# DerekRowell/AudioSDR

Hardware: AMD Instinct MI355X
Metric: Msamples/s through full SSB demod chain, batched 128-sample blocks (higher is better)
Workload: dtype f32

## Files before the change

### audiosdr_amd/binding.py

```python
import ctypes as C
import os

import numpy as np

BLOCK = 128
ALL = -1
STREAM_BATCH = (1 << 64) - 1
LSBmode, USBmode, CW_LSBmode, CW_USBmode, AMmode, SAMmode, WSPRmode = range(7)
(audioAM, audioCW, audioWSPR, audio2100, audio2300, audio2500, audio2700, audio2900, audio3100, audio3300,
 audioBypass) = range(11)
AGCoff, AGCfast, AGCmedium, AGCslow = range(4)
TAPS = ["SCALED_I", "SCALED_Q", "NB_I", "NB_Q", "IF_I", "IF_Q", "MIX_I", "MIX_Q", "DEMOD", "AUDIO_FILT", "AGC", "ALS"]

_HERE = os.path.dirname(os.path.abspath(__file__))


class AsdrError(RuntimeError):
    pass


def library_path():
    return os.path.join(_HERE, "libasdr_hip.so")


def library_sha256(path=None):
    import hashlib
    with open(path or library_path(), "rb") as f:
        return hashlib.sha256(f.read()).hexdigest()


_f, _i, _u = C.c_float, C.c_int, C.c_uint
_SETTERS_VOID = ["init", "enableAudioFilter", "disableAudioFilter", "enableALSfilter", "disableALSfilter",
                 "setALSfilterNotch", "setALSfilterPeak", "setALSfilterAdaptive", "setALSfilterStatic", "enableAGC",
                 "disableAGC", "enableNoiseBlanker", "disableNoiseBlanker"]
_SETTERS_F = ["setInputGain", "setIQgainBalance", "setOutputGain", "setAGCthreshold", "setAGCslope", "setAGCkneeWidth",
              "setAGCattackTime", "setAGCreleaseTime", "setAGChangTime", "setAGCstaticGain", "setNoiseBlankerThreshold",
              "setNoiseBlankerThresholdDb"]
_SETTERS_I = ["setMute", "setAudioFilter", "setAGCmode"]
_GETTERS_F = ["getTuningOffset", "getBPFlower", "getBPFupper", "getAGCthreshold", "getAGCslope", "getAGCkneeWidth",
              "getAGCattack", "getAGCrelease", "getAAGalphaAttack", "getAGCbetaAttack", "getAGCalphaRelease",
              "getAGCbetaRelease", "getAGCstaticGain", "getAMcarrierLevel", "getSAMfrequency"]
_GETTERS_I = ["getMute", "getAudioFilter", "ALSfilterIsEnabled", "ALSfilterIsNotch", "ALSfilterIsPeak",
              "ALSfilterIsAdaptive", "AGCisEnabled", "AGCisActive", "NoiseBlankerisEnabled", "NoiseBlankerDetection",
              "getSAMphaseLockStatus"]

EXPORTS = (["asdr_create", "asdr_destroy", "asdr_last_error", "asdr_n_channels", "asdr_update", "asdr_update_device",
            "asdr_synchronize", "asdr_setDemodMode", "asdr_getDemodMode", "asdr_setALSfilterParams", "asdr_getAGClookup",
            "asdr_read_status", "asdr_control_plane_flush", "asdr_get_chain_constants", "asdr_stream_pipeline_launches", "asdr_schedule_layout", "asdr_set_exact_unknown_mode", "asdr_get_exact_unknown_mode", "asdr_stream_pipeline_recoveries", "asdr_stream_pipeline_max_groups", "asdr_set_stream_fir_helpers", "asdr_stream_pipeline_h3_calls", "asdr_set_stream_pipeline", "asdr_set_sam_launch_form", "asdr_set_als_launch_form", "asdr_debug_set_stream_spin_limit", "asdr_debug_set_stream_max_groups", "asdr_enable_taps", "asdr_read_taps", "asdr_last_kernel_ms", "asdr_version",
            "asdr_kernel_timing_begin", "asdr_kernel_timing_end", "asdr_set_launch_timing", "asdr_region_timing_begin", "asdr_region_timing_end", "asdr_update_device_strided", "asdr_capture_open",
            "asdr_capture_close", "asdr_capture_capacity", "asdr_capture_position", "asdr_capture_rewind",
            "asdr_capture_device_ptr", "asdr_capture_update_device", "asdr_capture_read",
            "asdr_create_sharded", "asdr_n_shards", "asdr_shard", "asdr_shard_first_channel", "asdr_shard_device",
            "asdr_host_alloc", "asdr_host_free", "asdr_host_register", "asdr_host_unregister", "asdr_set_host_chunks",
            "asdr_host_path_info", "asdr_stream_pipeline_alloc_failures", "asdr_set_launch_split", "asdr_order_after", "asdr_order_before", "asdr_lane_calls", "asdr_sam_role_calls", "asdr_sam_chunk_calls", "asdr_als_role_calls", "asdr_set_lanes"] +
           ["asdr_" + n for n in _SETTERS_VOID + _SETTERS_F + _SETTERS_I + _GETTERS_F + _GETTERS_I])

_lib = None


def host_autopin(on=-1):
    return int(load_library().asdr_host_autopin(int(on)))


def host_autopin_clear():
    load_library().asdr_host_autopin_clear()


def host_autopin_info():
    out = (C.c_long * 4)()
    load_library().asdr_host_autopin_info(out)
    return {"registered_now": int(out[0]), "registrations": int(out[1]), "released": int(out[2]), "refused": int(out[3])}


def kernels_launched(reset=False):
    L = load_library()
    out = {}
    for i in range(L.asdr_kernels_count()):
        n = int(L.asdr_kernels_launches(i))
        if n:
            out[L.asdr_kernels_name(i).decode()] = n
    if reset:
        L.asdr_kernels_launches_reset()
    return out


def load_library(path=None):
    global _lib
    if _lib is not None and path is None:
        return _lib
    p = path or library_path()
    if not os.path.exists(p):
        raise AsdrError("%s not found: build it with `python -m audiosdr_amd.build` (hipcc, gfx950). "
                        "There is no CPU fallback." % p)
    L = C.CDLL(p)
    vp, i16p = C.c_void_p, C.POINTER(C.c_int16)
    L.asdr_create.argtypes = [_i, _i]; L.asdr_create.restype = vp
    L.asdr_destroy.argtypes = [vp]; L.asdr_destroy.restype = None
    L.asdr_last_error.restype = C.c_char_p
    L.asdr_version.restype = C.c_char_p
    L.asdr_set_pool_priority.argtypes = [_i]; L.asdr_set_pool_priority.restype = _i
    L.asdr_host_autopin.argtypes = [_i]; L.asdr_host_autopin.restype = _i
    L.asdr_host_autopin_clear.restype = None
    L.asdr_host_autopin_info.argtypes = [C.POINTER(C.c_long)]; L.asdr_host_autopin_info.restype = _i
    L.asdr_kernels_count.restype = _i
    L.asdr_kernels_name.argtypes = [_i]; L.asdr_kernels_name.restype = C.c_char_p
    L.asdr_kernels_launches.argtypes = [_i]; L.asdr_kernels_launches.restype = C.c_ulonglong
    L.asdr_kernels_launches_reset.restype = None
    L.asdr_n_channels.argtypes = [vp]; L.asdr_n_channels.restype = _i
    L.asdr_update.argtypes = [vp, i16p, i16p, i16p, _i]; L.asdr_update.restype = _i
    L.asdr_update_device.argtypes = [vp, vp, vp, vp, _i, vp]; L.asdr_update_device.restype = _i
    L.asdr_synchronize.argtypes = [vp]; L.asdr_synchronize.restype = _i
    L.asdr_update_device_strided.argtypes = [vp, vp, vp, vp, _i, C.c_long, C.c_long, vp]; L.asdr_update_device_strided.restype = _i
    L.asdr_capture_open.argtypes = [vp, C.c_long]; L.asdr_capture_open.restype = _i
    for n in ("asdr_capture_close", "asdr_capture_rewind"):
        getattr(L, n).argtypes = [vp]; getattr(L, n).restype = _i
    for n in ("asdr_capture_capacity", "asdr_capture_position"):
        getattr(L, n).argtypes = [vp]; getattr(L, n).restype = C.c_long
    L.asdr_capture_device_ptr.argtypes = [vp]; L.asdr_capture_device_ptr.restype = vp
    L.asdr_capture_update_device.argtypes = [vp, vp, vp, _i, C.c_long, vp]; L.asdr_capture_update_device.restype = _i
    L.asdr_capture_read.argtypes = [vp, _i, C.c_long, C.c_long, i16p]; L.asdr_capture_read.restype = _i
    L.asdr_last_kernel_ms.argtypes = [vp]; L.asdr_last_kernel_ms.restype = _f
    for n in _SETTERS_VOID:
        fn = getattr(L, "asdr_" + n); fn.argtypes = [vp, _i]; fn.restype = None
    for n in _SETTERS_F:
        fn = getattr(L, "asdr_" + n); fn.argtypes = [vp, _i, _f]; fn.restype = None
    for n in _SETTERS_I:
        fn = getattr(L, "asdr_" + n); fn.argtypes = [vp, _i, _i]; fn.restype = None
    for n in _GETTERS_F:
        fn = getattr(L, "asdr_" + n); fn.argtypes = [vp, _i]; fn.restype = _f
    for n in _GETTERS_I:
        fn = getattr(L, "asdr_" + n); fn.argtypes = [vp, _i]; fn.restype = _i
    L.asdr_setDemodMode.argtypes = [vp, _i, _i]; L.asdr_setDemodMode.restype = _f
    L.asdr_getDemodMode.argtypes = [vp, _i]; L.asdr_getDemodMode.restype = C.c_int16
    L.asdr_setALSfilterParams.argtypes = [vp, _i, _u, _f, _f]; L.asdr_setALSfilterParams.restype = None
    L.asdr_getAGClookup.argtypes = [vp, _i, _i]; L.asdr_getAGClookup.restype = _f
    i32p, fp = C.POINTER(C.c_int32), C.POINTER(C.c_float)
    L.asdr_read_status.argtypes = [vp, i32p, i32p, i32p, fp, fp]; L.asdr_read_status.restype = _i
    if path is None or hasattr(L, "asdr_get_chain_constants"):
        L.asdr_get_chain_constants.argtypes = [vp, _i, C.POINTER(C.c_float)]; L.asdr_get_chain_constants.restype = C.c_uint
    if path is None or hasattr(L, "asdr_control_plane_flush"):
        L.asdr_control_plane_flush.argtypes = [vp, C.POINTER(C.c_longlong)]; L.asdr_control_plane_flush.restype = _i
    L.asdr_enable_taps.argtypes = [vp, _i]; L.asdr_enable_taps.restype = _i
    L.asdr_read_taps.argtypes = [vp, fp]; L.asdr_read_taps.restype = _i
    L.asdr_kernel_timing_begin.argtypes = [vp, _i]; L.asdr_kernel_timing_begin.restype = _i
    if path is None or hasattr(L, "asdr_stream_pipeline_launches"):
        L.asdr_stream_pipeline_launches.argtypes = [vp]; L.asdr_stream_pipeline_launches.restype = C.c_long
    if path is None or hasattr(L, "asdr_set_stream_pipeline"):
        L.asdr_stream_pipeline_recoveries.argtypes = [vp]; L.asdr_stream_pipeline_recoveries.restype = C.c_long
        L.asdr_stream_pipeline_max_groups.argtypes = [vp]; L.asdr_stream_pipeline_max_groups.restype = _i
        if hasattr(L, "asdr_set_stream_fir_helpers"):
            L.asdr_set_stream_fir_helpers.argtypes = [vp, _i]; L.asdr_set_stream_fir_helpers.restype = _i
            L.asdr_stream_pipeline_h3_calls.argtypes = [vp]; L.asdr_stream_pipeline_h3_calls.restype = C.c_long
        L.asdr_set_stream_pipeline.argtypes = [vp, _i]; L.asdr_set_stream_pipeline.restype = _i
        L.asdr_set_sam_launch_form.argtypes = [vp, _i, _i]; L.asdr_set_sam_launch_form.restype = _i
        if hasattr(L, "asdr_set_als_launch_form"):
            L.asdr_set_als_launch_form.argtypes = [vp, _i]; L.asdr_set_als_launch_form.restype = _i
        L.asdr_debug_set_stream_spin_limit.argtypes = [vp, _u]; L.asdr_debug_set_stream_spin_limit.restype = _i
        L.asdr_debug_set_stream_max_groups.argtypes = [vp, _i]; L.asdr_debug_set_stream_max_groups.restype = _i
    if path is None or hasattr(L, "asdr_set_exact_unknown_mode"):
        L.asdr_set_exact_unknown_mode.argtypes = [vp, _i]; L.asdr_set_exact_unknown_mode.restype = _i
        L.asdr_get_exact_unknown_mode.argtypes = [vp]; L.asdr_get_exact_unknown_mode.restype = _i
    if path is None or hasattr(L, "asdr_schedule_layout"):
        L.asdr_schedule_layout.argtypes = [vp, C.POINTER(C.c_int)]; L.asdr_schedule_layout.restype = _i
    if path is None or hasattr(L, "asdr_region_timing_begin"):
        L.asdr_set_launch_timing.argtypes = [vp, _i]; L.asdr_set_launch_timing.restype = _i
        L.asdr_region_timing_begin.argtypes = [vp, vp]; L.asdr_region_timing_begin.restype = _i
        L.asdr_region_timing_end.argtypes = [vp, C.POINTER(C.c_float), C.POINTER(C.c_long)]; L.asdr_region_timing_end.restype = _i
    L.asdr_kernel_timing_end.argtypes = [vp, fp, _i]; L.asdr_kernel_timing_end.restype = _i
    if path is None or hasattr(L, "asdr_create_sharded"):
        L.asdr_create_sharded.argtypes = [_i, _i, C.POINTER(C.c_int)]; L.asdr_create_sharded.restype = vp
        L.asdr_n_shards.argtypes = [vp]; L.asdr_n_shards.restype = _i
        L.asdr_shard.argtypes = [vp, _i]; L.asdr_shard.restype = vp
        L.asdr_shard_first_channel.argtypes = [vp, _i]; L.asdr_shard_first_channel.restype = _i
        L.asdr_shard_device.argtypes = [vp, _i]; L.asdr_shard_device.restype = _i
        L.asdr_host_alloc.argtypes = [C.c_size_t]; L.asdr_host_alloc.restype = vp
        L.asdr_host_free.argtypes = [vp]; L.asdr_host_free.restype = None
        L.asdr_host_register.argtypes = [vp, C.c_size_t]; L.asdr_host_register.restype = _i
        L.asdr_host_unregister.argtypes = [vp]; L.asdr_host_unregister.restype = _i
        L.asdr_set_host_chunks.argtypes = [vp, _i]; L.asdr_set_host_chunks.restype = _i
        L.asdr_host_path_info.argtypes = [vp, C.POINTER(C.c_int)]; L.asdr_host_path_info.restype = _i
        L.asdr_stream_pipeline_alloc_failures.argtypes = [vp]; L.asdr_stream_pipeline_alloc_failures.restype = C.c_long
        L.asdr_set_launch_split.argtypes = [vp, _i, _i]; L.asdr_set_launch_split.restype = _i
        L.asdr_order_after.argtypes = [vp, vp]; L.asdr_order_after.restype = _i
        L.asdr_order_before.argtypes = [vp, vp]; L.asdr_order_before.restype = _i
        L.asdr_lane_calls.argtypes = [vp]; L.asdr_lane_calls.restype = C.c_long
        L.asdr_sam_role_calls.argtypes = [vp]; L.asdr_sam_role_calls.restype = C.c_long
        L.asdr_als_role_calls.argtypes = [vp]; L.asdr_als_role_calls.restype = C.c_long
        L.asdr_sam_chunk_calls.argtypes = [vp]; L.asdr_sam_chunk_calls.restype = C.c_long
        L.asdr_set_lanes.argtypes = [vp, _i, _i]; L.asdr_set_lanes.restype = _i
    if path is None or hasattr(L, "asdr_lanes_overlap_probe"):
        L.asdr_lanes_overlap_probe.argtypes = [vp]; L.asdr_lanes_overlap_probe.restype = _i
        L.asdr_lanes_enabled.argtypes = [vp]; L.asdr_lanes_enabled.restype = _i
        L.asdr_stream_pipeline_headroom_refusals.argtypes = [vp]; L.asdr_stream_pipeline_headroom_refusals.restype = C.c_long
    if path is None:
# ... 112 lines not shown
    def update_device(self, dI, dQ, dOut, n_blocks, stream=0):
        self._chk(self._L.asdr_update_device(self._h, C.c_void_p(dI), C.c_void_p(dQ), C.c_void_p(dOut), int(n_blocks),
                                             C.c_void_p(stream)))

    def update_device_strided(self, dI, dQ, dOut, n_blocks, in_stride_blocks, out_stride_blocks, stream=0):
        self._chk(self._L.asdr_update_device_strided(self._h, C.c_void_p(dI), C.c_void_p(dQ), C.c_void_p(dOut), int(n_blocks),
                                                     int(in_stride_blocks), int(out_stride_blocks), C.c_void_p(stream)))

    def synchronize(self):
        self._chk(self._L.asdr_synchronize(self._h))

    def capture_open(self, capacity_blocks):
        self._chk(self._L.asdr_capture_open(self._h, int(capacity_blocks)))

    def capture_close(self):
        self._chk(self._L.asdr_capture_close(self._h))

    def capture_rewind(self):
        self._chk(self._L.asdr_capture_rewind(self._h))

    @property
    def capture_position(self):
        return int(self._L.asdr_capture_position(self._h))

    @property
    def capture_capacity(self):
        return int(self._L.asdr_capture_capacity(self._h))

    def capture_device_ptr(self):
        return int(self._L.asdr_capture_device_ptr(self._h) or 0)

    def capture_update_device(self, dI, dQ, n_blocks, in_stride_blocks=None, stream=0):
        self._chk(self._L.asdr_capture_update_device(self._h, C.c_void_p(dI), C.c_void_p(dQ), int(n_blocks),
                                                     int(n_blocks if in_stride_blocks is None else in_stride_blocks), C.c_void_p(stream)))

    def capture_read(self, ch, first_block=0, n_blocks=None):
        if n_blocks is None:
            n_blocks = self.capture_position - first_block
        out = np.empty(int(n_blocks) * BLOCK, dtype=np.int16)
        self._chk(self._L.asdr_capture_read(self._h, int(ch), int(first_block), int(n_blocks), out.ctypes.data_as(C.POINTER(C.c_int16))))
        return out

    def chain_constants(self, ch=0):
        out = (C.c_float * 12)()
        hang = int(self._L.asdr_get_chain_constants(self._h, int(ch), out))
        return hang, np.array(list(out), dtype=np.float32)

    def control_plane_flush(self):
        st = (C.c_longlong * 4)()
        self._chk(self._L.asdr_control_plane_flush(self._h, st))
        return {"rows_refilled": int(st[0]), "schedule_rebuilt": bool(st[1]), "waves_plain": int(st[2]) & 0x1FFFFF,
                "waves_sam": (int(st[2]) >> 21) & 0x1FFFFF, "waves_als": (int(st[2]) >> 42) & 0x1FFFFF, "agc_tables_alive": int(st[3])}

    def last_kernel_ms(self):
        return float(self._L.asdr_last_kernel_ms(self._h))

    def set_exact_unknown_mode(self, on=True):
        self._chk(self._L.asdr_set_exact_unknown_mode(self._h, 1 if on else 0))

    def stream_pipeline_launches(self):
        return int(self._L.asdr_stream_pipeline_launches(self._h))

    def stream_pipeline_recoveries(self):
        return int(self._L.asdr_stream_pipeline_recoveries(self._h))

    def stream_pipeline_max_groups(self):
        return int(self._L.asdr_stream_pipeline_max_groups(self._h))

    def set_stream_fir_helpers(self, mode):
        self._chk(self._L.asdr_set_stream_fir_helpers(self._h, int(mode)))

    def stream_pipeline_h3_calls(self):
        return int(self._L.asdr_stream_pipeline_h3_calls(self._h))

    def set_stream_pipeline(self, on=True):
        self._chk(self._L.asdr_set_stream_pipeline(self._h, 1 if on else 0))

    def set_sam_launch_form(self, fused=False, split_min_channels=0):
        self._chk(self._L.asdr_set_sam_launch_form(self._h, 1 if fused else 0, int(split_min_channels)))

    def set_als_launch_form(self, split_min_channels=0):
        self._chk(self._L.asdr_set_als_launch_form(self._h, int(split_min_channels)))

    def debug_set_stream_max_groups(self, groups):
        self._chk(self._L.asdr_debug_set_stream_max_groups(self._h, int(groups)))

    def debug_set_stream_spin_limit(self, polls):
        self._chk(self._L.asdr_debug_set_stream_spin_limit(self._h, int(polls)))

    def schedule_layout(self):
        out = (C.c_int * 8)()
        self._chk(self._L.asdr_schedule_layout(self._h, out))
        v = list(out)
        return {"plain": v[0], "sam": v[1], "als_long": v[2], "als_compact": v[3], "sam_als": v[4], "remainders": v[5],
                "remainder_kind": v[6], "sam_three_launches": bool(v[7] & 1), "als_two_launches": bool(v[7] & 2)}

    def set_launch_timing(self, on):
        self._chk(self._L.asdr_set_launch_timing(self._h, 1 if on else 0))

    def region_timing_begin(self, stream=None):
        self._chk(self._L.asdr_region_timing_begin(self._h, stream))

    def region_timing_end(self):
        ms, n = C.c_float(0.0), C.c_long(0)
        self._chk(self._L.asdr_region_timing_end(self._h, C.byref(ms), C.byref(n)))
        return float(ms.value), int(n.value)
# ... 92 lines not shown
```

### audiosdr_amd/csrc/asdr_device.h

```cpp
#ifndef ASDR_DEVICE_H_
#define ASDR_DEVICE_H_

#include <stdint.h>

#define ASDR_N 128
#define ASDR_PLL_WRAP_MAX 64

#define ASDR_F_NB_EN        (1u << 0)
#define ASDR_F_AF_EN        (1u << 1)
#define ASDR_F_AGC_EN       (1u << 2)
#define ASDR_F_ALS_EN       (1u << 3)
#define ASDR_F_ALS_NOTCH    (1u << 4)
#define ASDR_F_ALS_ADAPTIVE (1u << 5)
#define ASDR_F_MUTED        (1u << 6)

#define ASDR_R_IF   (1u << 0)
#define ASDR_R_AF   (1u << 1)
#define ASDR_R_NB   (1u << 2)
#define ASDR_R_ALS  (1u << 3)
#define ASDR_R_IMG  (1u << 4)
#define ASDR_R_ALL  (1u << 5)

typedef struct {
  uint32_t mode;
// ... 59 lines not shown
#define ASDR_LO_ENTRIES 8
#define ASDR_LO_WRITER 0x100u
#define ASDR_LO_WRITER_LANE(l) (0x100u << (l))

typedef struct {
  uint32_t key_phase, key_inc;
  float phase_end;
  uint32_t pad_;
  float c[ASDR_N], s[ASDR_N];
} LoEntry;

typedef struct {
  const ChanParams *params;
  ChanSmall *small;
  int16_t *nb_hist;
  uint8_t *nb_mask;
  float *hil_q, *hil_i, *als_x, *als_w;
  float *audio_prev;
  const float *agc_tab;
  const SlotInfo *sched;
  int32_t n_sched;
  int32_t n_channels;
  const int16_t *in_i, *in_q;
  int16_t *out;
  int32_t n_blocks;
  uint32_t nb_phase;
  uint32_t als_phase;
  LoEntry *lo_cache;
  uint32_t lo_parity;
  uint32_t lo_write;
  uint32_t lo_writer_bit;
  uint32_t direct_lo;
  int32_t direct_ch0;
  uint32_t direct_mode, direct_flags;
  int32_t in_stride;
  int32_t out_stride;
  float *taps;
  float *xch_a;
  float *xch_b;
  float *xch_c;
  uint32_t *stream_prog;
  uint32_t *stream_err;
  uint32_t stream_spin_limit;
  const uint32_t *run_if;
  int32_t stream_waves;
  float *xch_sam;
  uint32_t *sam_lock;
  uint32_t sam_set, sam_sets;
  uint32_t sam_set_stride, sam_lock_stride;
  float *als_stage;
  uint32_t als_stage_cur, als_stage_prev;
  LoEntry *lo_ring;
  ChainConsts k;
} UpdateArgs;
#define ASDR_ALS_STAGE_SLOTS 32
#define ASDR_ALS_CHUNK 8
#define ASDR_STREAM_DEPTH 4
#define ASDR_LO_RING 8
#define ASDR_STREAM_SPIN_LIMIT (1u << 18)
#define ASDR_STREAM_FAIL 0xFFFFFFFFu
#define ASDR_SNAP_BYTES (448 + 1536 + ASDR_NB_MASK_ROW + 1024 + 1024 + 512)

#define ASDR_KERNEL_PLAIN 0
#define ASDR_KERNEL_SAM 1
#define ASDR_KERNEL_ALS 2
#define ASDR_KERNEL_ALS_SMALL 3
#define ASDR_KERNEL_SAM_ALS 4
#define ASDR_KERNEL_KINDS 5
#ifndef ASDR_SAM_WAVES
#define ASDR_SAM_WAVES 4
#endif

#endif
```

### audiosdr_amd/csrc/asdr_host.cpp

```cpp
#include <hip/hip_runtime.h>

#include <algorithm>
#include <atomic>
#include <chrono>
#include <condition_variable>
#include <functional>
#include <memory>
#include <mutex>
#include <thread>
#include <cmath>
#include <cstdio>
#include <cstring>
#include <string>
#include <unordered_map>
#include <vector>

#include "../../include/asdr.h"
#include "asdr_device.h"
#include "asdr_tables.h"

#ifndef ASDR_SAM_CHUNK
#define ASDR_SAM_CHUNK 8
#define ASDR_SAM_CHUNK_SETS 32
#define ASDR_SAM_CHUNK_MAX_WAVES 512
// ... 118 lines not shown
  explicit CopyPool(int n) { for (int i = 0; i < n; i++) th_.emplace_back([this] { loop(); }); }
  ~CopyPool() { { std::lock_guard<std::mutex> g(m_); quit_ = true; } cv_.notify_all(); for (auto &t : th_) t.join(); }
  int threads() const { return (int)th_.size(); }
  void start(Job *j) { j->workers_left.store((int)th_.size()); { std::lock_guard<std::mutex> g(m_); job_ = j; gen_++; } cv_.notify_all(); }
  static void work(Job *j) {
    const int n_tasks = j->n_chunks * j->slices;
    for (int t; (t = j->next_in.fetch_add(1)) < n_tasks;) { const int k = t / j->slices; j->copy_in(k, t % j->slices, j->slices); j->in_done[k].fetch_add(1, std::memory_order_release); }
    for (int t; (t = j->next_out.fetch_add(1)) < n_tasks;) {
      const int k = t / j->slices;
      while (!j->out_ready[k].load(std::memory_order_acquire)) nap();
      j->copy_out(k, t % j->slices, j->slices); j->out_finished.fetch_add(1, std::memory_order_release);
    }
  }
 private:
  void loop() {
    unsigned long seen = 0;
    for (;;) {
      Job *j;
      { std::unique_lock<std::mutex> g(m_); cv_.wait(g, [&] { return quit_ || gen_ != seen; }); if (quit_) return; seen = gen_; j = job_; }
      work(j);
      j->workers_left.fetch_sub(1, std::memory_order_release);
    }
  }
  std::vector<std::thread> th_;
  std::mutex m_; std::condition_variable cv_;
  Job *job_ = nullptr; unsigned long gen_ = 0; bool quit_ = false;
};

struct HostPlan { int K = 1; std::vector<int> bound, need_in, last_part; long sched_gen = -1; int n_blocks = 0; };

}

#define ASDR_LANES 8
#define ASDR_AUX_STREAMS (ASDR_KERNEL_KINDS + 1 + 8)
struct asdr_batch {
  int n = 0, device = 0;
  hipStream_t stream = nullptr;
  std::vector<Chan> ch;
  std::vector<AgcTable> agc_pool;
  std::unordered_map<uint64_t, std::vector<int>> agc_index;
  std::vector<uint32_t> agc_refs;
  std::vector<ChanParams> hp;
  std::vector<uint32_t> reset;
  std::vector<SlotInfo> sched;
  std::vector<int32_t> dirty;
  std::vector<uint8_t> dirty_flag;
  bool all_dirty = true;
  bool sched_dirty = true, reset_pending = true, agc_pool_dirty = true;
  bool agc_refs_changed = true;
  int reset_lo = 0x7fffffff, reset_hi = -1;
  int kind_first[ASDR_KERNEL_KINDS] = {}, kind_slots[ASDR_KERNEL_KINDS] = {}, kind_uniform_slots[ASDR_KERNEL_KINDS] = {};
  int left_first = 0, left_slots = 0, left_kind = ASDR_KERNEL_PLAIN;
  bool kind_direct[ASDR_KERNEL_KINDS] = {};
  long stat_rows_refilled = 0, stat_sched_rebuilds = 0, stat_bulk_uploads = 0;
  int stat_lo_groups_without_entry = 0;
  ChanParams *d_params = nullptr;
  ChanSmall *d_small = nullptr;
  int16_t *d_nb_hist = nullptr;
  uint8_t *d_nb_mask = nullptr;
  float *d_hil_q = nullptr, *d_hil_i = nullptr, *d_als_x = nullptr,
        *d_als_w = nullptr, *d_agc_tab = nullptr, *d_taps = nullptr;
  float *d_audio_prev = nullptr;
  bool exact_unknown_mode = true;
  size_t agc_tab_cap = 0;
  SlotInfo *d_sched = nullptr;
  uint32_t *d_reset = nullptr;
  int16_t *d_io[3] = {nullptr, nullptr, nullptr};
  int16_t *h_io[3] = {nullptr, nullptr, nullptr};
  size_t h_io_cap = 0;
  hipStream_t h2d_stream = nullptr, d2h_stream = nullptr;
  std::vector<hipEvent_t> ev_host;
  HostPlan host_plan;
  std::unique_ptr<CopyPool> copy_pool;
  int host_chunks_forced = 0;
  hipStream_t lane[ASDR_LANES + 1] = {};
  hipEvent_t ev_lane[ASDR_LANES + 1] = {};
  int n_lanes = 2, n_lanes_sam = 3;
  int sched_lanes = 2;
  bool lanes_pending = false;
  bool sched_sam_heavy = false;
  bool last_was_lanes = false;
  int lanes_min_waves = 1024;
  bool lanes_enabled = true;
  bool lanes_forced = false;
  long stat_lane_calls = 0;
  int launch_split = 1, launch_split_min_waves = 2048;
  int stat_host_chunks = 0, stat_host_pinned = 0;
  std::vector<asdr_batch *> shards;
  std::vector<int> shard_first;
  void *workers = nullptr;
  int16_t *d_capture = nullptr;
  long capture_cap = 0, capture_pos = 0;
  size_t io_cap = 0;
  bool taps_on = false;
  hipEvent_t ev0 = nullptr, ev1 = nullptr;
  bool ev_valid = false;
  bool time_calls = false;
  hipEvent_t rev0 = nullptr, rev1 = nullptr;
  hipStream_t region_stream = nullptr;
  bool region_on_lanes = false;
  long region_calls = -1;
  std::vector<hipEvent_t> tev;
  size_t tev_used = 0;
  hipStream_t last_stream = nullptr;
  hipEvent_t ev_last = nullptr;
  hipStream_t aux[ASDR_AUX_STREAMS] = {};
// ... 132 lines not shown
  c.agc_en = true;
  rebuild_agc(b, c);
}

void chan_init(asdr_batch *b, int idx) {
  Chan &c = b->ch[idx];
  c.audio_table = ASDR_TBL_AUDIO_BASE + ASDR_audio2700;
  c.if_table = ASDR_TBL_IF_SSB;
  mark_reset(b, idx, ASDR_R_AF | ASDR_R_IF | ASDR_R_IMG | ASDR_R_NB);
  agc_init(b, c);
  set_mode(b, idx, ASDR_LSBmode);
  c.muted = false;
}

void fill_params(const Chan &c, ChanParams &p) {
  memset(&p, 0, sizeof p);
  p.mode = c.mode;
  p.flags = (c.nb_en ? ASDR_F_NB_EN : 0u) | (c.af_en ? ASDR_F_AF_EN : 0u) | (c.agc_en ? ASDR_F_AGC_EN : 0u) |
            (c.als_en ? ASDR_F_ALS_EN : 0u) | (c.als_notch ? ASDR_F_ALS_NOTCH : 0u) |
            (c.als_adaptive ? ASDR_F_ALS_ADAPTIVE : 0u) | (c.muted ? ASDR_F_MUTED : 0u);
  p.if_table = c.if_table; p.audio_table = c.audio_table; p.agc_table = c.agc_table;
  p.in_gain_i = c.in_gain_i; p.in_gain_q = c.in_gain_q; p.output_gain = c.output_gain;
  p.freq_shift = c.freq_shift; p.nb_threshold = c.nb_threshold;
  p.agc_alpha_att = c.agc_alpha_att; p.agc_beta_att = c.agc_beta_att;
  p.agc_alpha_rel = c.agc_alpha_rel; p.agc_beta_rel = c.agc_beta_rel;
  p.agc_static_gain = c.agc_static_gain; p.agc_hang_count = c.agc_hang_count;
  p.als_m = c.als_m; p.als_delay = c.als_delay; p.als_lambda = c.als_lambda;
}

int g_force_split = -1;
int kernel_kind(const ChanParams &p) {
  if (g_force_split < 0) g_force_split = getenv("ASDR_FORCE_SPLIT") ? 1 : 0;
  if (g_force_split && !(p.flags & ASDR_F_ALS_EN)) return ASDR_KERNEL_SAM;
  if (p.flags & ASDR_F_ALS_EN) {
    const bool small = p.als_m >= 0 && p.als_m <= 64 && p.als_delay >= 0 && p.als_delay + p.als_m <= 65;
    return !small ? ASDR_KERNEL_ALS : (p.mode == ASDR_SAMmode ? ASDR_KERNEL_SAM_ALS : ASDR_KERNEL_ALS_SMALL);
  }
  return (p.mode == ASDR_SAMmode) ? ASDR_KERNEL_SAM : ASDR_KERNEL_PLAIN;
}
#ifndef ASDR_SAM_SPLIT_MIN_CHANNELS
#define ASDR_SAM_SPLIT_MIN_CHANNELS 512
#endif
uint64_t sched_key(const ChanParams &p) {
  return ((uint64_t)kernel_kind(p) << 60) | ((uint64_t)(p.mode & 0xFFFF) << 40) | ((uint64_t)(p.flags & 0xFF) << 32) |
         ((uint64_t)(p.if_table & 0xFF) << 24) | ((uint64_t)(p.audio_table & 0xFF) << 16) | (uint64_t)(p.agc_table & 0xFFFF);
}

void mark_dirty(asdr_batch *b, int i) {
  if (b->all_dirty) return;
  if (!b->dirty_flag[i]) { b->dirty_flag[i] = 1; b->dirty.push_back(i); }
  if (b->dirty.size() > (size_t)b->n / 8 + 64) { b->all_dirty = true; }
}

void flush_host(asdr_batch *b, std::vector<int32_t> &rows_out, bool &bulk, bool &sched_rebuilt) {
  const int rows = b->n + 1;
  compact_agc_pool(b);
  bulk = b->all_dirty;
  rows_out.clear();
  b->stat_rows_refilled = 0;
  if (bulk) {
    for (int i = 0; i < rows; i++) {
      const uint64_t old_key = sched_key(b->hp[i]);
      fill_params(b->ch[i], b->hp[i]);
      if (i < b->n && sched_key(b->hp[i]) != old_key) b->sched_dirty = true;
    }
    b->stat_rows_refilled = rows;
    b->stat_bulk_uploads++;
  } else if (!b->dirty.empty()) {
    std::sort(b->dirty.begin(), b->dirty.end());
    for (int32_t i : b->dirty) {
      const uint64_t old_key = sched_key(b->hp[i]);
      fill_params(b->ch[i], b->hp[i]);
      if (sched_key(b->hp[i]) != old_key) b->sched_dirty = true;
      b->dirty_flag[i] = 0;
    }
    rows_out = b->dirty;
    b->stat_rows_refilled = (long)rows_out.size();
  }
  b->dirty.clear();
  if (bulk) std::fill(b->dirty_flag.begin(), b->dirty_flag.end(), 0);
  b->all_dirty = false;
  sched_rebuilt = false;
  if (b->sched_dirty) {
    std::vector<std::pair<uint64_t, int32_t>> order(b->n);
    for (int i = 0; i < b->n; i++) order[i] = {sched_key(b->hp[i]), i};
    std::sort(order.begin(), order.end());
    int uni[ASDR_KERNEL_KINDS] = {}, rem[ASDR_KERNEL_KINDS] = {};
    int n_sam = 0;
    for (int i = 0; i < b->n; i++) { const int k = (int)(order[i].first >> 60); n_sam += (k == ASDR_KERNEL_SAM || k == ASDR_KERNEL_SAM_ALS); }
    b->sam_split = !b->sam_fused && n_sam >= b->sam_split_min;
    {
      int n_als_small = 0;
      for (int i = 0; i < b->n; i++) n_als_small += ((int)(order[i].first >> 60) == ASDR_KERNEL_ALS_SMALL);
      b->als_split = n_als_small >= b->als_split_min;
    }
    const bool sam_general_only = !b->sam_split;
    int left = 0; bool left_general = false;
    for (int i = 0; i < b->n;) {
      int j = i + 1;
      while (j < b->n && order[j].first == order[i].first) j++;
      const int k = (int)(order[i].first >> 60), g = j - i;
      if (k == ASDR_KERNEL_SAM && sam_general_only) rem[k] += g;
      else { uni[k] += g / 8 * 8; left += g % 8; if (g % 8) left_general = left_general || (k != ASDR_KERNEL_PLAIN); }
      i = j;
    }
    int pos = 0;
    for (int k = 0; k < ASDR_KERNEL_KINDS; k++) {
      b->kind_first[k] = pos; b->kind_uniform_slots[k] = uni[k]; b->kind_slots[k] = uni[k] + ((rem[k] + 7) / 8) * 8;
      pos += b->kind_slots[k];
    }
    b->left_first = pos; b->left_slots = (left + 7) / 8 * 8; b->left_kind = left_general ? ASDR_KERNEL_ALS : ASDR_KERNEL_PLAIN;
    pos += b->left_slots;
    b->sched.assign(pos, SlotInfo{b->n, b->hp[b->n].mode, b->hp[b->n].flags, 0u});
    int at_u[ASDR_KERNEL_KINDS], at_m[ASDR_KERNEL_KINDS], at_left = b->left_first;
    for (int k = 0; k < ASDR_KERNEL_KINDS; k++) { at_u[k] = b->kind_first[k]; at_m[k] = b->kind_first[k] + uni[k]; }
    std::unordered_map<uint64_t, uint32_t> lo_of_key;
    {
      std::vector<std::pair<int, uint64_t>> cand;
      for (int i = 0; i < b->n;) {
        int j = i + 1;
        while (j < b->n && order[j].first == order[i].first) j++;
        const int k = (int)(order[i].first >> 60), g = j - i;
        const int whole = (k == ASDR_KERNEL_SAM && sam_general_only) ? 0 : g / 8 * 8;
        const uint32_t gm = b->hp[order[i].second].mode;
        const bool mixes_early = (gm == ASDR_USBmode || gm == ASDR_LSBmode || gm == ASDR_CW_USBmode || gm == ASDR_CW_LSBmode || gm == ASDR_WSPRmode || gm == ASDR_AMmode);
        if (whole > 0 && mixes_early) cand.push_back({-whole, order[i].first});
        i = j;
      }
// ... 5 lines not shown
      int j = i + 1;
      while (j < b->n && order[j].first == order[i].first) j++;
      const int k = (int)(order[i].first >> 60), g = j - i;
      const bool fused = (k == ASDR_KERNEL_SAM && sam_general_only);
      const int whole = fused ? 0 : g / 8 * 8;
      const auto lo_it = lo_of_key.find(order[i].first);
      const uint32_t lo_id = (whole > 0 && lo_it != lo_of_key.end()) ? lo_it->second : 0u;
      for (int t = 0; t < g; t++) {
        const int c = order[i + t].second;
        int &at = (t < whole) ? at_u[k] : (fused ? at_m[k] : at_left);
        const uint32_t lo = (t < whole) ? (lo_id | ((t < 8 && lo_id) ? ASDR_LO_WRITER : 0u)) : 0u;
        b->sched[at++] = SlotInfo{c, b->hp[c].mode, b->hp[c].flags, lo};
      }
      i = j;
    }
    {
      const int sam_slots_ = b->kind_slots[ASDR_KERNEL_SAM] + b->kind_slots[ASDR_KERNEL_SAM_ALS];
      b->sched_sam_heavy = b->sam_split && 2 * sam_slots_ >= pos;
      b->sched_lanes = b->sched_sam_heavy ? b->n_lanes_sam : b->n_lanes;
    }
    for (int k = 0; k < ASDR_KERNEL_KINDS; k++) {
      const long w = b->kind_uniform_slots[k] / 8;
      for (int l = 1; l < b->sched_lanes; l++) {
        const int lo = b->kind_first[k] + (int)(w * l / b->sched_lanes) * 8, hi = b->kind_first[k] + (int)(w * (l + 1) / b->sched_lanes) * 8;
        uint32_t seen = 0;
        for (int sl = lo; sl < hi; sl += 8) {
          const uint32_t id = b->sched[sl].lo & 0xFFu;
          if (id == 0u || (seen >> id) & 1u) continue;
          seen |= 1u << id;
          for (int t = 0; t < 8; t++) b->sched[sl + t].lo |= ASDR_LO_WRITER_LANE(l);
        }
      }
    }
    for (int k = 0; k < ASDR_KERNEL_KINDS; k++) {
      const SlotInfo *sl = b->sched.data() + b->kind_first[k];
      bool direct = b->kind_uniform_slots[k] > 0;
      for (int j = 1; j < b->kind_uniform_slots[k] && direct; j++)
        direct = (sl[j].ch == sl[0].ch + j) && sl[j].mode == sl[0].mode && sl[j].flags == sl[0].flags;
      b->kind_direct[k] = direct;
    }
    {
      const SlotInfo *sl = b->sched.data() + b->kind_first[ASDR_KERNEL_PLAIN];
      bool ssb = b->kind_uniform_slots[ASDR_KERNEL_PLAIN] > 0;
      for (int j = 0; j < b->kind_uniform_slots[ASDR_KERNEL_PLAIN] && ssb; j += 8) {
        const uint32_t m = sl[j].mode;
        ssb = (m == ASDR_USBmode || m == ASDR_LSBmode || m == ASDR_CW_USBmode || m == ASDR_CW_LSBmode || m == ASDR_WSPRmode ||
               m == ASDR_AMmode);
      }
      b->plain_uniform_ssb = ssb;
    }
    b->sched_dirty = false;
    sched_rebuilt = true;
    b->stat_sched_rebuilds++;
  }
}

int flush(asdr_batch *b, hipStream_t stream) {
  const int rows = b->n + 1;
  std::vector<int32_t> changed;
  bool bulk = false, sched_rebuilt = false;
  flush_host(b, changed, bulk, sched_rebuilt);
  bool uploaded = false;
  if (b->agc_pool_dirty) {
    const size_t need = b->agc_pool.size() * ASDR_AGC_TAB_ROW;
    if (need > b->agc_tab_cap) {
      HIPCHK(hipStreamSynchronize(stream));
      if (b->d_agc_tab) HIPCHK(hipFree(b->d_agc_tab));
      b->agc_tab_cap = need * 2;
      HIPCHK(hipMalloc(&b->d_agc_tab, b->agc_tab_cap * sizeof(float)));
    }
    std::vector<float> flat(need);
    for (size_t i = 0; i < b->agc_pool.size(); i++) memcpy(&flat[i * ASDR_AGC_TAB_ROW], b->agc_pool[i].v, sizeof(float) * ASDR_AGC_TAB_ROW);
    HIPCHK(hipMemcpyAsync(b->d_agc_tab, flat.data(), need * sizeof(float), hipMemcpyHostToDevice, stream));
    HIPCHK(hipStreamSynchronize(stream));
    b->agc_pool_dirty = false;
  }
  if (bulk) {
    HIPCHK(hipMemcpyAsync(b->d_params, b->hp.data(), rows * sizeof(ChanParams), hipMemcpyHostToDevice, stream));
    uploaded = true;
  } else {
    for (size_t i = 0; i < changed.size();) {
      size_t j = i + 1;
      while (j < changed.size() && changed[j] == changed[j - 1] + 1) j++;
      HIPCHK(hipMemcpyAsync(b->d_params + changed[i], &b->hp[changed[i]], (j - i) * sizeof(ChanParams), hipMemcpyHostToDevice, stream));
      uploaded = true;
      i = j;
    }
  }
  if (sched_rebuilt) {
    HIPCHK(hipMemcpyAsync(b->d_sched, b->sched.data(), b->sched.size() * sizeof(SlotInfo), hipMemcpyHostToDevice, stream));
    uploaded = true;
  }
  if (uploaded) HIPCHK(hipStreamSynchronize(stream));
  return 0;
}

void fill_args(asdr_batch *b, UpdateArgs &a) {
  memset(&a, 0, sizeof a);
  a.params = b->d_params; a.small = b->d_small;
  a.nb_hist = b->d_nb_hist; a.nb_mask = b->d_nb_mask; a.hil_q = b->d_hil_q; a.hil_i = b->d_hil_i;
  a.als_x = b->d_als_x; a.als_w = b->d_als_w; a.agc_tab = b->d_agc_tab;
  a.audio_prev = b->exact_unknown_mode ? b->d_audio_prev : nullptr;
  a.sched = b->d_sched; a.n_sched = 0; a.n_channels = b->n;
  a.taps = b->taps_on ? b->d_taps : nullptr;
  a.nb_phase = b->nb_phase; a.als_phase = b->als_phase;
  a.lo_cache = b->d_lo; a.lo_parity = b->lo_parity; a.lo_write = 0; a.lo_writer_bit = ASDR_LO_WRITER;
  a.k = b->k;
}

int apply_resets(asdr_batch *b, hipStream_t stream) {
  if (!b->reset_pending) return 0;
  const int lo = b->reset_lo < 0 ? 0 : b->reset_lo, hi = b->reset_hi > b->n ? b->n : b->reset_hi;
  if (hi >= lo) {
    const int cnt = hi - lo + 1;
    HIPCHK(hipMemcpyAsync(b->d_reset + lo, b->reset.data() + lo, cnt * sizeof(uint32_t), hipMemcpyHostToDevice, stream));
    UpdateArgs a;
    fill_args(b, a);
    if (asdr_launch_reset(&a, b->d_reset, lo, cnt, stream) != 0) return fail("reset kernel launch failed");
    HIPCHK(hipStreamSynchronize(stream));
    std::fill(b->reset.begin() + lo, b->reset.begin() + hi + 1, 0u);
  }
  b->reset_pending = false; b->reset_lo = 0x7fffffff; b->reset_hi = -1;
  return 0;
}

inline bool is_sharded(const asdr_batch *b) { return b && !b->shards.empty(); }
asdr_batch *shard_of(asdr_batch *b, int &ch) {
  if (ch < 0 || ch >= b->n) return nullptr;
  const std::vector<int> &f = b->shard_first;
  int g = (int)(std::upper_bound(f.begin(), f.end(), ch) - f.begin()) - 1;
  ch -= f[g];
  return b->shards[g];
}
template <typename F>
void each(asdr_batch *&b, int ch, F f) {
  if (!b) return;
  if (is_sharded(b)) {
    asdr_batch *const parent = b;
    if (ch == ASDR_ALL) { for (asdr_batch *sh : parent->shards) { b = sh; each(b, ASDR_ALL, f); } }
    else { int local = ch; asdr_batch *sh = shard_of(parent, local); if (sh) { b = sh; each(b, local, f); } }
    b = parent;
    return;
  }
  if (ch == ASDR_ALL) { for (int i = 0; i < b->n; i++) f(i, b->ch[i]); b->all_dirty = true; }
  else if (ch >= 0 && ch < b->n) { f(ch, b->ch[ch]); mark_dirty(b, ch); }
  else return;
}
const Chan *get(asdr_batch *&b, int ch) {
  if (is_sharded(b)) { asdr_batch *sh = shard_of(b, ch); if (!sh) return nullptr; b = sh; }
  return (b && ch >= 0 && ch < b->n) ? &b->ch[ch] : nullptr;
}

constexpr int kPoolMax = 16;
int g_pool_priority = -1;
bool g_pool_created = false;
struct StreamPool { hipStream_t s[kPoolMax] = {}; int size = 0; std::mutex m; };
StreamPool g_pool[16];
constexpr int kPoolDevices = 16;
hipStream_t pool_stream(int device, int i) {
  if (device < 0 || device >= kPoolDevices) return nullptr;
// ... 73 lines not shown
  }
  return 0;
}
int sync_all(asdr_batch *b) {
  HIPCHK(hipStreamSynchronize(b->last_stream));
  HIPCHK(hipStreamSynchronize(b->stream));
  if (b->lanes_pending) { for (int l = 0; l < ASDR_LANES + 1; l++) if (b->lane[l]) HIPCHK(hipStreamSynchronize(b->lane[l])); b->lanes_pending = false; }

  return 0;
}

int check_stream_error(asdr_batch *b) {
  if (!b->stream_launched || !b->d_stream_prog) return 0;
  if (sync_all(b) != 0) return -1;
  uint32_t *word = b->d_stream_prog + 3 * ((b->n + 7) / 8) + 1, v[2] = {0, 0};
  HIPCHK(hipMemcpy(v, word, sizeof v, hipMemcpyDeviceToHost));
  b->stream_launched = false;
  b->stat_stream_recoveries = (long)v[1];
  if (v[0]) return fail("streaming pipeline: error word still set after the recovery launches (internal error)");
  return 0;
}

int read_small(asdr_batch *b, int ch, ChanSmall &s) {
  if (!b || ch < 0 || ch >= b->n) return fail("bad channel");
  if (is_sharded(b)) b = shard_of(b, ch);
  if (b->device == ASDR_NO_DEVICE) return fail("control-plane-only batch has no device state");
  HIPCHK(hipSetDevice(b->device));
  if (sync_all(b) != 0) return -1;
  if (check_stream_error(b) != 0) return -1;
  if (apply_resets(b, b->stream) != 0) return -1;
  HIPCHK(hipMemcpy(&s, b->d_small + ch, sizeof s, hipMemcpyDeviceToHost));
  return 0;
}

}

#define FOR_SHARDS(b, call) do { if (is_sharded(b)) { for (asdr_batch *sh_ : (b)->shards) { const int rc_ = (call); if (rc_ != 0) return rc_; } return 0; } } while (0)

extern "C" {

const char *asdr_last_error(void) { return g_err.c_str(); }
}
int asdr_internal_fail(const std::string &m) { return fail(m); }
extern "C" {
const char *asdr_version(void) { return "asdr-hip 0.1 (gfx950, wave64, -ffp-contract=off)"; }

asdr_batch_t *asdr_create(int n_channels, int device) {
  if (n_channels <= 0 || n_channels > (1 << 20)) { fail("n_channels must be in 1..1048576"); return nullptr; }
  asdr_batch *b = new asdr_batch();
  b->n = n_channels; b->device = device;
  b->sam_fused = getenv("ASDR_SAM_FUSED") != nullptr;
  b->sam_split_min = getenv("ASDR_SAM_SPLIT_MIN") ? atoi(getenv("ASDR_SAM_SPLIT_MIN")) : ASDR_SAM_SPLIT_MIN_CHANNELS;
  b->stream_pipeline = getenv("ASDR_NO_STREAM_PIPELINE") == nullptr;
  b->als_split_min = getenv("ASDR_ALS_SPLIT_MIN") ? atoi(getenv("ASDR_ALS_SPLIT_MIN")) : 0x7fffffff;
  if (getenv("ASDR_LAUNCH_SPLIT")) b->launch_split = std::max(1, std::min(atoi(getenv("ASDR_LAUNCH_SPLIT")), 8));
  if (getenv("ASDR_LAUNCH_SPLIT_MIN_WAVES")) b->launch_split_min_waves = std::max(8, atoi(getenv("ASDR_LAUNCH_SPLIT_MIN_WAVES")));
  const size_t rows = (size_t)n_channels + 1;
  if (device != ASDR_NO_DEVICE) {
    int ndev = 0;
    if (hipGetDeviceCount(&ndev) != hipSuccess || ndev <= 0) { delete b; fail("no HIP device: libasdr_hip has no CPU path"); return nullptr; }
    if (device < 0 || device >= ndev) { delete b; fail("bad device ordinal"); return nullptr; }
    if (device >= 16) { delete b; fail("device ordinal >= 16: the per-device stream pool of this library has 16 entries"); return nullptr; }
    if (hipSetDevice(device) != hipSuccess) { delete b; fail("hipSetDevice failed"); return nullptr; }
    autopin_batch_created();
    bool ok = true;
    auto alloc = [&](void **p, size_t bytes) { if (ok && hipMalloc(p, bytes) != hipSuccess) ok = false; };
    alloc((void **)&b->d_params, rows * sizeof(ChanParams));
    alloc((void **)&b->d_small, rows * sizeof(ChanSmall));
    alloc((void **)&b->d_nb_hist, rows * 768 * sizeof(int16_t));
    alloc((void **)&b->d_nb_mask, rows * ASDR_NB_MASK_ROW * sizeof(uint8_t));
    alloc((void **)&b->d_hil_q, rows * 256 * sizeof(float));
    alloc((void **)&b->d_hil_i, rows * 256 * sizeof(float));
    alloc((void **)&b->d_als_x, rows * 256 * sizeof(float));
    alloc((void **)&b->d_als_w, rows * 128 * sizeof(float));
    alloc((void **)&b->d_audio_prev, rows * 128 * sizeof(float));
    if (ok && hipMemset(b->d_audio_prev, 0, rows * 128 * sizeof(float)) != hipSuccess) ok = false;
    alloc((void **)&b->d_sched, (rows + 32) * sizeof(SlotInfo));
    alloc((void **)&b->d_reset, rows * sizeof(uint32_t));
    alloc((void **)&b->d_lo, (1 + ASDR_LANES) * 2 * ASDR_LO_ENTRIES * sizeof(LoEntry));
    if (ok && hipMemset(b->d_lo, 0xFF, (1 + ASDR_LANES) * 2 * ASDR_LO_ENTRIES * sizeof(LoEntry)) != hipSuccess) ok = false;
    if (ok && hipStreamSynchronize(nullptr) != hipSuccess) ok = false;
    for (int i = 0; i < ASDR_LANES + 1 && ok; i++)
      if (hipEventCreateWithFlags(&b->ev_lane[i], hipEventDisableTiming) != hipSuccess) ok = false;
    b->lanes_enabled = getenv("ASDR_NO_LANES") == nullptr;
    b->sam_role_streams = getenv("ASDR_NO_SAM_ROLE_STREAMS") == nullptr;
    b->als_role_streams = getenv("ASDR_NO_ALS_ROLE_STREAMS") == nullptr;
    if (getenv("ASDR_ALS_ROLE_STAGES")) b->als_role_stages = atoi(getenv("ASDR_ALS_ROLE_STAGES")) == 2 ? 2 : 3;
    if (ok && (b->stream = pool_stream(device, 0)) == nullptr) ok = false;
    if (ok && hipEventCreate(&b->ev0) != hipSuccess) ok = false;
    if (ok && hipEventCreate(&b->ev1) != hipSuccess) ok = false;
    if (ok && hipEventCreate(&b->rev0) != hipSuccess) ok = false;
    if (ok && hipEventCreate(&b->rev1) != hipSuccess) ok = false;
    if (ok && hipEventCreateWithFlags(&b->ev_last, hipEventDisableTiming) != hipSuccess) ok = false;
    if (ok && hipEventCreateWithFlags(&b->ev_fork, hipEventDisableTiming) != hipSuccess) ok = false;
    for (int i = 0; i < ASDR_AUX_STREAMS && ok; i++)
      if (hipEventCreateWithFlags(&b->ev_join[i], hipEventDisableTiming) != hipSuccess) ok = false;
    if (ok && asdr_kernels_upload_tables() != 0) ok = false;
    if (ok) {
      int cus = 0;
      const int cap = asdr_stream_capacity(device, &cus, 1);
      const int cap3 = asdr_stream_capacity(device, nullptr, 3);
      b->stream_cap_h3 = cap3 > 0 ? cap3 : 0; b->stream_cus = cus;
      { const char *e = getenv("ASDR_STREAM_H3"); if (e) b->stream_h3 = atoi(e) != 0 ? 1 : 0; }
      b->stream_cap_workgroups = cap > 0 ? cap : 0;
      b->stream_max_waves = cap >= 3 ? cap / 3 : 0;
      if (b->stream_max_waves > ASDR_STREAM_MAX_WAVES) b->stream_max_waves = ASDR_STREAM_MAX_WAVES;
      b->stream_query_waves = b->stream_max_waves;
    }
    if (!ok) { fail("device allocation / table upload failed"); asdr_destroy(b); return nullptr; }
  }

  ChainConsts &k = b->k;
  k.if_center = kIFcenter;
  k.two_pi_f = (float)(2.0 * kPI);
  k.half_pi_f = (float)(0.5 * kPI);
  k.inv_two_pi_d = 1.0 / (double)k.two_pi_f;
  k.sin_index_scale_d = (65535.0 / (double)k.two_pi_f) * (1.0 + 0x1p-49);
  k.half_pi_d = kPI / 2.0;
  k.phase_inc_unit = k.two_pi_f / kFs;
  k.nb_alpha = 0.995f;
  k.nb_beta = (float)(1.0 - (double)k.nb_alpha);
  {
    const float wn = 0.07f, zeta = 0.707f, Ka = 1000.f;
    const float tau1 = Ka / (wn * wn);
    const float tau2 = 2 * zeta / wn;
    k.pll_b0 = (float)((double)(2 * Ka / tau1) * (1.0 + 2.0 * (double)tau2));
    k.pll_b1 = (float)((double)(2 * Ka / tau1) * (1.0 - 2.0 * (double)tau2));
    k.pll_a1 = -1.0f;
  }
  k.pll_alpha_freq = 0.995f;
  k.pll_beta_freq = (float)(1.0 - (double)k.pll_alpha_freq);
  k.pll_f_conv = kFs / k.two_pi_f;
  k.pll_lock_lo = (float)((double)kIFcenter - 1000.0);
  k.pll_lock_hi = (float)((double)kIFcenter + 1000.0);

  b->ch.assign(rows, Chan());
  b->hp.resize(rows);
  memset(b->hp.data(), 0, rows * sizeof(ChanParams));
  b->dirty_flag.assign(rows, 0);
  b->reset.assign(rows, ASDR_R_ALL);
  b->reset_lo = 0; b->reset_hi = (int)rows - 1;
  for (size_t i = 0; i < rows; i++) chan_init(b, (int)i);
  b->all_dirty = true; b->sched_dirty = true; b->reset_pending = true;
  return b;
}

asdr_batch_t *asdr_create_sharded(int n_channels, int n_shards, const int *devices) {
  if (n_channels <= 0 || n_channels > (1 << 23)) { fail("n_channels must be in 1..8388608"); return nullptr; }
  if (n_shards <= 0 || n_shards > 64 || n_shards > n_channels || !devices) { fail("n_shards must be in 1..min(64, n_channels), with one device ordinal per shard"); return nullptr; }
  asdr_batch *b = new asdr_batch();
  b->n = n_channels; b->device = ASDR_NO_DEVICE;
  b->shard_first.resize((size_t)n_shards + 1);
  for (int g = 0; g <= n_shards; g++) b->shard_first[g] = (int)(((long)n_channels * g) / n_shards);
  for (int g = 0; g < n_shards; g++) {
    asdr_batch *sh = asdr_create(b->shard_first[g + 1] - b->shard_first[g], devices[g]);
    if (!sh) { const std::string e = g_err; asdr_destroy(b); fail("shard " + std::to_string(g) + ": " + e); return nullptr; }
    b->shards.push_back(sh);
  }
  b->k = b->shards[0]->k;
  return b;
}
int asdr_n_shards(const asdr_batch_t *b) { return b ? (is_sharded(b) ? (int)b->shards.size() : 1) : 0; }
asdr_batch_t *asdr_shard(asdr_batch_t *b, int shard) {
  if (!b) return nullptr;
  if (!is_sharded(b)) return shard == 0 ? b : nullptr;
  return (shard >= 0 && shard < (int)b->shards.size()) ? b->shards[shard] : nullptr;
}
int asdr_shard_first_channel(const asdr_batch_t *b, int shard) {
  if (!b) return -1;
  if (!is_sharded(b)) return shard == 0 ? 0 : (shard == 1 ? b->n : -1);
  return (shard >= 0 && shard <= (int)b->shards.size()) ? b->shard_first[shard] : -1;
}
int asdr_shard_device(const asdr_batch_t *b, int shard) {
  if (!b) return ASDR_NO_DEVICE;
  if (!is_sharded(b)) return b->device;
  return (shard >= 0 && shard < (int)b->shards.size()) ? b->shards[shard]->device : ASDR_NO_DEVICE;
}

void asdr_destroy(asdr_batch_t *b) {
  if (!b) return;
  if (is_sharded(b) || !b->shard_first.empty()) { shard_workers_stop(b); for (asdr_batch *sh : b->shards) asdr_destroy(sh); delete b; return; }
  if (b->device == ASDR_NO_DEVICE) { delete b; return; }
  hipSetDevice(b->device);
  hipDeviceSynchronize();
  autopin_batch_gone();
  void *ptrs[] = {b->d_params, b->d_small, b->d_nb_hist, b->d_nb_mask, b->d_hil_q, b->d_hil_i, b->d_als_x, b->d_als_w,
                  b->d_agc_tab, b->d_taps, b->d_sched, b->d_reset, b->d_lo, b->d_io[0], b->d_io[1], b->d_io[2], b->d_capture,
                  b->d_xch_a, b->d_xch_b, b->d_stream_prog, b->d_lo_ring, b->d_xch_sam, b->d_audio_prev, b->d_stream_snap, b->d_als_stage, b->d_xch_sam_chunk};
  for (void *p : ptrs) if (p) hipFree(p);
  b->copy_pool.reset();
  for (int i = 0; i < 3; i++) if (b->h_io[i]) hipHostFree(b->h_io[i]);
  for (hipEvent_t e : b->ev_host) hipEventDestroy(e);
// ... 96 lines not shown
  if (als_roles) {
    const uintptr_t in_bytes = ((uintptr_t)(b->n - 1) * (uintptr_t)in_stride_blocks + (uintptr_t)n_blocks) * ASDR_N * sizeof(int16_t);
    const uintptr_t out_bytes = ((uintptr_t)(b->n - 1) * (uintptr_t)out_stride_blocks + (uintptr_t)n_blocks) * ASDR_N * sizeof(int16_t);
    const uintptr_t o0 = (uintptr_t)dOut, o1 = o0 + out_bytes;
    for (uintptr_t i0 : {(uintptr_t)dI, (uintptr_t)dQ}) if (o0 < i0 + in_bytes && i0 < o1) als_roles = false;
  }
  if (als_roles && !b->d_als_stage) {
    float *st = nullptr;
    if (hipMalloc(&st, (size_t)(b->n + 1) * ASDR_ALS_STAGE_SLOTS * ASDR_N * sizeof(float)) == hipSuccess) b->d_als_stage = st; else { (void)hipGetLastError(); als_roles = false; }
  }
  const bool per_block = n_blocks > 1 && (sam_split || als_split || total_slots >= 8 * ASDR_PER_BLOCK_LAUNCH_WAVES);
  bool io_alias = false;
  {
    const uintptr_t in_bytes = ((uintptr_t)(b->n - 1) * (uintptr_t)in_stride_blocks + (uintptr_t)n_blocks) * ASDR_N * sizeof(int16_t);
    const uintptr_t out_bytes = ((uintptr_t)(b->n - 1) * (uintptr_t)out_stride_blocks + (uintptr_t)n_blocks) * ASDR_N * sizeof(int16_t);
    const uintptr_t o0 = (uintptr_t)dOut, o1 = o0 + out_bytes;
    for (uintptr_t i0 : {(uintptr_t)dI, (uintptr_t)dQ}) io_alias = io_alias || (o0 < i0 + in_bytes && i0 < o1);
  }
  int pipe_sub = -1, other_waves = 0;
  for (int i = 0; i < n_sub; i++) { if (subs[i].kind == ASDR_KERNEL_PLAIN && subs[i].uniform) pipe_sub = i; else other_waves += subs[i].slots / 8; }
  bool take_pipeline = parts == 1 && b->stream_pipeline && !io_alias && n_blocks >= ASDR_STREAM_MIN_BLOCKS && pipe_sub >= 0 && b->plain_uniform_ssb &&
                       other_waves <= ASDR_STREAM_SIDE_WAVES && !sam_split && !als_split &&
#ifndef ASDR_TIMELINE
                       !b->taps_on &&
#endif
                       subs[pipe_sub].slots / 8 <= b->stream_max_waves;
  if (take_pipeline && other_waves > 0 && b->stream_cap_workgroups > 0 &&
      3 * (subs[pipe_sub].slots / 8) + other_waves + ASDR_STREAM_SIDE_MARGIN > b->stream_cap_workgroups) { take_pipeline = false; b->stat_stream_headroom_refusals++; }
  if (take_pipeline) {
    if (!b->d_xch_a) {
      float *xa = nullptr, *xb = nullptr; uint32_t *prog = nullptr; LoEntry *ring = nullptr; void *snap = nullptr;
      const size_t n_prog = (size_t)(3 * ((b->n + 7) / 8) + 3);
      bool ok = hipMalloc(&xa, (size_t)(b->n + 1) * ASDR_STREAM_DEPTH * 2 * ASDR_N * sizeof(float)) == hipSuccess &&
                hipMalloc(&xb, (size_t)(b->n + 1) * ASDR_STREAM_DEPTH * (ASDR_N + 1) * sizeof(float)) == hipSuccess &&
                hipMalloc(&prog, n_prog * sizeof(uint32_t)) == hipSuccess &&
                hipMalloc(&ring, ASDR_LO_RING * sizeof(LoEntry)) == hipSuccess &&
                hipMalloc(&snap, (size_t)(((b->n + 7) / 8) * 8) * ASDR_SNAP_BYTES) == hipSuccess &&
                hipMemsetAsync(prog, 0, n_prog * sizeof(uint32_t), stream) == hipSuccess;
      if (!ok) {
        for (void *p : {(void *)xa, (void *)xb, (void *)prog, (void *)ring, snap}) if (p) hipFree(p);
        (void)hipGetLastError();
        b->stream_pipeline = false; b->stat_stream_alloc_failures++; take_pipeline = false;
      } else {
        b->d_xch_a = xa; b->d_xch_b = xb; b->d_stream_prog = prog; b->d_lo_ring = ring; b->d_stream_snap = snap;
      }
    }
  }
  if (take_pipeline) {
    const UpdateArgs a_side = a;
    const int w = subs[pipe_sub].slots / 8;
    HIPCHK(hipMemsetAsync(b->d_stream_prog, 0, (size_t)(3 * w + 1) * sizeof(uint32_t), stream));
    if (n_sub > 1) HIPCHK(hipEventRecord(b->ev_fork, stream));
    a.sched = b->d_sched + subs[pipe_sub].first; a.n_sched = subs[pipe_sub].slots;
    a.direct_ch0 = -1;
    if (b->kind_direct[ASDR_KERNEL_PLAIN]) { const SlotInfo &s0 = b->sched[subs[pipe_sub].first]; a.direct_ch0 = s0.ch; a.direct_mode = s0.mode; a.direct_flags = s0.flags; a.direct_lo = s0.lo; }
    a.lo_write = 0u;
    a.xch_a = b->d_xch_a; a.xch_b = b->d_xch_b; a.xch_c = b->d_xch_b + (size_t)(b->n + 1) * ASDR_STREAM_DEPTH * ASDR_N; a.stream_prog = b->d_stream_prog; a.stream_err = b->d_stream_prog + 3 * ((b->n + 7) / 8) + 1;
    a.stream_waves = w; a.lo_ring = b->d_lo_ring; a.stream_spin_limit = b->stream_spin_limit;
    if (e0) HIPCHK(hipEventRecord(e0, stream));
    if (asdr_launch_stream_snapshot(&a, b->d_stream_snap, 0, stream) != 0) return fail("stream snapshot launch failed");
    const bool h3 = b->stream_h3 != 0 && b->stream_cap_h3 > 0 && 3 * w + other_waves + ASDR_STREAM_SIDE_MARGIN <= b->stream_cap_h3 &&
                    (b->stream_h3 == 1 || 3 * w <= b->stream_cus);
    if (h3) b->stat_stream_h3_calls++;
    if (asdr_launch_stream(&a, stream, h3 ? 3 : 1) != 0) return fail("stream kernel launch failed");
    if (asdr_launch_stream_snapshot(&a, b->d_stream_snap, 1, stream) != 0) return fail("stream restore launch failed");
    {
      UpdateArgs f = a;
      f.run_if = a.stream_err; f.stream_waves = 0; f.xch_a = nullptr; f.xch_b = nullptr; f.xch_c = nullptr; f.stream_prog = nullptr; f.lo_ring = nullptr;
      if (asdr_launch_update(&f, ASDR_KERNEL_PLAIN, 1, stream) != 0) return fail("stream fallback launch failed");
    }
    if (asdr_launch_stream_ack(a.stream_err, stream) != 0) return fail("stream acknowledge launch failed");
    {
      int n_aux = 0;
      for (int i = 0; i < n_sub; i++) {
        if (i == pipe_sub) continue;
        hipStream_t s = aux_stream(b, n_aux++);
        if (!s) return fail("stream creation failed");
        HIPCHK(hipStreamWaitEvent(s, b->ev_fork, 0));
        UpdateArgs o = a_side;
        o.sched = b->d_sched + subs[i].first; o.n_sched = subs[i].slots; o.direct_ch0 = -1; o.lo_write = 1u;
        if (subs[i].uniform && b->kind_direct[subs[i].kind]) { const SlotInfo &s0 = b->sched[subs[i].first]; o.direct_ch0 = s0.ch; o.direct_mode = s0.mode; o.direct_flags = s0.flags; o.direct_lo = s0.lo; }
        if (asdr_launch_update(&o, subs[i].kind, subs[i].uniform, s) != 0) return fail("update kernel launch failed");
        HIPCHK(hipEventRecord(b->ev_join[n_aux - 1], s));
      }
      for (int j = 0; j < n_aux; j++) HIPCHK(hipStreamWaitEvent(stream, b->ev_join[j], 0));
    }
    if (e1) HIPCHK(hipEventRecord(e1, stream));
    b->stream_launched = true; b->stat_stream_launches++;
    b->ev_last_valid = true;
    b->ev_valid = (e0 != nullptr && e0 == b->ev0);
    if (b->region_calls >= 0) b->region_calls++;
    b->last_stream = stream; b->last_was_lanes = false;
    b->nb_phase = (b->nb_phase + (uint32_t)(n_blocks % 3)) % 3u;
    b->als_phase = (b->als_phase + (uint32_t)n_blocks) & 1u;
    b->lo_parity ^= 1u;
    return 0;
  }
  const int n_launch = per_block ? n_blocks : 1;
  float *const taps = a.taps;
  if (e0 && part == 0) HIPCHK(hipEventRecord(e0, stream));
  if (use_lanes) {
    if (batch_stream) {
      if (b->ev_last_valid && !b->last_was_lanes) {
        HIPCHK(hipEventRecord(b->ev_last, b->last_stream));
        for (int i = 0; i <= b->sched_lanes; i++) { hipStream_t ls = lane_stream(b, i == b->sched_lanes ? ASDR_LANES : i); if (!ls) return fail("stream creation failed"); HIPCHK(hipStreamWaitEvent(ls, b->ev_last, 0)); }
      }
    } else {
      HIPCHK(hipEventRecord(b->ev_fork, stream));
      for (int i = 0; i <= b->sched_lanes; i++) { hipStream_t ls = lane_stream(b, i == b->sched_lanes ? ASDR_LANES : i); if (!ls) return fail("stream creation failed"); HIPCHK(hipStreamWaitEvent(ls, b->ev_fork, 0)); }
    }
    const int NL = b->sched_lanes;
    for (int l = 0; l <= NL; l++) {
      hipStream_t ls = lane_stream(b, (l == NL) ? ASDR_LANES : l);
      if (!ls) return fail("stream creation failed");
      for (int lb = 0; lb < n_launch; lb++) {
        for (int i = 0; i < n_sub; i++) {
          const Sub &su = subs[i];
          const long w = su.slots / 8;
          int lo = (int)(w * l / NL) * 8, cnt = (int)(w * (l + 1) / NL) * 8 - lo;
          if (l == NL) { lo = 0; cnt = su.uniform ? 0 : su.slots; } else if (!su.uniform) cnt = 0;
          const int first = su.first + lo;
          if (cnt == 0) continue;
          UpdateArgs al = a;
          al.sched = b->d_sched + first; al.n_sched = cnt;
          al.direct_ch0 = -1;
          if (su.uniform && b->kind_direct[su.kind]) { const SlotInfo &s0 = b->sched[su.first]; al.direct_ch0 = s0.ch + lo; al.direct_mode = s0.mode; al.direct_flags = s0.flags; al.direct_lo = s0.lo; }
          al.lo_cache = b->d_lo + (size_t)(1 + (l % ASDR_LANES)) * 2 * ASDR_LO_ENTRIES;
          al.lo_write = 1u;
          al.lo_writer_bit = ASDR_LO_WRITER_LANE(l % ASDR_LANES);
          if (sam_split && (su.kind == ASDR_KERNEL_SAM || su.kind == ASDR_KERNEL_SAM_ALS)) set_sam_rows(al, su.kind, first, 0);
          const int form = (als_split && su.kind == ASDR_KERNEL_ALS_SMALL && su.uniform) ? 2 : su.uniform;
          if (per_block) {
            al.in_i = dI + (size_t)lb * ASDR_N; al.in_q = dQ + (size_t)lb * ASDR_N; al.out = dOut + (size_t)lb * ASDR_N; al.n_blocks = 1;
            al.nb_phase = (b->nb_phase + (uint32_t)(lb % 3)) % 3u;
            al.als_phase = (b->als_phase + (uint32_t)lb) & 1u;
            al.lo_parity = b->lo_parity ^ (uint32_t)(lb & 1);
          }
          if (asdr_launch_update(&al, su.kind, form, ls) != 0) return fail("update kernel launch failed");
        }
      }
    }
    if (!batch_stream) { if (lanes_join_into(b, stream) != 0) return -1; b->lanes_pending = false; b->last_was_lanes = false; b->last_stream = stream; }
    else { b->lanes_pending = true; b->last_was_lanes = true; }
    b->ev_last_valid = true; b->ev_valid = false; b->stat_lane_calls++;
    if (b->region_calls >= 0) b->region_calls++;
    b->nb_phase = (b->nb_phase + (uint32_t)(n_blocks % 3)) % 3u;
    b->als_phase = (b->als_phase + (uint32_t)n_blocks) & 1u;
    b->lo_parity ^= (uint32_t)(n_launch & 1);
    return 0;
  }
  struct Item { int sub, first, slots; };
  Item items[ASDR_AUX_STREAMS + 1]; int n_items = 0;
  for (int i = 0; i < n_sub; i++) {
    const long w = subs[i].slots / 8;
    const int lo = (int)(w * part / parts) * 8, cnt = (int)(w * (part + 1) / parts) * 8 - lo;
    if (cnt == 0) continue;
    int pieces = 1;
    if (b->launch_split > 1 && cnt / 8 >= b->launch_split_min_waves) pieces = std::min(b->launch_split, ASDR_AUX_STREAMS + 1 - n_items - (n_sub - 1 - i));
    if (pieces < 1) pieces = 1;
    for (int q = 0; q < pieces; q++) {
      const int qlo = (int)((long)(cnt / 8) * q / pieces) * 8, qhi = (int)((long)(cnt / 8) * (q + 1) / pieces) * 8;
      if (qhi > qlo && n_items < ASDR_AUX_STREAMS + 1) items[n_items++] = Item{i, subs[i].first + lo + qlo, qhi - qlo};
    }
  }
  int main_item = 0;
  for (int i = 1; i < n_items; i++) if (items[i].slots > items[main_item].slots) main_item = i;
  const bool sam_roles = b->sam_role_streams && per_block && n_launch >= 2 && parts == 1 && n_items == 1 && taps == nullptr && sam_split &&
                         (subs[items[0].sub].kind == ASDR_KERNEL_SAM || subs[items[0].sub].kind == ASDR_KERNEL_SAM_ALS);
  hipStream_t s_pre = nullptr, s_pll = nullptr;
  if (sam_roles) {
    s_pre = aux_stream(b, 0); s_pll = aux_stream(b, 1);
    if (!s_pre || !s_pll) return fail("stream creation failed");
    for (int i = 0; i < 6; i++) if (!b->ev_role[i]) HIPCHK(hipEventCreateWithFlags(&b->ev_role[i], hipEventDisableTiming));
    HIPCHK(hipEventRecord(b->ev_fork, stream));
    HIPCHK(hipStreamWaitEvent(s_pre, b->ev_fork, 0)); HIPCHK(hipStreamWaitEvent(s_pll, b->ev_fork, 0));
    b->stat_sam_role_calls++;
  }
  bool sam_chunks = sam_roles && subs[items[0].sub].kind == ASDR_KERNEL_SAM && subs[items[0].sub].uniform && n_blocks >= 2 * ASDR_SAM_CHUNK &&
                    items[0].slots <= 8 * ASDR_SAM_CHUNK_MAX_WAVES && getenv("ASDR_NO_SAM_CHUNKS") == nullptr;
  auto chunk_tiles = [&](int slots) -> bool {
    if ((size_t)slots <= b->xch_sam_chunk_slots) return true;
    if (hipStreamSynchronize(stream) != hipSuccess) return false;
    float *grown = nullptr;
    const size_t per_set = (size_t)slots * 2 * ASDR_N * sizeof(float) + (size_t)slots * sizeof(uint32_t);
    if (hipMalloc(&grown, ASDR_SAM_CHUNK_SETS * per_set) != hipSuccess) { (void)hipGetLastError(); return false; }
    if (b->d_xch_sam_chunk) hipFree(b->d_xch_sam_chunk);
    b->d_xch_sam_chunk = grown; b->xch_sam_chunk_slots = (size_t)slots;
    return true;
  };
  if (sam_chunks && !chunk_tiles(items[0].slots)) sam_chunks = false;
  int parity_launches_sam = -1;
  if (sam_chunks) {
    constexpr int S = ASDR_SAM_CHUNK_SETS, G = ASDR_SAM_CHUNK, R = S / G;
    static_assert(S % G == 0 && R >= 4, "tile sets for four chunks");
    for (int i = 0; i < 3 * R; i++) if (!b->ev_samc[i]) HIPCHK(hipEventCreateWithFlags(&b->ev_samc[i], hipEventDisableTiming));
    const int i0 = items[0].sub, first0 = items[0].first;
    const size_t slots = b->xch_sam_chunk_slots;
    a.sched = b->d_sched + first0; a.n_sched = items[0].slots; a.direct_ch0 = -1; a.lo_write = 1u;
    if (b->kind_direct[subs[i0].kind]) { const SlotInfo &s0 = b->sched[subs[i0].first]; a.direct_ch0 = s0.ch; a.direct_mode = s0.mode; a.direct_flags = s0.flags; a.direct_lo = s0.lo; }
    a.xch_sam = b->d_xch_sam_chunk; a.sam_lock = reinterpret_cast<uint32_t *>(b->d_xch_sam_chunk + (size_t)S * slots * 2 * ASDR_N);
    a.sam_sets = (uint32_t)S; a.sam_set_stride = (uint32_t)(slots * 2 * ASDR_N); a.sam_lock_stride = (uint32_t)slots;
    a.taps = nullptr;
    const int n_chunks = (n_blocks + G - 1) / G;
    auto chunk_args = [&](int k) {
      const int b0 = k * G, g = (n_blocks - b0 < G) ? n_blocks - b0 : G;
      a.in_i = dI + (size_t)b0 * ASDR_N; a.in_q = dQ + (size_t)b0 * ASDR_N; a.out = dOut + (size_t)b0 * ASDR_N; a.n_blocks = g;
      a.nb_phase = (b->nb_phase + (uint32_t)(b0 % 3)) % 3u;
      a.als_phase = (b->als_phase + (uint32_t)b0) & 1u;
      a.lo_parity = b->lo_parity ^ (uint32_t)(k & 1);
      a.sam_set = (uint32_t)(b0 % S);
    };
    for (int k = 0; k <= n_chunks; k++) {
      if (k < n_chunks) {
        const int kr = k % R;
        chunk_args(k);
        if (asdr_launch_sam_role(&a, ASDR_KERNEL_SAM, 1, 0, stream) != 0) return fail("update kernel launch failed");
        HIPCHK(hipEventRecord(b->ev_samc[kr], stream)); HIPCHK(hipStreamWaitEvent(s_pll, b->ev_samc[kr], 0));
        if (asdr_launch_sam_role(&a, ASDR_KERNEL_SAM, 1, 1, s_pll) != 0) return fail("update kernel launch failed");
        HIPCHK(hipEventRecord(b->ev_samc[R + kr], s_pll));
      }
      if (k >= 1) {
        chunk_args(k - 1);
        HIPCHK(hipStreamWaitEvent(stream, b->ev_samc[R + (k - 1) % R], 0));
        if (asdr_launch_sam_role(&a, ASDR_KERNEL_SAM, 1, 2, stream) != 0) return fail("update kernel launch failed");
      }
    }
    parity_launches_sam = n_chunks;
    b->stat_sam_chunk_calls++;
  }
  const bool als_role_call = als_roles && n_items == 1 && taps == nullptr;
  int parity_launches = n_launch;
  if (als_role_call) {
    constexpr int S = ASDR_ALS_STAGE_SLOTS, G = ASDR_ALS_CHUNK, R = S / G;
    static_assert(S % G == 0 && R >= 3, "the stage holds at least three chunks");
    hipStream_t s_chain = aux_stream(b, 0);
    if (!s_chain) return fail("stream creation failed");
    for (int i = 0; i < 2 * R; i++) if (!b->ev_als[i]) HIPCHK(hipEventCreateWithFlags(&b->ev_als[i], hipEventDisableTiming));
    HIPCHK(hipEventRecord(b->ev_fork, stream));
    HIPCHK(hipStreamWaitEvent(s_chain, b->ev_fork, 0));
    const int i0 = items[0].sub, first0 = items[0].first;
    a.sched = b->d_sched + first0; a.n_sched = items[0].slots; a.direct_ch0 = -1; a.lo_write = 1u;
    if (b->kind_direct[subs[i0].kind]) { const SlotInfo &s0 = b->sched[subs[i0].first]; a.direct_ch0 = s0.ch; a.direct_mode = s0.mode; a.direct_flags = s0.flags; a.direct_lo = s0.lo; }
    a.als_stage = b->d_als_stage; a.als_stage_cur = 0u; a.als_stage_prev = (uint32_t)(S - 1); a.als_phase = b->als_phase;
    if (asdr_launch_als_stage_seed(&a, 0, b->n, s_chain) != 0) return fail("update kernel launch failed");
    const int n_chunks = (n_blocks + G - 1) / G;
    static_assert(ASDR_SAM_CHUNK == ASDR_ALS_CHUNK, "the two chunked forms share the tile sets");
    constexpr int RT = ASDR_SAM_CHUNK_SETS / G;
    static_assert(RT == R, "the front stage's wait indexes ev_als[(k - RT) % R]: the event of back chunk k - RT only while tile sets and stage slots hold the same number of chunks");
    hipStream_t s_front = nullptr;
    bool three = b->als_role_stages == 3 && chunk_tiles(items[0].slots);
    if (three) { s_front = aux_stream(b, 1); if (!s_front) three = false; }
    if (three) {
      for (int i = 2 * R; i < 3 * R; i++) if (!b->ev_als[i]) HIPCHK(hipEventCreateWithFlags(&b->ev_als[i], hipEventDisableTiming));
      HIPCHK(hipStreamWaitEvent(s_front, b->ev_fork, 0));
      const size_t slots = b->xch_sam_chunk_slots;
      a.xch_sam = b->d_xch_sam_chunk; a.sam_lock = reinterpret_cast<uint32_t *>(b->d_xch_sam_chunk + (size_t)ASDR_SAM_CHUNK_SETS * slots * 2 * ASDR_N);
      a.sam_sets = (uint32_t)ASDR_SAM_CHUNK_SETS; a.sam_set_stride = (uint32_t)(slots * 2 * ASDR_N); a.sam_lock_stride = (uint32_t)slots;
    }
    for (int k = 0; k < n_chunks; k++) {
      const int b0 = k * G, g = (n_blocks - b0 < G) ? n_blocks - b0 : G;
      a.in_i = dI + (size_t)b0 * ASDR_N; a.in_q = dQ + (size_t)b0 * ASDR_N; a.out = dOut + (size_t)b0 * ASDR_N; a.n_blocks = g;
      a.nb_phase = (b->nb_phase + (uint32_t)(b0 % 3)) % 3u;
      a.als_phase = (b->als_phase + (uint32_t)b0) & 1u;
      a.lo_parity = b->lo_parity ^ (uint32_t)(k & 1);
      a.als_stage_cur = (uint32_t)(b0 % S); a.als_stage_prev = (uint32_t)((b0 + S - 1) % S);
      a.sam_set = (uint32_t)(b0 % ASDR_SAM_CHUNK_SETS);
      if (three) {
        if (k >= RT) HIPCHK(hipStreamWaitEvent(s_front, b->ev_als[(k - RT) % R], 0));
        if (asdr_launch_als_role(&a, 2, s_front) != 0) return fail("update kernel launch failed");
        HIPCHK(hipEventRecord(b->ev_als[2 * R + k % R], s_front)); HIPCHK(hipStreamWaitEvent(s_chain, b->ev_als[2 * R + k % R], 0));
      }
      if (k >= R - 1) HIPCHK(hipStreamWaitEvent(s_chain, b->ev_als[R + (k + 1) % R], 0));
      if (asdr_launch_als_role(&a, three ? 3 : 0, s_chain) != 0) return fail("update kernel launch failed");
      HIPCHK(hipEventRecord(b->ev_als[k % R], s_chain)); HIPCHK(hipStreamWaitEvent(stream, b->ev_als[k % R], 0));
      if (asdr_launch_als_role(&a, 1, stream) != 0) return fail("update kernel launch failed");
      HIPCHK(hipEventRecord(b->ev_als[R + k % R], stream));
    }
    parity_launches = n_chunks;
    b->stat_als_role_calls++;
  }
  if (parity_launches_sam >= 0) parity_launches = parity_launches_sam;
  for (int lb = 0; lb < ((als_role_call || sam_chunks) ? 0 : n_launch); lb++) {
    if (per_block) {
      a.in_i = dI + (size_t)lb * ASDR_N; a.in_q = dQ + (size_t)lb * ASDR_N; a.out = dOut + (size_t)lb * ASDR_N; a.n_blocks = 1;
      a.nb_phase = (b->nb_phase + (uint32_t)(lb % 3)) % 3u;
      a.als_phase = (b->als_phase + (uint32_t)lb) & 1u;
      a.lo_parity = b->lo_parity ^ (uint32_t)(lb & 1);
      a.taps = (lb == n_launch - 1) ? taps : nullptr;
    }
    if (n_items > 1) HIPCHK(hipEventRecord(b->ev_fork, stream));
    int n_aux = 0;
    for (int it = 0; it < n_items; it++) {
      const int i = items[it].sub, first = items[it].first;
      hipStream_t s = (it == main_item) ? stream : aux_stream(b, n_aux++);
      if (!s && it != main_item) return fail("stream creation failed");
      if (it != main_item) HIPCHK(hipStreamWaitEvent(s, b->ev_fork, 0));
      a.sched = b->d_sched + first; a.n_sched = items[it].slots;
      a.direct_ch0 = -1;
      a.lo_write = 1u;
      if (subs[i].uniform && b->kind_direct[subs[i].kind]) {
        const SlotInfo &s0 = b->sched[subs[i].first];
        a.direct_ch0 = s0.ch + (first - subs[i].first); a.direct_mode = s0.mode; a.direct_flags = s0.flags; a.direct_lo = s0.lo;
        if (first != subs[i].first) a.lo_write = 0u;
      }
      const bool sam3 = sam_split && (subs[i].kind == ASDR_KERNEL_SAM || subs[i].kind == ASDR_KERNEL_SAM_ALS);
      if (sam3) set_sam_rows(a, subs[i].kind, first, sam_roles ? (lb & 1) : 0);
      const int form = (als_split && subs[i].kind == ASDR_KERNEL_ALS_SMALL && subs[i].uniform) ? 2 : subs[i].uniform;
      if (sam_roles) {
        const int pa = lb & 1;
        if (lb >= 2) HIPCHK(hipStreamWaitEvent(s_pre, b->ev_role[4 + pa], 0));
        if (asdr_launch_sam_role(&a, subs[i].kind, form, 0, s_pre) != 0) return fail("update kernel launch failed");
        HIPCHK(hipEventRecord(b->ev_role[pa], s_pre)); HIPCHK(hipStreamWaitEvent(s_pll, b->ev_role[pa], 0));
        if (asdr_launch_sam_role(&a, subs[i].kind, form, 1, s_pll) != 0) return fail("update kernel launch failed");
        HIPCHK(hipEventRecord(b->ev_role[2 + pa], s_pll)); HIPCHK(hipStreamWaitEvent(stream, b->ev_role[2 + pa], 0));
        if (asdr_launch_sam_role(&a, subs[i].kind, form, 2, stream) != 0) return fail("update kernel launch failed");
        HIPCHK(hipEventRecord(b->ev_role[4 + pa], stream));
        continue;
      }
      if (asdr_launch_update(&a, subs[i].kind, form, s) != 0) return fail("update kernel launch failed");
      if (it != main_item) HIPCHK(hipEventRecord(b->ev_join[n_aux - 1], s));
    }
    for (int j = 0; j < n_aux; j++) HIPCHK(hipStreamWaitEvent(stream, b->ev_join[j], 0));
  }
  if (part + 1 < parts) return 0;
  if (e1) HIPCHK(hipEventRecord(e1, stream));
  b->ev_last_valid = true;
  b->ev_valid = (e0 != nullptr && e0 == b->ev0);
  if (b->region_calls >= 0) b->region_calls++;
  b->last_stream = stream; b->last_was_lanes = false;
  b->nb_phase = (b->nb_phase + (uint32_t)(n_blocks % 3)) % 3u;
  b->als_phase = (b->als_phase + (uint32_t)n_blocks) & 1u;
  b->lo_parity ^= (uint32_t)(parity_launches & 1);
  return 0;
}

extern "C" {
int asdr_update_device_strided(asdr_batch_t *b, const int16_t *dI, const int16_t *dQ, int16_t *dOut, int n_blocks,
                               long in_stride_blocks, long out_stride_blocks, void *stream_) {
  if (is_sharded(b)) {
    if (!dI || !dQ) return 0;
    if (!dOut) return fail("null output");
    for (asdr_batch *sh : b->shards) if (sh->device != b->shards[0]->device || sh->device == ASDR_NO_DEVICE)
      return fail("sharded batch over several devices: device pointers go to the shards (asdr_shard), host rows to asdr_update");
    for (size_t g = 0; g < b->shards.size(); g++) {
      const size_t f = (size_t)b->shard_first[g];
      if (update_device_part(b->shards[g], dI + f * (size_t)in_stride_blocks * ASDR_N, dQ + f * (size_t)in_stride_blocks * ASDR_N,
                             dOut + f * (size_t)out_stride_blocks * ASDR_N, n_blocks, in_stride_blocks, out_stride_blocks, stream_, 0, 1) != 0) return -1;
    }
    return 0;
  }
  return update_device_part(b, dI, dQ, dOut, n_blocks, in_stride_blocks, out_stride_blocks, stream_, 0, 1);
}

int asdr_update_device(asdr_batch_t *b, const int16_t *dI, const int16_t *dQ, int16_t *dOut, int n_blocks, void *stream_) {
  return asdr_update_device_strided(b, dI, dQ, dOut, n_blocks, n_blocks, n_blocks, stream_);
// ... 834 lines not shown
  b->sam_fused = fused != 0;
  b->sam_split_min = split_min_channels > 0 ? split_min_channels : ASDR_SAM_SPLIT_MIN_CHANNELS;
  b->sched_dirty = true;
  return 0;
}
int asdr_debug_set_stream_max_groups(asdr_batch_t *b, int groups) {
  if (!b) return fail("null batch");
  FOR_SHARDS(b, asdr_debug_set_stream_max_groups(sh_, groups));
  if (groups < 0 || groups > ASDR_STREAM_MAX_WAVES) return fail("bad group count");
  if (b->stream_query_waves > 0 && groups > b->stream_query_waves) groups = b->stream_query_waves;
  b->stream_max_waves = groups;
  return 0;
}
int asdr_debug_set_stream_spin_limit(asdr_batch_t *b, unsigned int polls) {
  if (!b) return fail("null batch");
  FOR_SHARDS(b, asdr_debug_set_stream_spin_limit(sh_, polls));
  b->stream_spin_limit = polls ? polls : ASDR_STREAM_SPIN_LIMIT;
  return 0;
}

int asdr_set_exact_unknown_mode(asdr_batch_t *b, int on) {
  if (!b) return fail("null batch");
  FOR_SHARDS(b, asdr_set_exact_unknown_mode(sh_, on));
  const bool want = on != 0;
  if (want && !b->exact_unknown_mode && b->device != ASDR_NO_DEVICE) {
    HIPCHK(hipSetDevice(b->device));
    if (sync_all(b) != 0) return -1;
    HIPCHK(hipMemset(b->d_audio_prev, 0, ((size_t)b->n + 1) * 128 * sizeof(float)));
    HIPCHK(hipStreamSynchronize(nullptr));
  }
  b->exact_unknown_mode = want;
  return 0;
}
int asdr_get_exact_unknown_mode(asdr_batch_t *b) { if (is_sharded(b)) b = b->shards[0]; return b ? (b->exact_unknown_mode ? 1 : 0) : -1; }

int asdr_schedule_layout(asdr_batch_t *b, int out[8]) {
  if (!b || !out) return fail("null argument");
  if (is_sharded(b)) {
    int acc[8] = {0, 0, 0, 0, 0, 0, -1, 0};
    for (asdr_batch *sh : b->shards) {
      int o[8];
      if (asdr_schedule_layout(sh, o) != 0) return -1;
      for (int k = 0; k < 6; k++) acc[k] += o[k];
      acc[6] = std::max(acc[6], o[6]); acc[7] |= o[7];
    }
    memcpy(out, acc, sizeof acc);
    return 0;
  }
  for (int k = 0; k < ASDR_KERNEL_KINDS; k++) out[k] = b->kind_slots[k];
  out[5] = b->left_slots; out[6] = b->left_slots ? b->left_kind : -1; out[7] = (b->sam_split ? 1 : 0) | (b->als_split ? 2 : 0);
  return 0;
}

int asdr_control_plane_flush(asdr_batch_t *b, long long stats[4]) {
  if (!b) return fail("null batch");
  if (is_sharded(b)) {
    long long acc[4] = {0, 0, 0, 0};
    for (asdr_batch *sh : b->shards) {
      long long st[4];
      if (asdr_control_plane_flush(sh, st) != 0) return -1;
      acc[0] += st[0]; acc[1] |= st[1]; acc[2] += st[2]; acc[3] += st[3];
    }
    if (stats) memcpy(stats, acc, sizeof acc);
    return 0;
  }
  if (b->device != ASDR_NO_DEVICE) return fail("asdr_control_plane_flush is for control-plane-only batches: a device batch flushes in update()");
  std::vector<int32_t> changed;
  bool bulk = false, rebuilt = false;
  flush_host(b, changed, bulk, rebuilt);
  b->agc_pool_dirty = false;
  if (stats) {
    stats[0] = b->stat_rows_refilled; stats[1] = rebuilt ? 1 : 0;
    const int lw = b->left_slots / 8;
    stats[2] = (long long)(b->kind_slots[ASDR_KERNEL_PLAIN] / 8 + (b->left_kind == ASDR_KERNEL_PLAIN ? lw : 0)) | ((long long)(b->kind_slots[ASDR_KERNEL_SAM] / 8) << 21) |
               ((long long)((b->kind_slots[ASDR_KERNEL_ALS] + b->kind_slots[ASDR_KERNEL_ALS_SMALL] + b->kind_slots[ASDR_KERNEL_SAM_ALS]) / 8 + (b->left_kind == ASDR_KERNEL_ALS ? lw : 0)) << 42);
    long long live = 0;
    for (uint32_t r : b->agc_refs) live += (r != 0);
    stats[3] = live;
  }
  return 0;
}

int asdr_enable_taps(asdr_batch_t *b, int on) {
  if (!b) return fail("null batch");
  FOR_SHARDS(b, asdr_enable_taps(sh_, on));
  if (b->device == ASDR_NO_DEVICE) return fail("control-plane-only batch has no device state");
  HIPCHK(hipSetDevice(b->device));
  if (on && !b->d_taps) {
    const size_t bytes = (size_t)ASDR_N_TAPS * b->n * ASDR_N * sizeof(float);
    HIPCHK(hipMalloc(&b->d_taps, bytes));
    HIPCHK(hipMemset(b->d_taps, 0, bytes));
    HIPCHK(hipStreamSynchronize(nullptr));
  }
  b->taps_on = on != 0;
  return 0;
}

int asdr_read_taps(asdr_batch_t *b, float *dst) {
  if (is_sharded(b)) {
    if (!dst) return fail("taps not enabled");
    std::vector<float> tmp;
    for (size_t g = 0; g < b->shards.size(); g++) {
      asdr_batch *sh = b->shards[g];
      tmp.resize((size_t)ASDR_N_TAPS * sh->n * ASDR_N);
      if (asdr_read_taps(sh, tmp.data()) != 0) return -1;
      for (int t = 0; t < ASDR_N_TAPS; t++)
// ... 12 lines not shown
```

### audiosdr_amd/csrc/asdr_kernels.hip

```cpp
#include <hip/hip_runtime.h>
#include <stdint.h>
#include <stddef.h>
#include <string.h>
#include <stdlib.h>
#include <type_traits>

#include "asdr_device.h"
#include "asdr_tables.h"
#include "../../include/asdr.h"

#define W0 0
#define W1 128
#define PH 256
#define XP 0
#ifndef ASDR_STRIDE
#define ASDR_STRIDE 388
#endif
#ifndef ASDR_AGC_QUIET_PATH
#define ASDR_AGC_QUIET_PATH 1
#endif
#ifndef ASDR_MW_OWN_STORES
#define ASDR_MW_OWN_STORES 1
#endif
#ifndef ASDR_AGC_LEAN
// ... 819 lines not shown
          const int i = 128 + n, h = s8 >> 2;
          float y = 0.0f;
          if (als_m_default) y = als_dot_split_const<ALS_M_DEFAULT>(L + AW + WH * h, L + XB + (i - D - h), h);
          else if (als_m_uniform) y = als_dot_split_uniform(L + AW + WH * h, L + XB + (i - D - h), M_u, h);
          else if (als_en && adaptive) y = als_dot_split(L + AW + WH * h, L + XB + (i - D - h), M, h);
          if (mine) {
            const float e = L[XB + i] - y;
            L[OUT + n] = notch ? e : y;
            if ((n & 3) == 0) L[SCR] = e;
          }
        } else if (mine) {
          if constexpr (!COMPACT) {
            const int i = 128 + n;
            const float y = als_dot<true, WH>(L + AW, L + XB, i - D, M);
            const float e = L[XB + i] - y;
            L[OUT + n] = notch ? e : y;
            if ((n & 3) == 0) L[SCR] = e;
          }
        }
        WAVE_SYNC();
        const int nu = (ep < 0) ? 0 : 4 * ep + 4;
        if (als_en && adaptive && nu < ASDR_N) {
          const float e = L[SCR];
          const int iu = 128 + nu;
          if (als_m_default) {
            als_tap_update_const<ALS_M_DEFAULT>(L + XB + iu - D - s8, L + AW + ALS_TAP(s8, WH), e, lam, s8);
          } else if (als_m_uniform && als_safe) {
            const float *xq = L + XB + iu - D - s8;
            float *wq = L + AW + ALS_TAP(s8, WH);
            const int nk = (M_u - s8 + 7) >> 3, nk_max = (M_u + 7) >> 3;
#pragma unroll 1
            for (int k0 = 0; k0 < nk_max; k0 += 8) {
              float xv[8], wv[8];
#pragma unroll
              for (int j = 0; j < 8; ++j) { xv[j] = xq[-8 * (k0 + j)]; wv[j] = wq[4 * (k0 + j)]; }
#pragma unroll
              for (int j = 0; j < 8; ++j) { const float gq = e * xv[j]; const float dq = lam * gq; const float wn = wv[j] + dq; wv[j] = (k0 + j < nk) ? wn : wv[j]; }
#pragma unroll
              for (int j = 0; j < 8; ++j) wq[4 * (k0 + j)] = wv[j];
            }
          } else if (als_safe) {
#pragma unroll 2
            for (int q = s8; q < M; q += 8) { const float gq = e * L[XB + iu - D - q]; const float dq = lam * gq; L[AW + ALS_TAP(q, WH)] += dq; }
          } else {
            if constexpr (!COMPACT) {
              for (int q = s8; q < M; q += 8) { const float gq = e * (((iu - D - q) >= 0 && (iu - D - q) < 256) ? L[XB + (iu - D - q)] : 0.0f); const float dq = lam * gq; L[AW + ALS_TAP(q, WH)] += dq; }
            }
          }
        }
        WAVE_SYNC();
      }
    }
}
template <int STRIDE, bool HAS_ALS, bool HAS_SAM, bool UNIFORM, int WAVES, int ROLE = 0, bool ONEBLK_ = false, int FIR_HELPERS = 1>
__device__ __forceinline__ void asdr_update_body(const UpdateArgs &a, float *lds_wg) {
  constexpr bool C16 = (STRIDE == 320);
  constexpr bool PRE_ROLE = (ROLE == 4 || ROLE == 8), POST_ROLE = (ROLE == 5 || ROLE == 9 || ROLE == 10), LOOPED_ROLE = (ROLE == 7 || ROLE == 8 || ROLE == 9 || ROLE == 10);
  constexpr bool DO1 = (ROLE == 0 || ROLE == 1 || PRE_ROLE || ROLE == 6 || ROLE == 7), DO2 = (ROLE == 0 || ROLE == 2 || POST_ROLE || ROLE == 6 || ROLE == 7),
                 DO3 = (ROLE == 0 || ROLE == 3 || POST_ROLE || ROLE == 6 || ROLE == 7);
  constexpr bool TO_ALS = (ROLE == 6 || ROLE == 7 || ROLE == 10);
#ifndef ASDR_ALS_FULL_OPT
#define ASDR_ALS_FULL_OPT 2
#endif
  constexpr bool ALS_LOOPFREE = (ASDR_ONEBLK_ALS != 0) && (ONEBLK_ || (ROLE >= 4 && !LOOPED_ROLE && ASDR_ONEBLK_ROLES));
  constexpr bool ALS_FULL_OPT = (ASDR_ALS_FULL_OPT >= 1) && ASDR_COMPACT_ROWS(STRIDE) && ALS_LOOPFREE,
                 ALS_FULL_OPT2 = (ASDR_ALS_FULL_OPT >= 2) && ASDR_COMPACT_ROWS(STRIDE) && ALS_LOOPFREE;
  constexpr bool STREAM = (ROLE >= 1 && ROLE <= 3);
  constexpr bool PIPE_PK = ((ASDR_PIPE_PK_MASK & 1) && HAS_ALS) || ((ASDR_PIPE_PK_MASK & 2) && !HAS_ALS && !HAS_SAM && ROLE == 0) ||
                           ((ASDR_PIPE_PK_MASK & 4) && (HAS_SAM || ROLE > 3)) || ((ASDR_PIPE_PK_MASK & 8) && STREAM);
  if (ROLE == 0 && a.run_if != nullptr && *a.run_if == 0u) return;
  constexpr bool MW = (WAVES > 1) && !HAS_SAM && (ROLE == 0);
  constexpr int MW_SHARE = MW ? ASDR_MW_SHARE : 0;
  const int wave = (WAVES > 1) ? (int)(threadIdx.x >> 6) : 0;
#ifndef ASDR_MW_ROT
#define ASDR_MW_ROT 0
#endif
  const uint32_t mw_b = blockIdx.x;
  const uint32_t mw_rot = (ASDR_MW_ROT == 0) ? mw_b : (ASDR_MW_ROT == 1) ? (mw_b >> 3) : (ASDR_MW_ROT == 2) ? ((mw_b >> 3) + (mw_b >> 8)) :
                          (ASDR_MW_ROT == 3) ? ((mw_b * 0x9E3779B1u) >> 30) : (ASDR_MW_ROT == 4) ? ((mw_b >> 3) % 3u) : (mw_b >> 5);
  const int mw_rel = MW ? (int)(((uint32_t)wave - mw_rot) & (uint32_t)(WAVES - 1)) : 0;
  float *const mwx = lds_wg + WAVES * 8 * STRIDE;
#ifndef ASDR_MW_STRAGGLER_PRIO
#define ASDR_MW_STRAGGLER_PRIO 0
#endif
  int *const mw_prog = reinterpret_cast<int *>(lds_wg + WAVES * 8 * STRIDE + 8 * WAVES * 16 + 260);
  int *const mw_flags = mw_prog + 4;
  constexpr bool PIPE_AGC = MW && WAVES == 4 && (MW_SHARE & 7) == 7 && (ASDR_MW_AGC_PIPELINED != 0) && (ASDR_AGC_LEAN != 0) && (ASDR_MW_OWN_STORES != 0) && ABL_ON(ABL_AGC) && ABL_ON(ABL_AF) && ABL_ON(ABL_NB);
  if constexpr (PIPE_AGC) { if (threadIdx.x < 3) mw_flags[1 + threadIdx.x] = 0; }
  if constexpr (MW && ASDR_MW_STRAGGLER_PRIO != 0) { if ((threadIdx.x & 63) == 0) mw_prog[wave] = 0; }
  auto mw_straggler = [&](int point) {
    if constexpr (MW && ASDR_MW_STRAGGLER_PRIO != 0) {
      if ((threadIdx.x & 63) == 0) mw_prog[wave] = point;
      const int4 pr = *reinterpret_cast<const int4 *>(mw_prog);
      const int behind = (pr.x < point) + (pr.y < point) + (pr.z < point) + (pr.w < point);
      const bool last = __builtin_amdgcn_readfirstlane(behind) == 0;
      if (last) __builtin_amdgcn_s_setprio(ASDR_MW_STRAGGLER_PRIO); else __builtin_amdgcn_s_setprio(0);
    }
  };
  constexpr int MWX = 16;
  auto mw_channel = [&](int q) -> int { const int sidx = (int)blockIdx.x * (8 * WAVES) + q; return (sidx < a.n_sched) ? a.direct_ch0 + sidx : a.n_channels; };
  const int wave_g = STREAM ? (int)blockIdx.x % a.stream_waves : (int)blockIdx.x * WAVES + wave;
  float *const lds = lds_wg + wave * 8 * STRIDE;
  const int lane = threadIdx.x & 63, c8 = lane >> 3, s8_ = lane & 7;
#ifndef ASDR_MW_SINE_LDS
#define ASDR_MW_SINE_LDS 0
#endif
  constexpr bool MW_SINE = MW && (ASDR_MW_SINE_LDS != 0);
  constexpr bool MW_SINE_LAZY = MW_SINE && (ASDR_MW_SINE_LDS == 2) && (MW_SHARE & 2) != 0 && WAVES == 4;
  constexpr bool SINE_LDS = HAS_SAM || (MW_SINE && !MW_SINE_LAZY);
  constexpr bool SINE_LDS_PC = HAS_SAM || MW_SINE;
  float *const sine_tab = HAS_SAM ? lds_wg + WAVES * 8 * STRIDE : (MW_SINE ? lds_wg + WAVES * 8 * STRIDE + 8 * WAVES * 16 : nullptr);
  float *const sine = SINE_LDS ? sine_tab : nullptr;
  int *const mw_sflag = reinterpret_cast<int *>(lds_wg + WAVES * 8 * STRIDE + 8 * WAVES * 16 + 260) + 8;
  if (HAS_SAM) for (int i = lane; i < ASDR_SINE_TABLE_LEN; i += 64) sine_tab[i] = c_sine[i];
  if (MW_SINE && !MW_SINE_LAZY) { for (int i = (int)threadIdx.x; i < ASDR_SINE_TABLE_LEN; i += 64 * WAVES) sine_tab[i] = c_sine[i]; __syncthreads(); }

  int4 slot = make_int4(a.n_channels, 0, 0, 0);
  const bool mw_pad = MW && (wave_g * 8 >= a.n_sched);
  if (UNIFORM && a.direct_ch0 >= 0) slot = make_int4(mw_pad ? a.n_channels : a.direct_ch0 + wave_g * 8 + c8, (int)a.direct_mode, (int)a.direct_flags, (int)((a.direct_lo & 0xFFu) | (wave_g == 0 ? a.lo_writer_bit : 0u)));
  else if (WAVES == 1 || wave_g * 8 < a.n_sched) slot = *reinterpret_cast<const int4 *>(a.sched + wave_g * 8 + c8);
  else { const ChanParams *pd = a.params + a.n_channels; slot.y = (int)pd->mode; slot.z = (int)pd->flags; }
  const int ch_ = slot.x;
  const bool valid = (UNIFORM && !mw_pad) || (ch_ < a.n_channels);
  const int loff_ = c8 * STRIDE;
#define P (*Pp)
  const ChainConsts K = a.k;

  const uint32_t mode = UNIFORM ? (uint32_t)__builtin_amdgcn_readfirstlane(slot.y) : (uint32_t)slot.y;
  const uint32_t pflags = UNIFORM ? (uint32_t)__builtin_amdgcn_readfirstlane(slot.z) : (uint32_t)slot.z;
  const uint32_t lo_slot = UNIFORM ? (uint32_t)__builtin_amdgcn_readfirstlane(slot.w) : 0u;
  const bool is_ssb = DO2 && ((mode == ASDR_USBmode) || (mode == ASDR_LSBmode) || (mode == ASDR_CW_USBmode) ||
                              (mode == ASDR_CW_LSBmode) || (mode == ASDR_WSPRmode));
#ifndef ASDR_MW_NO_AM
#define ASDR_MW_NO_AM 0
#endif
  const bool is_am = !C16 && !(MW && ASDR_MW_NO_AM) && (mode == ASDR_AMmode), is_sam = (HAS_SAM || ROLE >= 4) && (mode == ASDR_SAMmode);
  const bool sub_q = (mode == ASDR_USBmode) || (mode == ASDR_CW_USBmode) || (mode == ASDR_WSPRmode);
  const bool nb_en = DO1 && (pflags & ASDR_F_NB_EN), af_en = DO3 && (pflags & ASDR_F_AF_EN), agc_en = DO3 && (pflags & ASDR_F_AGC_EN);
  if constexpr (MW_SINE_LAZY) {
    if (!(ABL_ON(ABL_NB) && __any(nb_en))) {
      for (int i = (int)threadIdx.x; i < ASDR_SINE_TABLE_LEN; i += 64 * WAVES) sine_tab[i] = c_sine[i];
      __syncthreads();
    }
  }
  const bool als_en = HAS_ALS && (pflags & ASDR_F_ALS_EN);
  const bool muted = pflags & ASDR_F_MUTED;
  const float two_pi = K.two_pi_f;
  WAVE_SYNC();
  uint32_t seen_in = 0u, seen_free = 0u, seen_lo = 0u, sig_pending = 0u;
  float carry_phase = 0.0f, carry_fsh = 0.0f;
  uint32_t carry_hs = 0u;
#ifndef ASDR_STREAM_PREFETCH_IN
#define ASDR_STREAM_PREFETCH_IN 1
#endif
  int4 pf_in[4] = {make_int4(0, 0, 0, 0), make_int4(0, 0, 0, 0), make_int4(0, 0, 0, 0), make_int4(0, 0, 0, 0)};
#ifndef ASDR_STREAM_R2_ONE_TRIP
#define ASDR_STREAM_R2_ONE_TRIP 1
#endif
#ifndef ASDR_STREAM_R2_PREFETCH
#define ASDR_STREAM_R2_PREFETCH 1
#endif
  constexpr bool R2_ONE_TRIP = (ROLE == 2) && (FIR_HELPERS == 3) && (ASDR_STREAM_R2_ONE_TRIP != 0);
  constexpr bool R2_PREFETCH = R2_ONE_TRIP && (ASDR_STREAM_R2_PREFETCH != 0);
  v4f r2n_key = (v4f){0.f, 0.f, 0.f, 0.f}, r2n_c4[4], r2n_s4[4], r2n_vi[4], r2n_vq[4];
  bool r2_pref = false;
  uint32_t r2_look_in = 0u, r2_look_lo = 0u;
#ifndef ASDR_STREAM_R1_CARRY
#define ASDR_STREAM_R1_CARRY 0
#endif
  float4 r1_if_s4 = make_float4(0.f, 0.f, 0.f, 0.f);
  float r1_if_cf[5] = {0.f, 0.f, 0.f, 0.f, 0.f}, r1_gain_i = 0.f, r1_gain_q = 0.f;
  uint32_t *const my_prog = STREAM ? a.stream_prog + (ROLE - 1) * a.stream_waves + wave_g : nullptr;

  constexpr bool ONEBLK = (!HAS_ALS || ASDR_ONEBLK_ALS) && (ONEBLK_ || (ROLE >= 4 && !LOOPED_ROLE && ASDR_ONEBLK_ROLES));
  constexpr bool UNIT_OK = (ASDR_UNIT_SCALE != 0) && ((ONEBLK && ROLE == 0) || ROLE == 1);
  static_assert(!C16 || (ONEBLK && UNIFORM && !HAS_ALS && !HAS_SAM && WAVES == 1 && ROLE == 0), "the 16-waves-per-CU form is the plain uniform one-block kernel");
#pragma unroll 1
  for (int blk = 0; blk < (ONEBLK ? 1 : a.n_blocks); ++blk) {
    int s8 = s8_; asm volatile("" : "+v"(s8));
    int loff = loff_; asm volatile("" : "+v"(loff));
    int ch = ch_; asm volatile("" : "+v"(ch));
    int lane_i = lane; asm volatile("" : "+v"(lane_i));
#ifdef ASDR_TIMELINE
    if (STREAM && a.taps != nullptr && wave_g == 0 && lane == 0) (reinterpret_cast<unsigned long long *>(a.taps) + 64 * (3 + ROLE) + 32 * (blk & 1))[16] = clock64();
#endif
    if (STREAM) {
      uint32_t *prog = a.stream_prog, *err = a.stream_err;
      const uint32_t b1 = (uint32_t)blk + 1u, freed = (blk >= ASDR_STREAM_DEPTH) ? (uint32_t)(blk - ASDR_STREAM_DEPTH + 1) : 0u;
      const bool need_in = (ROLE != 1) && seen_in < b1, need_free = (ROLE != 3) && seen_free < freed;
      if ((need_in || need_free) && sig_pending) { stream_signal(my_prog, sig_pending, lane); sig_pending = 0u; }
      if (need_in) { seen_in = stream_wait(prog + (ROLE - 2) * a.stream_waves + wave_g, b1, err, a.stream_spin_limit); if (seen_in == ASDR_STREAM_FAIL) break; }
      if (need_free) { seen_free = stream_wait(prog + ROLE * a.stream_waves + wave_g, freed, err, a.stream_spin_limit); if (seen_free == ASDR_STREAM_FAIL) break; }
    }
    const ChanParams *Pp = row_ptr(a.params, (uint32_t)ch * (uint32_t)sizeof(ChanParams));
    ChanSmall *S = row_ptr(a.small, (uint32_t)ch * (uint32_t)sizeof(ChanSmall));
    float *L = lds + loff;
    int *Li = reinterpret_cast<int *>(L);
    constexpr bool PLB = (ASDR_PIPE_BANK_SELECT != 0);
#define pl_st (PLB ? ((lane_i & 15) >> 2) : (s8 & 3))
#define pl_iq (PLB ? (lane_i & 1) : (s8 >> 2))
#define pl_c (PLB ? (2 * (lane_i >> 4) + ((lane_i >> 1) & 1)) : (lane_i >> 3))
#define pa_c (PLB ? (2 * (lane_i >> 4) + (lane_i & 1)) : (lane_i >> 3))
#define pa_real (PLB ? ((lane_i & 3) < 2) : ((lane_i & 7) < 4))
#if ASDR_PIPE_BANK_SELECT
#define PL_CH(c) (__builtin_amdgcn_ds_bpermute((c) << 5, ch))
#define Sp row_ptr(a.small, (uint32_t)PL_CH(pl_c) * (uint32_t)sizeof(ChanSmall))
#define Spa row_ptr(a.small, (uint32_t)PL_CH(pa_c) * (uint32_t)sizeof(ChanSmall))
#define Ppl row_ptr(a.params, (uint32_t)PL_CH(pl_c) * (uint32_t)sizeof(ChanParams))
#define Ppa row_ptr(a.params, (uint32_t)PL_CH(pa_c) * (uint32_t)sizeof(ChanParams))
#define Lp (lds + pl_c * STRIDE)
#define Lpa (lds + pa_c * STRIDE)
#else
#define PL_CH(c) ch
#define Sp S
#define Spa S
#define Ppl Pp
#define Ppa Pp
#define Lp L
#define Lpa L
#endif
    const bool af_en_pa = (PLB && !UNIFORM) ? (__builtin_amdgcn_ds_bpermute(pa_c << 5, af_en ? 1 : 0) != 0) : af_en;
    const int k0 = 16 * s8, kA = 8 * s8, kF = 4 * s8;
    const bool lead = (s8 == 0);
#ifdef ASDR_TIMELINE
    const int tl_wg = ((int)blockIdx.x == 0) ? 0 : (((int)blockIdx.x == 683) ? 1 : (((int)blockIdx.x == 1365) ? 2 : (((int)blockIdx.x == 2047) ? 3 : -1)));
    const int tl_slot = STREAM ? ((wave_g == 0) ? 2 * (3 + ROLE) + (blk & 1) : -1)
                               : (MW ? ((tl_wg < 0) ? -1 : 4 * tl_wg + wave)
                                     : ((wave_g == 0) ? 0 : ((wave_g == 2731) ? 1 : ((wave_g == 5461) ? 2 : ((wave_g == 8191) ? 3 : -1)))));
    unsigned long long *tl = reinterpret_cast<unsigned long long *>(a.taps) + 32 * (tl_slot < 0 ? 0 : tl_slot);
#define TL(i) do { if (a.taps != nullptr && tl_slot >= 0 && lane == 0) tl[i] = clock64(); } while (0)
    const bool tap_on = false;
    TL(0);
    if (MW && a.taps != nullptr && tl_slot >= 0 && lane == 0) { uint32_t hw; asm volatile("s_getreg_b32 %0, hwreg(HW_REG_HW_ID)" : "=s"(hw)); tl[29] = hw; }
#else
#define TL(i) do { } while (0)
    const bool tap_on = (a.taps != nullptr) && valid && (blk == a.n_blocks - 1);
#endif
    float *tap_base = tap_on ? a.taps + (size_t)ch * ASDR_N + kA : nullptr;
    const size_t tap_stride = (size_t)a.n_channels * ASDR_N;
#define TAP8(id, h, v) do { if (tap_on) store8(tap_base + (size_t)(id) * tap_stride + 64 * (h), v); } while (0)
#define TAP4(id, m, v) do { if (tap_on) store4(tap_base - kA + kF + (size_t)(id) * tap_stride + 32 * (m), v); } while (0)
#define TAP_ROW(id, rowoff) do { if (tap_on) { for (int h_ = 0; h_ < 2; ++h_) { float tv_[8]; load8(L + (rowoff) + kA + 64 * h_, tv_); \
                                  store8(tap_base + (size_t)(id) * tap_stride + 64 * h_, tv_); } } } while (0)

    uint32_t status = S->status;
    const uint32_t status_in = status;
    const bool mix_early = is_ssb || (DO2 && is_am);
    float mphase = 0.0f, minc = 0.0f, mphase_end = 0.0f;
    float fsh_raw = 0.0f;
    if (mix_early) {
      if (ROLE == 2 && blk > 0) { mphase = carry_phase; fsh_raw = carry_fsh; }
      else { mphase = is_ssb ? S->phase_ssb : S->phase_am; fsh_raw = P.freq_shift; }
    }
    const float nb_thr = P.nb_threshold;
    const uint32_t lo_e = (lo_slot & 0xFFu) ? (lo_slot & 0xFFu) - 1u : 0u;
    const bool lo_has = (ROLE == 2) || ((lo_slot & 0xFFu) != 0u);
    const LoEntry *lo_rd = (ROLE == 2) ? a.lo_ring + (blk % ASDR_LO_RING) : a.lo_cache + (a.lo_parity & 1u) * ASDR_LO_ENTRIES + lo_e;
    uint32_t lo_kp, lo_ki;
    float lo_end;
    v4f r2_c4[4], r2_s4[4], r2_vi[4], r2_vq[4];
    if (ROLE == 2) {
      v4f key;
      if (R2_PREFETCH && r2_pref) {
        key = r2n_key;
#pragma unroll
        for (int m = 0; m < 4; ++m) { r2_c4[m] = r2n_c4[m]; r2_s4[m] = r2n_s4[m]; r2_vi[m] = r2n_vi[m]; r2_vq[m] = r2n_vq[m]; }
        r2_pref = false;
      } else {
      if (seen_lo < (uint32_t)blk + 1u) { seen_lo = stream_wait(a.stream_prog + 3 * a.stream_waves, (uint32_t)blk + 1u, a.stream_err, a.stream_spin_limit); if (seen_lo == ASDR_STREAM_FAIL) break; }
      if (R2_ONE_TRIP) {
        const float *lp = lo_rd->c + 4 * s8_, *xp = a.xch_a + ((size_t)ch * ASDR_STREAM_DEPTH + (size_t)(blk % ASDR_STREAM_DEPTH)) * (2 * ASDR_N) + 4 * s8_;
        asm volatile("global_load_dwordx4 %0, %17, off sc1\n\t"
                     "global_load_dwordx4 %1, %18, off sc1\n\tglobal_load_dwordx4 %2, %18, off offset:128 sc1\n\tglobal_load_dwordx4 %3, %18, off offset:256 sc1\n\tglobal_load_dwordx4 %4, %18, off offset:384 sc1\n\t"
                     "global_load_dwordx4 %5, %18, off offset:512 sc1\n\tglobal_load_dwordx4 %6, %18, off offset:640 sc1\n\tglobal_load_dwordx4 %7, %18, off offset:768 sc1\n\tglobal_load_dwordx4 %8, %18, off offset:896 sc1\n\t"
                     "global_load_dwordx4 %9, %19, off sc1\n\tglobal_load_dwordx4 %10, %19, off offset:128 sc1\n\tglobal_load_dwordx4 %11, %19, off offset:256 sc1\n\tglobal_load_dwordx4 %12, %19, off offset:384 sc1\n\t"
                     "global_load_dwordx4 %13, %19, off offset:512 sc1\n\tglobal_load_dwordx4 %14, %19, off offset:640 sc1\n\tglobal_load_dwordx4 %15, %19, off offset:768 sc1\n\tglobal_load_dwordx4 %16, %19, off offset:896 sc1\n\t"
                     "s_waitcnt vmcnt(0)"
                     : "=&v"(key), "=&v"(r2_c4[0]), "=&v"(r2_c4[1]), "=&v"(r2_c4[2]), "=&v"(r2_c4[3]), "=&v"(r2_s4[0]), "=&v"(r2_s4[1]), "=&v"(r2_s4[2]), "=&v"(r2_s4[3]),
                       "=&v"(r2_vi[0]), "=&v"(r2_vi[1]), "=&v"(r2_vi[2]), "=&v"(r2_vi[3]), "=&v"(r2_vq[0]), "=&v"(r2_vq[1]), "=&v"(r2_vq[2]), "=&v"(r2_vq[3])
                     : "v"(lo_rd), "v"(lp), "v"(xp) : "memory");
      } else
      asm volatile("global_load_dwordx4 %0, %1, off sc1\n\ts_waitcnt vmcnt(0)" : "=&v"(key) : "v"(lo_rd) : "memory");
      }
      lo_kp = __float_as_uint(key[0]); lo_ki = __float_as_uint(key[1]); lo_end = key[2];
    } else {
      lo_kp = lo_rd->key_phase; lo_ki = lo_rd->key_inc; lo_end = lo_rd->phase_end;
    }
    const uint32_t ns = (a.nb_phase + (uint32_t)blk) % 3u;
    const uint32_t hs = (ROLE == 2 && blk > 0) ? carry_hs : (S->hil_slot & 1u);
    const uint32_t ns_mid = (ns + 1u) % 3u, ns_new = (ns + 2u) % 3u;
    float carrier_now = 0.0f;
    bool carrier_fresh = false;
    const size_t io = ((size_t)ch * a.in_stride + blk) * ASDR_N + kA;
    const size_t io_out = ((size_t)ch * a.out_stride + blk) * ASDR_N + kA;
    const bool nb_wave = ABL_ON(ABL_NB) && __any(nb_en);
    int16_t *hist = row_ptr(a.nb_hist, (uint32_t)ch * 1536u);
    uint32_t *mrow = reinterpret_cast<uint32_t *>(row_ptr(a.nb_mask, (uint32_t)ch * ASDR_NB_MASK_ROW + 4u * (uint32_t)s8));

    union Raw8 { int4 v; int16_t s[8]; };
    Raw8 ri[2], rq[2], roi[2], roq[2], rmi[2], rmq[2];
    ri[0].v = ri[1].v = rq[0].v = rq[1].v = make_int4(0, 0, 0, 0);
    roi[0].v = roi[1].v = roq[0].v = roq[1].v = rmi[0].v = rmi[1].v = rmq[0].v = rmq[1].v = make_int4(0, 0, 0, 0);
    uint32_t mkc[5] = {0x01010101u, 0x01010101u, 0x01010101u, 0x01010101u, 0x01010101u};
    float gain_i, gain_q;
    if (ROLE == 1 && ASDR_STREAM_R1_CARRY && blk > 0) { gain_i = r1_gain_i; gain_q = r1_gain_q; }
    else { gain_i = P.in_gain_i; gain_q = P.in_gain_q; if (ROLE == 1) { r1_gain_i = gain_i; r1_gain_q = gain_q; } }
    float g_oi = gain_i, g_oq = gain_q, g_mi = 0.0f, g_mq = 0.0f, nb_avg0 = 0.0f;
    uint32_t agc_hc_early = 0u, agc_hang_early = 0u;
    bool agc_piped = false;
    if (nb_wave && nb_en) {
      g_oi = S->nb_gain[ns][0]; g_oq = S->nb_gain[ns][1]; g_mi = S->nb_gain[ns_mid][0]; g_mq = S->nb_gain[ns_mid][1];
      nb_avg0 = S->nb_avg;
      if constexpr (PIPE_AGC) { agc_hc_early = S->agc_hang_counter; agc_hang_early = P.agc_hang_count; }
      const int4 *old4 = reinterpret_cast<const int4 *>(hist + ns * 256 + kA), *mid4 = reinterpret_cast<const int4 *>(hist + ns_mid * 256 + kA);
#if ASDR_NT_LOADS >= 2
      rmi[0].v = mid4[0]; rmi[1].v = mid4[8]; rmq[0].v = mid4[16]; rmq[1].v = mid4[24];
      roi[0].v = load_int4_nt(old4); roi[1].v = load_int4_nt(old4 + 8); roq[0].v = load_int4_nt(old4 + 16); roq[1].v = load_int4_nt(old4 + 24);
#else
      rmi[0].v = mid4[0]; rmi[1].v = mid4[8]; rmq[0].v = mid4[16]; rmq[1].v = mid4[24];
      roi[0].v = old4[0]; roi[1].v = old4[8]; roq[0].v = old4[16]; roq[1].v = old4[24];
#endif
#pragma unroll
      for (int r = 0; r < 5; ++r) mkc[r] = mrow[8 * r];
      if constexpr (C16) {
        const uint32_t all1 = (mkc[0] & mkc[1] & mkc[2] & mkc[3] & mkc[4]) == 0x01010101u && (mkc[0] | mkc[1] | mkc[2] | mkc[3] | mkc[4]) == 0x01010101u ? 0x01010101u : 0u;
#pragma unroll
        for (int r = 0; r < 5; ++r) mkc[r] = all1;
      }
    }
    if (DO1 && valid) {
      const int4 *pi = reinterpret_cast<const int4 *>(a.in_i + io);
      const int4 *pq = reinterpret_cast<const int4 *>(a.in_q + io);
      if constexpr (ROLE == 1 && ASDR_STREAM_PREFETCH_IN != 0) {
        if (blk == 0) { ri[0].v = load_int4_nt(pi); ri[1].v = load_int4_nt(pi + 8); rq[0].v = load_int4_nt(pq); rq[1].v = load_int4_nt(pq + 8); }
        else { ri[0].v = pf_in[0]; ri[1].v = pf_in[1]; rq[0].v = pf_in[2]; rq[1].v = pf_in[3]; }
      } else {
#if ASDR_NT_LOADS >= 1
      ri[0].v = load_int4_nt(pi); ri[1].v = load_int4_nt(pi + 8); rq[0].v = load_int4_nt(pq); rq[1].v = load_int4_nt(pq + 8);
#else
      ri[0].v = pi[0]; ri[1].v = pi[8]; rq[0].v = pq[0]; rq[1].v = pq[8];
#endif
      }
    }
    if (mix_early) minc = (is_ssb ? -fsh_raw : -K.if_center) * K.phase_inc_unit;
    bool ph_ready = false;
    bool lo_hit = false;
    if ((blk == 0 || ROLE == 2) && lo_has) lo_hit = __all(mix_early && __float_as_uint(mphase) == lo_kp && __float_as_uint(minc) == lo_ki);
    if (lo_hit && lead) { if (is_ssb) S->phase_ssb = lo_end; else S->phase_am = lo_end; }

    if (nb_wave) {
    } else if (DO1) {
      const bool unit_in = UNIT_OK && __all(gain_i == 1.0f && gain_q == 1.0f);
#pragma unroll
      for (int h = 0; h < 2; ++h) {
        float xi[8], xq[8];
        scale8(ri[h].s, (double)gain_i, xi, unit_in); scale8(rq[h].s, (double)gain_q, xq, unit_in);
        TAP8(ASDR_TAP_SCALED_I, h, xi); TAP8(ASDR_TAP_SCALED_Q, h, xq);
        store8(L + W0 + kA + 64 * h, xi); store8(L + W1 + kA + 64 * h, xq);
        SCHED_FENCE();
      }
    }

    float4 if_s4 = make_float4(0.f, 0.f, 0.f, 0.f);
    float if_cf[5] = {0.f, 0.f, 0.f, 0.f, 0.f};
    bool if_pre = false;
    auto load_if_rows_early = [&]() {
      if_s4 = *reinterpret_cast<const float4 *>(&Sp->if_state[pl_iq][4 * pl_st]);
      const float *cf = &c_bq_pool[Ppl->if_table][5 * pl_st];
#pragma unroll
      for (int z = 0; z < 5; ++z) if_cf[z] = cf[z];
      if_pre = true;
    };
    TL(1);
    if (nb_wave) {
      float vio[16], vqo[16], mgm[16], mgt[8];
      if (!nb_en) {
#pragma unroll
        for (int h = 0; h < 2; ++h) { roi[h].v = ri[h].v; roq[h].v = rq[h].v; }
      }
      const bool own_tail = (s8 >= 1);
      if (C16 && nb_en) {
        int4 *ni = reinterpret_cast<int4 *>(hist + ns_new * 256 + kA);
        store_int4_nt(ni, ri[0].v); store_int4_nt(ni + 8, ri[1].v); store_int4_nt(ni + 16, rq[0].v); store_int4_nt(ni + 24, rq[1].v);
        if (lead) { S->nb_gain[ns_new][0] = gain_i; S->nb_gain[ns_new][1] = gain_q; }
      }
      const bool unit_ring = UNIT_OK && __all(g_oi == 1.0f && g_oq == 1.0f && (!nb_en || (g_mi == 1.0f && g_mq == 1.0f)));
      auto env4 = [&](const float *pw4, float *mg4) {
        if (unit_ring) {
#pragma unroll
          for (int j = 0; j < 4; ++j) mg4[j] = fast_sqrt1_short(pw4[j]);
        } else {
#pragma unroll
          for (int j = 0; j < 4; ++j) mg4[j] = fast_sqrt1(pw4[j]);
        }
      };
      if constexpr (C16) {
        auto mid_piece = [&](int h) {
          float vim[8], vqm[8], bm8[8], pw[8];
          scale8(rmi[h].s, (double)g_mi, vim, unit_ring); scale8(rmq[h].s, (double)g_mq, vqm, unit_ring);
#pragma unroll
          for (int j = 0; j < 8; ++j) pw[j] = vim[j] * vim[j] + vqm[j] * vqm[j];
          env4(pw, mgm + 8 * h); env4(pw + 4, mgm + 8 * h + 4);
#pragma unroll
          for (int j = 0; j < 8; ++j) bm8[j] = K.nb_beta * mgm[8 * h + j];
          if (nb_en) store8(L + NB_B + 50 + kA + 64 * h, bm8);
// ... 195 lines not shown
        }
        if constexpr (MW_SINE_LAZY) {
          const uint32_t p1 = (uint32_t)__builtin_amdgcn_readfirstlane((int)__float_as_uint(mphase)), i1 = (uint32_t)__builtin_amdgcn_readfirstlane((int)__float_as_uint(minc));
          const bool differ = mix_early && !__all(__float_as_uint(mphase) == p1 && __float_as_uint(minc) == i1);
          if (lane_i == 0) mw_sflag[wave] = differ ? 1 : 0;
        }
        TL(17);
        __syncthreads();
        TL(18);
        if constexpr (MW_SINE_LAZY) {
          const int4 sf = *reinterpret_cast<const int4 *>(mw_sflag);
          if (__builtin_amdgcn_readfirstlane(sf.x | sf.y | sf.z | sf.w) != 0 && mw_rel != 0) {
#pragma unroll 1
            for (int i = (mw_rel - 1) * 64 + lane_i; i < ASDR_SINE_TABLE_LEN; i += 192) { sine_tab[i] = c_sine[i]; asm volatile("" ::: "memory"); }
          }
        }
        if (ASDR_MW_PRIO && mw_rel == 0) __builtin_amdgcn_s_setprio(ASDR_MW_PRIO);
        if (mw_rel == 0 && lane_i < 8 * WAVES) {
          const int q = lane_i;
          const float4 in4 = *reinterpret_cast<const float4 *>(mwx + MWX * q);
          const int fl = __float_as_int(in4.w);
          const bool any_phase = __any((fl & 1) != 0);
          const float pe = nb_chain(lds_wg + q * STRIDE, row_ptr(a.small, (uint32_t)mw_channel(q) * (uint32_t)sizeof(ChanSmall)), in4.x, in4.y, in4.z, any_phase, (fl & 2) != 0, nb_en, is_ssb);
          mwx[MWX * q + 4] = pe;
          if (ASDR_MW_OWN_STORES) { mwx[MWX * q] = nb_avg_end; mwx[MWX * q + 1] = __int_as_float(any_phase ? 1 : 0); }
        }
#ifndef ASDR_MW_PRIO_REL0_TAIL
#define ASDR_MW_PRIO_REL0_TAIL 0
#endif
        if (ASDR_MW_PRIO && mw_rel == 0) __builtin_amdgcn_s_setprio(ASDR_MW_PRIO_REL0_TAIL);
        TL(19);
        __syncthreads();
        TL(20);
        if constexpr (PIPE_AGC) {
          const int fl = __float_as_int(mwx[MWX * (lane_i & (8 * WAVES - 1)) + 7]);
          agc_piped = __all((fl & 1) != 0) && __any((fl & 2) != 0);
        }
        if (lead) {
          mphase_end = mwx[MWX * (wave * 8 + c8) + 4];
          if (ASDR_MW_OWN_STORES) {
            if (nb_en) S->nb_avg = mwx[MWX * (wave * 8 + c8)];
            if (mix_early && !lo_hit && __float_as_int(mwx[MWX * (wave * 8 + c8) + 1]) != 0) { if (is_ssb) S->phase_ssb = mphase_end; else S->phase_am = mphase_end; }
          }
        }
      } else {
        CHAIN_PRIO_ON();
        if (lead) mphase_end = nb_chain(L, S, nb_avg0, mphase, minc, chain_phase_own, mix_early && !lo_hit, nb_en, is_ssb);
        CHAIN_PRIO_OFF();
      }
      ph_ready = mix_early && !lo_hit;
      WAVE_SYNC();
      uint32_t fm = 0u, ft = 0u;
      if (nb_en) {
        const float thr = nb_thr;
#pragma unroll
        for (int h = 0; h < 2; ++h) {
          float av[8];
          load8(L + NB_B + 50 + kA + 64 * h, av);
#pragma unroll
          for (int j = 0; j < 8; ++j) fm = fm + fm + ((mgm[8 * h + j] > av[j] * thr) ? 1u : 0u);
        }
        if (own_tail) {
          float av[8];
          if (s8 >= 2) load8(L + kA - 12, av);
          else { const float4 t4 = *reinterpret_cast<const float4 *>(L); av[0] = av[1] = av[2] = av[3] = 0.0f; av[4] = t4.x; av[5] = t4.y; av[6] = t4.z; av[7] = t4.w; }
#pragma unroll
          for (int j = 0; j < 8; ++j) ft = ft + ft + (((64 + kA + j >= 78) && (mgt[j] > av[j] * thr)) ? 1u : 0u);
        }
      }
      TL(3);
      if (C16 && DO1 && ABL_ON(ABL_IF)) { load_if_rows_early(); }
      const unsigned long long det_bal = __ballot((fm | ft) != 0u);
      const bool ch_det = ((uint32_t)(det_bal >> (8 * c8)) & 0xFFu) != 0u;
      bool nb_quiet = !ch_det;
      if (nb_en && lead) status = (status & ~ASDR_S_NB_DETECTED) | (ch_det ? ASDR_S_NB_DETECTED : 0u);
#pragma unroll
      for (int r = 0; r < 5; ++r) nb_quiet = nb_quiet && (mkc[r] == 0x01010101u);
      if constexpr (C16) {
        if (__any(!nb_quiet) && nb_en) {
#pragma unroll
          for (int r = 0; r < 5; ++r) mkc[r] = mrow[8 * r];
        }
      }
#ifdef ASDR_NB_ALWAYS_SLOW
      const bool nb_slow = true;
#else
      const bool nb_slow = __any(!nb_quiet);
#endif
      if constexpr (C16) {
        asm volatile("" : "+v"(roi[0].v.x), "+v"(roi[1].v.x), "+v"(roq[0].v.x), "+v"(roq[1].v.x));
#pragma unroll
        for (int h = 0; h < 2; ++h) { scale8(roi[h].s, (double)g_oi, vio + 8 * h, unit_ring); scale8(roq[h].s, (double)g_oq, vqo + 8 * h, unit_ring); }
      }
      if (nb_slow) {
        const float mask_tab = c_mask_val[lane_i & 7];
        const uint32_t group4 = (uint32_t)(lane_i & 56) << 2;
        uint8_t *const mb = reinterpret_cast<uint8_t *>(Li + NB_MSKB);
        WAVE_SYNC();
        if (nb_en) {
          auto scan8 = [&](uint32_t v) {
            { const uint32_t t1 = (uint32_t)__builtin_amdgcn_update_dpp(0, (int)v, 0x111, 0xF, 0xF, true); v += (s8 >= 1) ? t1 : 0u; }
            { const uint32_t t2 = (uint32_t)__builtin_amdgcn_update_dpp(0, (int)v, 0x112, 0xF, 0xF, true); v += (s8 >= 2) ? t2 : 0u; }
            { const uint32_t t4 = (uint32_t)__builtin_amdgcn_update_dpp(0, (int)v, 0x114, 0xF, 0xF, true); v += (s8 >= 4) ? t4 : 0u; }
            return v;
          };
          const uint32_t cnt_t = (uint32_t)__builtin_popcount(ft), cnt_a = (uint32_t)__builtin_popcount(fm >> 8), cnt_b = (uint32_t)__builtin_popcount(fm & 0xFFu);
          const uint32_t inc_t = scan8(cnt_t), inc_a = scan8(cnt_a), inc_b = scan8(cnt_b);
// ... 382 lines not shown
        if (lo_hit) {
          if (RING_PREFETCH) {
#pragma unroll
            for (int j = 0; j < 4; ++j) { cc[j] = lo_c[4 * m + j]; sn[j] = lo_s[4 * m + j]; }
          } else { load4(lo_rd->c + kF + 32 * m, cc); load4(lo_rd->s + kF + 32 * m, sn); }
        } else if (mix_uni) {
          load4(lds + STRIDE + PH + kF + 32 * m, cc); load4(lds + 2 * STRIDE + PH + kF + 32 * m, sn);
        } else {
          float ph[4];
          load4(L + PH + kF + 32 * m, ph);
#ifndef ASDR_MIX_SERIAL_LOOKUPS
          sincos_batch<4, SINE_LDS_PC>(SINE_LDS_PC ? sine_tab : nullptr, ph, cc, sn, two_pi, SinIndexK{K.inv_two_pi_d, K.sin_index_scale_d}, K.half_pi_d);
#else
#pragma unroll
          for (int j = 0; j < 4; ++j) {
            cc[j] = cos_f32(sine, ph[j], two_pi, SinIndexK{K.inv_two_pi_d, K.sin_index_scale_d}, K.half_pi_d); sn[j] = sin_f32(sine, ph[j], two_pi, SinIndexK{K.inv_two_pi_d, K.sin_index_scale_d});
            if ((j & 1) == 1) SCHED_FENCE();
          }
#endif
        }
#pragma unroll
        for (int j = 0; j < 4; ++j) {
          mi[j] = vi[j] * cc[j] - vq[j] * sn[j];
          mq[j] = vq[j] * cc[j] + vi[j] * sn[j];
        }
        if (qn_direct) {
#pragma unroll
          for (int j = 0; j < 4; ++j) qn[4 * m + j] = mq[j];
        } else { store4(L + W0 + kF + 32 * m, mi); store4(L + W1 + kF + 32 * m, mq); }
#ifndef ASDR_TEMPORAL_RINGS
        if (is_ssb) store4_nt(hi_ring + hs * 128 + 32 * m, mi);
#else
        if (is_ssb) store4(hi_ring + hs * 128 + 32 * m, mi);
#endif
      }
    }

    float4 af_s4 = make_float4(0.f, 0.f, 0.f, 0.f);
    float af_cf[5] = {0.f, 0.f, 0.f, 0.f, 0.f};
    float agc_gain_in = 0.f, agc_old0 = 0.f, agc_carrier0 = 0.f;
    uint32_t agc_hc0 = 0u;
    int agc_tab_idx = 0;
    const bool mw_audio_duty = (MW_SHARE & 1) && (mw_rel == 1 || mw_rel == 2);
    const int mw_casc = PLB ? (4 * (lane_i >> 4) + (lane_i & 3)) : (lane_i >> 2);
    ChanSmall *mw_af_S = S;
    auto load_af_agc_state = [&]() {
    ChanSmall *const Saf = PLB ? Spa : S; const ChanParams *const Paf = PLB ? Ppa : Pp;
    if (ABL_ON(ABL_AF) && (((MW_SHARE & 1) != 0) ? af_en : af_en_pa)) {
      if constexpr ((MW_SHARE & 1) != 0) {
        if (mw_audio_duty) {
          const int chq = mw_channel(16 * (mw_rel - 1) + mw_casc);
          mw_af_S = row_ptr(a.small, (uint32_t)chq * (uint32_t)sizeof(ChanSmall));
          af_s4 = *reinterpret_cast<const float4 *>(&mw_af_S->af_state[4 * pl_st]);
          const float *cf = &c_bq_pool[row_ptr(a.params, (uint32_t)chq * (uint32_t)sizeof(ChanParams))->audio_table][5 * pl_st];
#pragma unroll
          for (int z = 0; z < 5; ++z) af_cf[z] = cf[z];
        }
      } else {
      af_s4 = *reinterpret_cast<const float4 *>(&Saf->af_state[4 * pl_st]);
      const float *cf = &c_bq_pool[Paf->audio_table][5 * pl_st];
#pragma unroll
      for (int z = 0; z < 5; ++z) af_cf[z] = cf[z];
      }
    }
    if (ABL_ON(ABL_AGC) && agc_en) {
      agc_gain_in = S->agc_gain; agc_old0 = S->agc_old_abs; agc_hc0 = S->agc_hang_counter; agc_carrier0 = S->am_carrier;
      agc_tab_idx = P.agc_table;
    }
    };
    if constexpr (!C16) load_af_agc_state();
    TL(7);
    if (__any(is_ssb)) {
      if (is_ssb && !qn_direct) {
#pragma unroll
        for (int m = 0; m < 4; ++m) load4(L + W1 + kF + 32 * m, qn + 4 * m);
      }
      WAVE_SYNC();
      if constexpr (C16) {
#pragma unroll
        for (int m = 0; m < 4; ++m) {
#pragma unroll
          for (int j = 0; j < 4; ++j) {
            const int k = kF + 32 * m + j;
            if (k >= 1) L[XP + k - 1] = hq_o[4 * m + j];
            L[XP + 127 + k] = hq_m[4 * m + j];
            if (k < 63) L[XP + 255 + k] = qn[4 * m + j];
          }
          store4_nt(hq_ring + hs * 128 + 32 * m, qn + 4 * m);
        }
        if (lead) S->hil_slot = hs ^ 1u;
        WAVE_SYNC();
        TL(8);
        v2f fa[4], fb[4];
#pragma unroll
        for (int e = 0; e < 4; ++e) { fa[e] = (v2f){0.0f, 0.0f}; fb[e] = (v2f){0.0f, 0.0f}; }
        if (ABL_ON(ABL_HIL)) hilbert_fir<0, 4, false>(L, 4 * s8, fa);
        WAVE_SYNC();
        {
          float t[32];
#pragma unroll
          for (int q = 0; q < 8; ++q) load4(L + XP + 64 + 32 * s8 + 4 * q, t + 4 * q);
          WAVE_SYNC();
#pragma unroll
          for (int q = 0; q < 8; ++q) store4(L + XP + 32 * s8 + 4 * q, t + 4 * q);
        }
#pragma unroll
        for (int m = 0; m < 4; ++m) {
// ... 13 lines not shown
        *reinterpret_cast<float4 *>(L + W1 + 64 + 8 * s8 + 4) = make_float4(fb[2][0], fb[2][1], fb[3][0], fb[3][1]);
        WAVE_SYNC();
      } else {
      if (is_ssb) {
        if (!RING_PREFETCH) {
#pragma unroll
          for (int m = 0; m < 4; ++m) {
            load4(hq_ring + hs * 128 + 32 * m, hq_o + 4 * m);
            load4(hq_ring + (hs ^ 1u) * 128 + 32 * m, hq_m + 4 * m);
          }
        }
#pragma unroll
        for (int m = 0; m < 4; ++m) {
#pragma unroll
          for (int j = 0; j < 4; ++j) {
            const int k = kF + 32 * m + j;
            if (k >= 1) L[XP + k - 1] = hq_o[4 * m + j];
            L[XP + 127 + k] = hq_m[4 * m + j];
          }
        }
#pragma unroll
        for (int m = 0; m < 4; ++m) {
#pragma unroll
          for (int j = 0; j < 4; ++j) L[XP + 255 + kF + 32 * m + j] = qn[4 * m + j];
#ifndef ASDR_TEMPORAL_RINGS
          store4_nt(hq_ring + hs * 128 + 32 * m, qn + 4 * m);
#else
          store4(hq_ring + hs * 128 + 32 * m, qn + 4 * m);
#endif
        }
        if (lead) S->hil_slot = hs ^ 1u;
        carry_hs = hs ^ 1u;
      }
      WAVE_SYNC();
      TL(8);
      mw_straggler(3);
      if constexpr (R2_PREFETCH) {
        const uint32_t b2 = (uint32_t)blk + 2u;
        if (blk + 1 < a.n_blocks && (seen_in < b2 || seen_lo < b2)) {
          const uint32_t ui = (uint32_t)__builtin_amdgcn_readfirstlane((int)r2_look_in), ul = (uint32_t)__builtin_amdgcn_readfirstlane((int)r2_look_lo);
          asm volatile("" ::: "memory");
          if (ui != ASDR_STREAM_FAIL && ui > seen_in) seen_in = ui;
          if (ul != ASDR_STREAM_FAIL && ul > seen_lo) seen_lo = ul;
        }
        if (blk + 1 < a.n_blocks && seen_in != ASDR_STREAM_FAIL && seen_lo != ASDR_STREAM_FAIL && seen_in >= b2 && seen_lo >= b2) {
          const LoEntry *ln = a.lo_ring + ((blk + 1) % ASDR_LO_RING);
          const float *lp = ln->c + kF, *xp = a.xch_a + ((size_t)ch * ASDR_STREAM_DEPTH + (size_t)((blk + 1) % ASDR_STREAM_DEPTH)) * (2 * ASDR_N) + kF;
          r2n_key = ld_sc1_v4(reinterpret_cast<const float *>(ln));
#pragma unroll
          for (int m = 0; m < 4; ++m) { r2n_c4[m] = ld_sc1_v4(lp + 32 * m); r2n_s4[m] = ld_sc1_v4(lp + ASDR_N + 32 * m); r2n_vi[m] = ld_sc1_v4(xp + 32 * m); r2n_vq[m] = ld_sc1_v4(xp + ASDR_N + 32 * m); }
          r2_pref = true;
        }
      }
      constexpr bool IDL_EARLY = (ROLE == 2);
      if (IDL_EARLY && is_ssb) {
#pragma unroll
        for (int m = 0; m < 4; ++m) load4(hi_ring + (hs ^ 1u) * 128 + 32 * m, idl + 4 * m);
      }
      constexpr int FIR_NE = (ROLE == 2) ? 8 / (FIR_HELPERS + 1) : 8;
      v2f acc2[FIR_NE];
#pragma unroll
      for (int e = 0; e < FIR_NE; ++e) acc2[e] = (v2f){0.0f, 0.0f};
      if (ROLE == 2) __syncthreads();
      if (ABL_ON(ABL_HIL) && is_ssb) hilbert_fir<0, FIR_NE>(L, k0 >> 1, acc2);
      if (ROLE == 2) __syncthreads(); else WAVE_SYNC();
      TL(9);
      if (!IDL_EARLY && is_ssb) {
#pragma unroll
        for (int m = 0; m < 4; ++m) {
#if ASDR_NT_LOADS >= 4
          load4_nt(hi_ring + (hs ^ 1u) * 128 + 32 * m, idl + 4 * m);
#else
          load4(hi_ring + (hs ^ 1u) * 128 + 32 * m, idl + 4 * m);
#endif
        }
      }
      if (is_ssb) {
#pragma unroll
        for (int e = 0; e < FIR_NE; e += 2) *reinterpret_cast<float4 *>(L + W1 + k0 + 2 * e) = make_float4(acc2[e][0], acc2[e][1], acc2[e + 1][0], acc2[e + 1][1]);
      }
      if (ROLE == 2) __syncthreads(); else WAVE_SYNC();
      }
      if (is_ssb) {
        const uint32_t sgn = sub_q ? 0x80000000u : 0u;
#pragma unroll
        for (int m = 0; m < 4; ++m) {
          float qh[4], au[4];
          load4(L + W1 + kF + 32 * m, qh);
#pragma unroll
          for (int j = 0; j < 4; ++j) au[j] = idl[4 * m + j] + __uint_as_float(__float_as_uint(qh[j]) ^ sgn);
          store4(L + W0 + kF + 32 * m, au);
          TAP4(ASDR_TAP_MIX_I, m, idl + 4 * m); TAP4(ASDR_TAP_MIX_Q, m, qh);
        }
      }
    }

    if (ABL_ON(ABL_ENV) && __any(do_env)) {
      WAVE_SYNC();
      {
        const int iq = pl_iq, st = pl_st;
        const bool do_env_p = PLB ? (__builtin_amdgcn_ds_bpermute(pl_c << 5, do_env ? 1 : 0) != 0) : do_env;
        float sv[4];
        ChanSmall *const Simg = Sp;
        const float4 s4 = *reinterpret_cast<const float4 *>(&Simg->img_state[iq][4 * st]);
        sv[0] = s4.x; sv[1] = s4.y; sv[2] = s4.z; sv[3] = s4.w;
        biquad_pipe<PIPE_PK>(Lp + (iq ? W1 : W0), do_env_p, st, &c_bq_pool[ASDR_TBL_AM_IMAGE][5 * st], sv);
        if (do_env_p) *reinterpret_cast<float4 *>(&Simg->img_state[iq][4 * st]) = make_float4(sv[0], sv[1], sv[2], sv[3]);
// ... 400 lines not shown
            *reinterpret_cast<float4 *>(mq + 8) = make_float4(agc_old0, __uint_as_float(agc_hc0), gain_in, agc_al_a);
            *reinterpret_cast<float4 *>(mq + 12) = make_float4(agc_be_a, agc_al_r, agc_be_r, __uint_as_float(agc_hang));
          }
        }
        TL(25);
        __syncthreads();
        TL(26);
        if (ASDR_MW_PRIO && mw_rel == 3) __builtin_amdgcn_s_setprio(ASDR_MW_PRIO);
        if (mw_rel == 3 && lane_i < 8 * WAVES) {
          const int q = lane_i;
          const bool active = (__float_as_int(mwx[MWX * q + 5]) == 0);
          float4 i0 = make_float4(0.f, 0.f, 0.f, 0.f), i1 = i0;
          if (ASDR_MW_OWN_STORES && active) { i0 = *reinterpret_cast<const float4 *>(mwx + MWX * q + 8); i1 = *reinterpret_cast<const float4 *>(mwx + MWX * q + 12); }
          const bool lean = LEAN_OK && !is_am && __all(!active || (__float_as_uint(i0.y) >= 128u && __float_as_uint(i1.w) >= 128u));
          if (q == 0) mw_flags[0] = lean ? 1 : 0;
          if (lean) {
            if (active) {
              float *Lc = lds_wg + q * STRIDE;
              float old_abs = i0.x;
              const float al_a = i0.w, be_a = i1.x;
              float x_[8];
              load8(Lc + AGC_GV, x_);
#pragma unroll 1
              for (int i2 = 0; i2 < ASDR_N; i2 += 16) {
                float xn_[8];
#pragma unroll
                for (int half = 0; half < 2; ++half) {
                  const int i = i2 + 8 * half;
                  float *x = half ? xn_ : x_, *xn = half ? x_ : xn_;
                  load8(Lc + AGC_GV + ((i + 8 < ASDR_N) ? i + 8 : i), xn);
                  float pb[8], ov[8];
#pragma unroll
                  for (int u = 0; u < 8; ++u) pb[u] = be_a * x[u];
#pragma unroll
                  for (int u = 0; u < 8; ++u) {
                    const float pa = al_a * old_abs;
                    const float v_new = pa + pb[u];
                    old_abs = (x[u] > old_abs) ? v_new : old_abs;
                    ov[u] = old_abs;
                  }
                  store8(Lc + AGC_GV + i, ov);
                }
              }
              mwx[MWX * q + 8] = old_abs;
            }
          } else
          if (active) {
            if (ASDR_MW_OWN_STORES) {
              mwx[MWX * q + 7] = agc_chain(std::true_type{}, lds_wg + q * STRIDE, nullptr, i0.x, __float_as_uint(i0.y), i0.z, i0.w, i1.x, i1.y, i1.z, __float_as_uint(i1.w), is_am, mwx[MWX * q + 6]);
              mwx[MWX * q + 8] = agc_old_end; mwx[MWX * q + 9] = __uint_as_float(agc_hc_end);
            } else {
            const int chq = mw_channel(q);
            ChanSmall *Sq = row_ptr(a.small, (uint32_t)chq * (uint32_t)sizeof(ChanSmall));
            const ChanParams *Pq = row_ptr(a.params, (uint32_t)chq * (uint32_t)sizeof(ChanParams));
            mwx[MWX * q + 7] = agc_chain(std::false_type{}, lds_wg + q * STRIDE, Sq, Sq->agc_old_abs, Sq->agc_hang_counter, Sq->agc_gain, Pq->agc_alpha_att, Pq->agc_beta_att,
                                       Pq->agc_alpha_rel, Pq->agc_beta_rel, Pq->agc_hang_count, is_am, mwx[MWX * q + 6]);
            }
          }
        }
        if (ASDR_MW_PRIO && mw_rel == 3) __builtin_amdgcn_s_setprio(0);
        TL(27);
        __syncthreads();
        TL(28);
        } else { TL(25); TL(26); TL(27); TL(28); }
        const bool lean_done = LEAN_OK && (agc_piped || __builtin_amdgcn_readfirstlane(mw_flags[0]) != 0);
        if (lean_done && !agc_quiet && agc_en) {
          agc_lean_finish(lead ? mwx[MWX * (wave * 8 + c8) + 8] : 0.0f);
        } else
        if (!agc_quiet && lead) {
          const float *mq = mwx + MWX * (wave * 8 + c8);
          const float g_end = mq[7]; status = (status & ~ASDR_S_AGC_ACTIVE) | (((double)g_end < 0.99) ? ASDR_S_AGC_ACTIVE : 0u);
          if (ASDR_MW_OWN_STORES && agc_en) { S->agc_old_abs = mq[8]; S->agc_hang_counter = __float_as_uint(mq[9]); S->agc_gain = g_end; }
        }
      } else {
#ifndef ASDR_AGC_LEAN1
#define ASDR_AGC_LEAN1 1
#endif
        constexpr bool LEAN1_OK = (ASDR_AGC_LEAN1 != 0) && !C16 && !(ROLE == 0 && WAVES == 1 && !ONEBLK_ && !HAS_ALS && !HAS_SAM && UNIFORM);
        const bool lean1 = LEAN1_OK && !agc_quiet && __all(!(agc_en && lead) || (!is_am && agc_hc0 >= 128u && agc_hang >= 128u));
        if (!agc_quiet) CHAIN_PRIO_ON();
        if (lean1) {
          float old_abs = agc_old0;
          if (agc_en && lead) {
            const float al_a = agc_al_a, be_a = agc_be_a;
            float x_[8];
            load8(L + AGC_GV, x_);
#pragma unroll 1
            for (int i2 = 0; i2 < ASDR_N; i2 += 16) {
              float xn_[8];
#pragma unroll
              for (int half = 0; half < 2; ++half) {
                const int i = i2 + 8 * half;
                float *x = half ? xn_ : x_, *xn = half ? x_ : xn_;
                load8(L + AGC_GV + ((i + 8 < ASDR_N) ? i + 8 : i), xn);
                float pb[8], ov[8];
#pragma unroll
                for (int u = 0; u < 8; ++u) pb[u] = be_a * x[u];
#pragma unroll
                for (int u = 0; u < 8; ++u) {
                  const float pa = al_a * old_abs;
                  const float v_new = pa + pb[u];
                  old_abs = (x[u] > old_abs) ? v_new : old_abs;
                  ov[u] = old_abs;
                }
                store8(L + AGC_GV + i, ov);
              }
            }
// ... 71 lines not shown
          float tx[16], tw[16], tn[16];
#pragma unroll
          for (int m = 0; m < 4; ++m) {
            if (m >= M0) load4(gx_prev + 32 * m, tx + 4 * m);
            if (m < NW) load4(gw + 32 * m, tw + 4 * m);
            load4(L + W0 + kF + 32 * m, tn + 4 * m);
          }
#pragma unroll
          for (int m = 0; m < 4; ++m) {
            if (m >= M0) store4(L + XB + kF + 32 * m, tx + 4 * m);
            store4(L + XB + 128 + kF + 32 * m, tn + 4 * m); store4(gx + 32 * m, tn + 4 * m);
            if (m < NW) {
              float *we = L + AW + ((kF + 32 * m) >> 1);
              *reinterpret_cast<float2 *>(we) = make_float2(tw[4 * m], tw[4 * m + 2]);
              *reinterpret_cast<float2 *>(we + WH) = make_float2(tw[4 * m + 1], tw[4 * m + 3]);
            }
          }
        }
        WAVE_SYNC();
        als_compute<COMPACT, XB, AW, WH, SCR, ALS_OUT>(L, als_en, adaptive, notch, M, D, lam, s8, k0);
        WAVE_SYNC();
        uint32_t flags_again = pflags;
        if constexpr (UNIFORM) asm volatile("" : "+s"(flags_again)); else asm volatile("" : "+v"(flags_again));
        if (flags_again & ASDR_F_ALS_EN) {
#pragma unroll
          for (int m = 0; m < NW; ++m) {
            const float *we = L + AW + ((kF + 32 * m) >> 1);
            const float2 e2 = *reinterpret_cast<const float2 *>(we), o2 = *reinterpret_cast<const float2 *>(we + WH);
            const float t[4] = {e2.x, o2.x, e2.y, o2.y};
            store4(gw + 32 * m, t);
          }
        }
      }
    }
    if (TO_ALS && valid) {
      float *gx = row_ptr(a.als_x, (uint32_t)ch * 1024u + ((a.als_phase + (uint32_t)blk) & 1u) * 512u + 4u * (uint32_t)kF);
      float *gs = (a.als_stage != nullptr) ? row_ptr(a.als_stage, (uint32_t)ch * (uint32_t)(ASDR_ALS_STAGE_SLOTS * 512) + ((a.als_stage_cur + (uint32_t)blk) % ASDR_ALS_STAGE_SLOTS) * 512u + 4u * (uint32_t)kF) : nullptr;
#pragma unroll
      for (int m = 0; m < 4; ++m) { float t[4]; load4(L + W0 + kF + 32 * m, t); store4(gx + 32 * m, t); if (gs != nullptr) store4(gs + 32 * m, t); }
    }
    if (DO3 && !TO_ALS && valid && a.audio_prev != nullptr) {
      float *ap = row_ptr(a.audio_prev, (uint32_t)ch * 512u + 4u * (uint32_t)kF);
#pragma unroll
      for (int m = 0; m < 4; ++m) {
        float t[4]; load4(L + W0 + kF + 32 * m, t);
#ifndef ASDR_PREV_TEMPORAL
        store4_nt(ap + 32 * m, t);
#else
        store4(ap + 32 * m, t);
#endif
      }
    }
    {
      const float og = P.output_gain;
      union { int4 v; int16_t s[8]; } ro[2];
#pragma unroll
      for (int h = 0; h < 2; ++h) {
        float au[8];
        load8(L + W0 + kA + 64 * h, au);
        TAP8(ASDR_TAP_ALS, h, au);
#pragma unroll
        for (int j = 0; j < 8; ++j) {
          const int v = (int)((double)(og * au[j]) * 32767.0);
          ro[h].s[j] = muted ? (int16_t)0 : (int16_t)v;
        }
        SCHED_FENCE();
      }
      if (DO3 && !TO_ALS && valid) {
        int4 *po = reinterpret_cast<int4 *>(a.out + io_out);
#ifndef ASDR_TEMPORAL_OUT
        store_int4_nt(po, ro[0].v); store_int4_nt(po + 8, ro[1].v);
#else
        po[0] = ro[0].v; po[8] = ro[1].v;
#endif
      }
    }
    if (POST_ROLE) store_status_bits(ASDR_S_AGC_ACTIVE);
    else if (!STREAM) { if (lead) S->status = status; }
    else { store_status_bits(ASDR_S_AGC_ACTIVE); sig_pending = (uint32_t)blk + 1u; }
    WAVE_SYNC();
    if (a.lo_write && ROLE != 2 && (lo_slot & a.lo_writer_bit) && (lo_slot & 0xFFu) != 0u && blk == a.n_blocks - 1 && mix_uni && __all(mix_early)) {
      uint32_t lo_wi = ((a.lo_parity & 1u) ^ 1u) * ASDR_LO_ENTRIES + lo_e;
      asm volatile("" : "+v"(lo_wi));
      LoEntry *lo_wr = a.lo_cache + lo_wi;
      const float start = lo_hit ? lo_end : __uint_as_float((uint32_t)__builtin_amdgcn_readfirstlane((int)__float_as_uint(mphase_end)));
      const float inc = __uint_as_float(inc_first);
      if (lane == 0) {
        float phase = start;
        const bool up = !(inc < 0.0f);
        const float wrapv = up ? -two_pi : two_pi, lim = up ? two_pi : 0.0f;
        const uint32_t flip = up ? 0u : 0x80000000u;
#pragma unroll 1
        for (int i = 0; i < ASDR_N; i += 8) {
          float pv[8];
#pragma unroll
          for (int u = 0; u < 8; ++u) {
            pv[u] = phase;
            const float t = phase + inc, tw = t + wrapv;
            phase = (__uint_as_float(__float_as_uint(t) ^ flip) > lim) ? tw : t;
          }
          store8(lds + (C16 ? 0 : PH) + i, pv);
        }
        lo_wr->key_phase = __float_as_uint(start); lo_wr->key_inc = __float_as_uint(inc); lo_wr->phase_end = phase;
      }
      WAVE_SYNC();
      const float2 p2 = *reinterpret_cast<const float2 *>(lds + (C16 ? 0 : PH) + 2 * lane_i);
      const float ph2[2] = {p2.x, p2.y};
      float c2[2], s2[2];
      sincos_batch<2, SINE_LDS>(sine, ph2, c2, s2, two_pi, SinIndexK{K.inv_two_pi_d, K.sin_index_scale_d}, K.half_pi_d);
      *reinterpret_cast<float2 *>(lo_wr->c + 2 * lane_i) = make_float2(c2[0], c2[1]);
      *reinterpret_cast<float2 *>(lo_wr->s + 2 * lane_i) = make_float2(s2[0], s2[1]);
      WAVE_SYNC();
    }
    TL(15);
  }
  if (STREAM && sig_pending) stream_signal(my_prog, sig_pending, lane);
#undef P
#undef PL_CH
#undef Sp
#undef Spa
#undef Ppl
#undef Ppa
#undef Lp
#undef Lpa
#undef pl_st
#undef pl_iq
#undef pl_c
#undef pa_c
#undef pa_real
}

#define ASDR_KERNEL(name, lds_floats, bounds, stride, als, sam, uni, waves)                                     \
  extern "C" __global__ __launch_bounds__(64 * waves, bounds) void name(UpdateArgs a) {                         \
    __shared__ __attribute__((aligned(16))) float lds[lds_floats];                                              \
    asdr_update_body<stride, als, sam, uni, waves>(a, lds);                                                     \
  }
ASDR_KERNEL(asdr_update_kernel, 8 * ASDR_STRIDE, ASDR_WAVES_PER_EU, ASDR_STRIDE, false, false, true, 1)
ASDR_KERNEL(asdr_update_kernel_mixed, 8 * ASDR_STRIDE, ASDR_WAVES_PER_EU, ASDR_STRIDE, false, false, false, 1)
extern "C" __global__ __launch_bounds__(64, ASDR_WAVES_PER_EU) void asdr_update_kernel_one(UpdateArgs a) {
  __shared__ __attribute__((aligned(16))) float lds[8 * ASDR_STRIDE];
  asdr_update_body<ASDR_STRIDE, false, false, true, 1, 0, true>(a, lds);
}
#define ASDR_C16_STRIDE 320
extern "C" __global__ __launch_bounds__(64, 4) void asdr_update_kernel_c16(UpdateArgs a) {
  __shared__ __attribute__((aligned(16))) float lds[8 * ASDR_C16_STRIDE];
  asdr_update_body<ASDR_C16_STRIDE, false, false, true, 1, 0, true>(a, lds);
}
#define ASDR_MW_WAVES 4
extern "C" __global__ __launch_bounds__(64 * ASDR_MW_WAVES, ASDR_WAVES_PER_EU) void asdr_update_kernel_mw(UpdateArgs a) {
  __shared__ __attribute__((aligned(16))) float lds[ASDR_MW_WAVES * 8 * ASDR_STRIDE + ASDR_MW_WAVES * 8 * 16 + 260 + 12];
  asdr_update_body<ASDR_STRIDE, false, false, true, ASDR_MW_WAVES, 0, true>(a, lds);
}
ASDR_KERNEL(asdr_update_kernel_sam, ASDR_SAM_WAVES * 8 * ASDR_STRIDE + 260, ASDR_WAVES_PER_EU, ASDR_STRIDE, false, true, false, ASDR_SAM_WAVES)
#ifndef ASDR_ALS_WAVES_PER_EU
#define ASDR_ALS_WAVES_PER_EU 3
#endif
#ifndef ASDR_ALS_LDS_PAD
#define ASDR_ALS_LDS_PAD 0
#endif
ASDR_KERNEL(asdr_update_kernel_als, 8 * 516 + 260 + ASDR_ALS_LDS_PAD, ASDR_ALS_WAVES_PER_EU, 516, true, true, true, 1)
ASDR_KERNEL(asdr_update_kernel_als_mixed, 8 * 516 + 260 + ASDR_ALS_LDS_PAD, ASDR_ALS_WAVES_PER_EU, 516, true, true, false, 1)
ASDR_KERNEL(asdr_update_kernel_als_small, 8 * ASDR_ALS_STRIDE, ASDR_WAVES_PER_EU, ASDR_ALS_STRIDE, true, false, true, 1)
ASDR_KERNEL(asdr_update_kernel_als_small_mixed, 8 * ASDR_ALS_STRIDE, ASDR_WAVES_PER_EU, ASDR_ALS_STRIDE, true, false, false, 1)
extern "C" __global__ __launch_bounds__(64, ASDR_WAVES_PER_EU) void asdr_update_kernel_als_small_one(UpdateArgs a) {
  __shared__ __attribute__((aligned(16))) float lds[8 * ASDR_ALS_STRIDE];
  asdr_update_body<ASDR_ALS_STRIDE, true, false, true, 1, 0, true>(a, lds);
}

extern "C" __global__ __launch_bounds__(64, ASDR_WAVES_PER_EU) void asdr_sam_pre_kernel(UpdateArgs a) {
  __shared__ __attribute__((aligned(16))) float lds[8 * ASDR_STRIDE];
  asdr_update_body<ASDR_STRIDE, false, false, false, 1, 4>(a, lds);
}
extern "C" __global__ __launch_bounds__(64, ASDR_WAVES_PER_EU) void asdr_sam_post_kernel(UpdateArgs a) {
  __shared__ __attribute__((aligned(16))) float lds[8 * ASDR_STRIDE];
  asdr_update_body<ASDR_STRIDE, false, false, false, 1, 5>(a, lds);
}
#ifndef ASDR_PRE_STRIDE
#define ASDR_PRE_STRIDE 260
#endif
extern "C" __global__ __launch_bounds__(64, 4) void asdr_sam_pre_kernel_uniform(UpdateArgs a) {
  __shared__ __attribute__((aligned(16))) float lds[8 * ASDR_PRE_STRIDE];
  asdr_update_body<ASDR_PRE_STRIDE, false, false, true, 1, 4>(a, lds);
}
#ifndef ASDR_POST_BOUNDS
#define ASDR_POST_BOUNDS ASDR_WAVES_PER_EU
#endif
extern "C" __global__ __launch_bounds__(64, ASDR_POST_BOUNDS) void asdr_sam_post_kernel_uniform(UpdateArgs a) {
  __shared__ __attribute__((aligned(16))) float lds[8 * ASDR_STRIDE];
  asdr_update_body<ASDR_STRIDE, false, false, true, 1, 5>(a, lds);
}
extern "C" __global__ __launch_bounds__(64, 2) void asdr_sam_pre_loop_kernel_uniform(UpdateArgs a) {
  __shared__ __attribute__((aligned(16))) float lds[8 * ASDR_STRIDE];
  asdr_update_body<ASDR_STRIDE, false, false, true, 1, 8>(a, lds);
}
extern "C" __global__ __launch_bounds__(64, 2) void asdr_sam_post_loop_kernel_uniform(UpdateArgs a) {
  __shared__ __attribute__((aligned(16))) float lds[8 * ASDR_STRIDE];
  asdr_update_body<ASDR_STRIDE, false, false, true, 1, 9>(a, lds);
}
extern "C" __global__ __launch_bounds__(64, 2) void asdr_als_back_loop_kernel(UpdateArgs a) {
  __shared__ __attribute__((aligned(16))) float lds[8 * ASDR_STRIDE];
  asdr_update_body<ASDR_STRIDE, false, false, true, 1, 10>(a, lds);
}
extern "C" __global__ __launch_bounds__(64, ASDR_WAVES_PER_EU) void asdr_sam_post_als_kernel(UpdateArgs a) {
  __shared__ __attribute__((aligned(16))) float lds[8 * ASDR_ALS_STRIDE];
// ... 219 lines not shown
  else if (role == 1) asdr_update_body<ASDR_STRIDE, false, false, true, 1, 2>(a, lds);
  else asdr_update_body<ASDR_STRIDE, false, false, true, 1, 3>(a, lds);
}

extern "C" __global__ __launch_bounds__(256, 1) void asdr_stream_kernel_h3(UpdateArgs a) {
  __shared__ __attribute__((aligned(16))) float lds[8 * ASDR_STRIDE];
  __shared__ __attribute__((aligned(16))) float lo_scratch[ASDR_N];
  const int role = (int)blockIdx.x / a.stream_waves;
  const int hw = (int)threadIdx.x >> 6;
  if (hw != 0) {
    if (role == 1) {
      if (hw == 1) asdr_stream_fir_helper<ASDR_STRIDE, 2, 2>(a, lds);
      else if (hw == 2) asdr_stream_fir_helper<ASDR_STRIDE, 4, 2>(a, lds);
      else asdr_stream_fir_helper<ASDR_STRIDE, 6, 2>(a, lds);
    } else if (blockIdx.x == 0 && hw == 1) asdr_stream_lo_role(a, lo_scratch);
    return;
  }
  if (role == 0) asdr_update_body<ASDR_STRIDE, false, false, true, 1, 1>(a, lds);
  else if (role == 1) asdr_update_body<ASDR_STRIDE, false, false, true, 1, 2, false, 3>(a, lds);
  else asdr_update_body<ASDR_STRIDE, false, false, true, 1, 3>(a, lds);
}

static const char *const k_kernel_names[] = {
  "asdr_als_back_loop_kernel",
  "asdr_als_kernel",
  "asdr_als_pre_kernel",
  "asdr_als_pre_loop_kernel",
  "asdr_als_stage_seed_kernel",
  "asdr_reset_kernel",
  "asdr_sam_pll_kernel",
  "asdr_sam_post_als_kernel",
  "asdr_sam_post_als_kernel_uniform",
  "asdr_sam_post_kernel",
  "asdr_sam_post_kernel_uniform",
  "asdr_sam_post_loop_kernel_uniform",
  "asdr_sam_pre_kernel",
  "asdr_sam_pre_kernel_uniform",
  "asdr_sam_pre_loop_kernel_uniform",
  "asdr_spin_kernel",
  "asdr_stream_ack_kernel",
  "asdr_stream_kernel",
  "asdr_stream_kernel_h3",
  "asdr_stream_restore_kernel",
  "asdr_stream_snapshot_kernel",
  "asdr_update_kernel",
  "asdr_update_kernel_als",
  "asdr_update_kernel_als_mixed",
  "asdr_update_kernel_als_small",
  "asdr_update_kernel_als_small_mixed",
  "asdr_update_kernel_als_small_one",
  "asdr_update_kernel_c16",
  "asdr_update_kernel_mixed",
  "asdr_update_kernel_mw",
  "asdr_update_kernel_one",
  "asdr_update_kernel_sam"
};
#define ASDR_N_KERNEL_NAMES ((int)(sizeof k_kernel_names / sizeof k_kernel_names[0]))
static unsigned long long g_kernel_launches[ASDR_N_KERNEL_NAMES];
static inline int kernel_name_index(const char *name) {
  for (int i = 0; i < ASDR_N_KERNEL_NAMES; ++i)
    if (strcmp(k_kernel_names[i], name) == 0) return i;
  return -1;
}
static inline void count_launch(int i) { if (i >= 0) __atomic_fetch_add(&g_kernel_launches[i], 1ull, __ATOMIC_RELAXED); }
#define ASDR_LAUNCH(kernel, ...) do { static const int site_index_ = kernel_name_index(#kernel); count_launch(site_index_); hipLaunchKernelGGL(kernel, __VA_ARGS__); } while (0)
extern "C" int asdr_kernels_count(void) { return ASDR_N_KERNEL_NAMES; }
extern "C" const char *asdr_kernels_name(int i) { return (i >= 0 && i < ASDR_N_KERNEL_NAMES) ? k_kernel_names[i] : nullptr; }
extern "C" unsigned long long asdr_kernels_launches(int i) { return (i >= 0 && i < ASDR_N_KERNEL_NAMES) ? __atomic_load_n(&g_kernel_launches[i], __ATOMIC_RELAXED) : 0ull; }
extern "C" void asdr_kernels_launches_reset(void) { for (int i = 0; i < ASDR_N_KERNEL_NAMES; ++i) __atomic_store_n(&g_kernel_launches[i], 0ull, __ATOMIC_RELAXED); }

extern "C" int asdr_launch_stream(const UpdateArgs *a, hipStream_t stream, int fir_helpers) {
  if (a->stream_waves <= 0) return 0;
  if (fir_helpers == 3) ASDR_LAUNCH(asdr_stream_kernel_h3, dim3(3 * a->stream_waves), dim3(256), 0, stream, *a);
  else ASDR_LAUNCH(asdr_stream_kernel, dim3(3 * a->stream_waves), dim3(128), 0, stream, *a);
  return hipGetLastError() == hipSuccess ? 0 : -1;
}
extern "C" int asdr_stream_capacity(int device, int *compute_units, int fir_helpers) {
  int per_cu = 0;
  hipDeviceProp_t prop;
  if (hipGetDeviceProperties(&prop, device) != hipSuccess) return -1;
  if ((fir_helpers == 3 ? hipOccupancyMaxActiveBlocksPerMultiprocessor(&per_cu, asdr_stream_kernel_h3, 256, 0)
                        : hipOccupancyMaxActiveBlocksPerMultiprocessor(&per_cu, asdr_stream_kernel, 128, 0)) != hipSuccess) return -1;
  if (compute_units) *compute_units = prop.multiProcessorCount;
  return per_cu * prop.multiProcessorCount;
}

template <bool RESTORE>
__device__ __forceinline__ void stream_snapshot_body(const UpdateArgs &a, uint4 *snap) {
  if (RESTORE && *a.stream_err == 0u) return;
  const int t = threadIdx.x;
  for (int j = 0; j < 8; ++j) {
    const int slot = (int)blockIdx.x * 8 + j;
    if (slot >= a.n_sched) return;
    const int ch = (a.direct_ch0 >= 0) ? a.direct_ch0 + slot : a.sched[slot].ch;
    if (ch >= a.n_channels) continue;
    uint4 *dst = snap + (size_t)slot * (ASDR_SNAP_BYTES / 16);
    for (int p = t; p < ASDR_SNAP_BYTES / 16; p += 256) {
      uint4 *row; int q = p;
      if (q < 28) row = reinterpret_cast<uint4 *>(a.small + ch);
      else if ((q -= 28) < 96) row = reinterpret_cast<uint4 *>(a.nb_hist + (size_t)ch * 768);
      else if ((q -= 96) < ASDR_NB_MASK_ROW / 16) row = reinterpret_cast<uint4 *>(a.nb_mask + (size_t)ch * ASDR_NB_MASK_ROW);
      else if ((q -= ASDR_NB_MASK_ROW / 16) < 64) row = reinterpret_cast<uint4 *>(a.hil_q + (size_t)ch * 256);
      else if ((q -= 64) < 64) row = reinterpret_cast<uint4 *>(a.hil_i + (size_t)ch * 256);
      else { q -= 64; row = a.audio_prev ? reinterpret_cast<uint4 *>(a.audio_prev + (size_t)ch * 128) : nullptr; }
      if (row == nullptr) continue;
      if (RESTORE) row[q] = dst[p]; else dst[p] = row[q];
// ... 32 lines not shown
    a.hil_q[(size_t)ch * 256 + t] = 0.0f; a.hil_q[(size_t)ch * 256 + 128 + t] = 0.0f;
    if (a.audio_prev != nullptr) a.audio_prev[(size_t)ch * 128 + t] = 0.0f;
  }
  __syncthreads();
  if (all && t == 0) { S->nb_avg = 10.0f; S->status = ASDR_S_AGC_ACTIVE; }
  if (all || (r & ASDR_R_IF)) { if (t < 32) (&S->if_state[0][0])[t] = 0.0f; }
  if (all || (r & ASDR_R_IMG)) { if (t < 32) (&S->img_state[0][0])[t] = 0.0f; }
  if (all || (r & ASDR_R_AF)) { if (t < 16) S->af_state[t] = 0.0f; }
  if (all || (r & ASDR_R_NB)) {
    for (int i = t; i < 768; i += 128) a.nb_hist[(size_t)ch * 768 + i] = 0;
    for (int i = t; i < ASDR_NB_MASK_ROW; i += 128) a.nb_mask[(size_t)ch * ASDR_NB_MASK_ROW + i] = 1;
    if (t < 6) (&S->nb_gain[0][0])[t] = 0.0f;
  }
  if (all || (r & ASDR_R_ALS)) {
    a.als_x[(size_t)ch * 256 + t] = 0.0f; a.als_x[(size_t)ch * 256 + 128 + t] = 0.0f;
    a.als_w[(size_t)ch * 128 + t] = 0.0f;
  }
}

extern "C" int asdr_launch_update(const UpdateArgs *a, int variant, int uniform, hipStream_t stream) {
  const int n_waves = a->n_sched / 8;
  if (n_waves <= 0) return 0;
  if (variant == ASDR_KERNEL_ALS || (variant == ASDR_KERNEL_SAM_ALS && a->xch_sam == nullptr)) { if (uniform) ASDR_LAUNCH(asdr_update_kernel_als, dim3(n_waves), dim3(64), 0, stream, *a); else ASDR_LAUNCH(asdr_update_kernel_als_mixed, dim3(n_waves), dim3(64), 0, stream, *a); }
  else if (variant == ASDR_KERNEL_ALS_SMALL && uniform == 2) {
    ASDR_LAUNCH(asdr_als_pre_kernel, dim3(n_waves), dim3(64), 0, stream, *a);
    ASDR_LAUNCH(asdr_als_kernel, dim3(n_waves), dim3(64), 0, stream, *a);
  }
  else if (variant == ASDR_KERNEL_ALS_SMALL) { if (uniform && ASDR_ONEBLK && ASDR_ONEBLK_ALS && a->n_blocks == 1 && a->run_if == nullptr) ASDR_LAUNCH(asdr_update_kernel_als_small_one, dim3(n_waves), dim3(64), 0, stream, *a); else if (uniform) ASDR_LAUNCH(asdr_update_kernel_als_small, dim3(n_waves), dim3(64), 0, stream, *a); else ASDR_LAUNCH(asdr_update_kernel_als_small_mixed, dim3(n_waves), dim3(64), 0, stream, *a); }
  else if ((variant == ASDR_KERNEL_SAM || variant == ASDR_KERNEL_SAM_ALS) && a->xch_sam != nullptr) {
    if (uniform) ASDR_LAUNCH(asdr_sam_pre_kernel_uniform, dim3(n_waves), dim3(64), 0, stream, *a);
    else ASDR_LAUNCH(asdr_sam_pre_kernel, dim3(n_waves), dim3(64), 0, stream, *a);
    ASDR_LAUNCH(asdr_sam_pll_kernel, dim3((a->n_sched + ASDR_PLL_LANES - 1) / ASDR_PLL_LANES), dim3(64), 0, stream, *a);
    if (variant == ASDR_KERNEL_SAM_ALS) {
      if (uniform) ASDR_LAUNCH(asdr_sam_post_als_kernel_uniform, dim3(n_waves), dim3(64), 0, stream, *a);
      else ASDR_LAUNCH(asdr_sam_post_als_kernel, dim3(n_waves), dim3(64), 0, stream, *a);
    } else {
      if (uniform) ASDR_LAUNCH(asdr_sam_post_kernel_uniform, dim3(n_waves), dim3(64), 0, stream, *a);
      else ASDR_LAUNCH(asdr_sam_post_kernel, dim3(n_waves), dim3(64), 0, stream, *a);
    }
  }
  else if (variant == ASDR_KERNEL_SAM) ASDR_LAUNCH(asdr_update_kernel_sam, dim3((n_waves + ASDR_SAM_WAVES - 1) / ASDR_SAM_WAVES), dim3(64 * ASDR_SAM_WAVES), 0, stream, *a);
  else {
    static int mw_on = -1, mw_min = ASDR_MW_MIN_WAVES, c16_on = ASDR_C16, c16_min = ASDR_C16_MIN_WAVES, c16_pad = 0;
    if (mw_on < 0) {
      const char *e = getenv("ASDR_MW"); mw_on = e ? atoi(e) : ASDR_MW; const char *m = getenv("ASDR_MW_MIN_WAVES"); if (m) mw_min = atoi(m);
      const char *c = getenv("ASDR_C16"); if (c) c16_on = atoi(c); const char *cm = getenv("ASDR_C16_MIN_WAVES"); if (cm) c16_min = atoi(cm);
      const char *cp = getenv("ASDR_C16_PAD"); if (cp) c16_pad = atoi(cp);
    }
    const uint32_t dm = a->direct_mode;
    const bool ssb_class = dm == ASDR_USBmode || dm == ASDR_LSBmode || dm == ASDR_CW_USBmode || dm == ASDR_CW_LSBmode || dm == ASDR_WSPRmode;
    if (uniform && c16_on && a->n_blocks == 1 && a->run_if == nullptr && a->direct_ch0 >= 0 && a->taps == nullptr && ssb_class && n_waves >= c16_min)
      ASDR_LAUNCH(asdr_update_kernel_c16, dim3(n_waves), dim3(64), (size_t)c16_pad, stream, *a);
    else
    if (uniform && mw_on && a->n_blocks == 1 && a->run_if == nullptr && a->direct_ch0 >= 0 && n_waves >= mw_min)
      ASDR_LAUNCH(asdr_update_kernel_mw, dim3((n_waves + ASDR_MW_WAVES - 1) / ASDR_MW_WAVES), dim3(64 * ASDR_MW_WAVES), 0, stream, *a);
    else
    if (uniform && ASDR_ONEBLK && a->n_blocks == 1 && a->run_if == nullptr) ASDR_LAUNCH(asdr_update_kernel_one, dim3(n_waves), dim3(64), 0, stream, *a);
    else if (uniform) ASDR_LAUNCH(asdr_update_kernel, dim3(n_waves), dim3(64), 0, stream, *a);
    else ASDR_LAUNCH(asdr_update_kernel_mixed, dim3(n_waves), dim3(64), 0, stream, *a);
  }
  return hipGetLastError() == hipSuccess ? 0 : -1;
}

extern "C" __global__ void asdr_als_stage_seed_kernel(UpdateArgs a, int ch0, int n) {
  const int c = (int)blockIdx.x, t = (int)threadIdx.x;
  if (c >= n) return;
  const size_t ch = (size_t)(ch0 + c);
  a.als_stage[ch * (ASDR_ALS_STAGE_SLOTS * ASDR_N) + a.als_stage_prev * ASDR_N + t] = a.als_x[ch * (2 * ASDR_N) + ((a.als_phase & 1u) ^ 1u) * ASDR_N + t];
}
extern "C" int asdr_launch_als_role(const UpdateArgs *a, int role, hipStream_t stream) {
  const int n_waves = a->n_sched / 8;
  if (n_waves <= 0) return 0;
  if (role == 2) ASDR_LAUNCH(asdr_sam_pre_loop_kernel_uniform, dim3(n_waves), dim3(64), 0, stream, *a);
  else if (role == 3) ASDR_LAUNCH(asdr_als_back_loop_kernel, dim3(n_waves), dim3(64), 0, stream, *a);
  else if (role == 0 && a->n_blocks > 1) ASDR_LAUNCH(asdr_als_pre_loop_kernel, dim3(n_waves), dim3(64), 0, stream, *a);
  else if (role == 0) ASDR_LAUNCH(asdr_als_pre_kernel, dim3(n_waves), dim3(64), 0, stream, *a);
  else ASDR_LAUNCH(asdr_als_kernel, dim3(n_waves), dim3(64), 0, stream, *a);
  return hipGetLastError() == hipSuccess ? 0 : -1;
}
extern "C" int asdr_launch_als_stage_seed(const UpdateArgs *a, int ch0, int n, hipStream_t stream) {
  if (n <= 0) return 0;
  ASDR_LAUNCH(asdr_als_stage_seed_kernel, dim3(n), dim3(ASDR_N), 0, stream, *a, ch0, n);
  return hipGetLastError() == hipSuccess ? 0 : -1;
}

extern "C" int asdr_launch_sam_role(const UpdateArgs *a, int variant, int uniform, int role, hipStream_t stream) {
  const int n_waves = a->n_sched / 8;
  if (n_waves <= 0) return 0;
  if (a->n_blocks > 1 || a->sam_sets > 1u) {
    if (!uniform || variant != ASDR_KERNEL_SAM) return -1;
    if (role == 0) ASDR_LAUNCH(asdr_sam_pre_loop_kernel_uniform, dim3(n_waves), dim3(64), 0, stream, *a);
    else if (role == 1) ASDR_LAUNCH(asdr_sam_pll_kernel, dim3((a->n_sched + ASDR_PLL_LANES - 1) / ASDR_PLL_LANES), dim3(64), 0, stream, *a);
    else ASDR_LAUNCH(asdr_sam_post_loop_kernel_uniform, dim3(n_waves), dim3(64), 0, stream, *a);
    return hipGetLastError() == hipSuccess ? 0 : -1;
  }
  if (role == 0) {
    if (uniform) ASDR_LAUNCH(asdr_sam_pre_kernel_uniform, dim3(n_waves), dim3(64), 0, stream, *a);
    else ASDR_LAUNCH(asdr_sam_pre_kernel, dim3(n_waves), dim3(64), 0, stream, *a);
  } else if (role == 1) {
    ASDR_LAUNCH(asdr_sam_pll_kernel, dim3((a->n_sched + ASDR_PLL_LANES - 1) / ASDR_PLL_LANES), dim3(64), 0, stream, *a);
  } else if (variant == ASDR_KERNEL_SAM_ALS) {
    if (uniform) ASDR_LAUNCH(asdr_sam_post_als_kernel_uniform, dim3(n_waves), dim3(64), 0, stream, *a);
    else ASDR_LAUNCH(asdr_sam_post_als_kernel, dim3(n_waves), dim3(64), 0, stream, *a);
  } else {
    if (uniform) ASDR_LAUNCH(asdr_sam_post_kernel_uniform, dim3(n_waves), dim3(64), 0, stream, *a);
    else ASDR_LAUNCH(asdr_sam_post_kernel, dim3(n_waves), dim3(64), 0, stream, *a);
// ... 18 lines not shown
```

### include/asdr.h

```cpp
#ifndef ASDR_H_
#define ASDR_H_

#include <stddef.h>
#include <stdint.h>

#ifdef __cplusplus
extern "C" {
#endif

#define ASDR_BLOCK_SAMPLES 128
#define ASDR_ALL (-1)
#define ASDR_NO_DEVICE (-1)

enum { ASDR_LSBmode = 0, ASDR_USBmode = 1, ASDR_CW_LSBmode = 2, ASDR_CW_USBmode = 3, ASDR_AMmode = 4,
       ASDR_SAMmode = 5, ASDR_WSPRmode = 6 };
enum { ASDR_audioAM = 0, ASDR_audioCW = 1, ASDR_audioWSPR = 2, ASDR_audio2100 = 3, ASDR_audio2300 = 4,
       ASDR_audio2500 = 5, ASDR_audio2700 = 6, ASDR_audio2900 = 7, ASDR_audio3100 = 8, ASDR_audio3300 = 9,
       ASDR_audioBypass = 10 };
enum { ASDR_AGCoff = 0, ASDR_AGCfast = 1, ASDR_AGCmedium = 2, ASDR_AGCslow = 3 };

typedef struct asdr_batch asdr_batch_t;

asdr_batch_t *asdr_create(int n_channels, int device);
void asdr_destroy(asdr_batch_t *b);
// ... 74 lines not shown
int asdr_ALSfilterIsNotch(asdr_batch_t *b, int ch);
int asdr_ALSfilterIsPeak(asdr_batch_t *b, int ch);
int asdr_ALSfilterIsAdaptive(asdr_batch_t *b, int ch);

void asdr_enableAGC(asdr_batch_t *b, int ch);
void asdr_disableAGC(asdr_batch_t *b, int ch);
int asdr_AGCisEnabled(asdr_batch_t *b, int ch);
int asdr_AGCisActive(asdr_batch_t *b, int ch);
void asdr_setAGCthreshold(asdr_batch_t *b, int ch, float db);
void asdr_setAGCslope(asdr_batch_t *b, int ch, float slope);
void asdr_setAGCmode(asdr_batch_t *b, int ch, int mode);
void asdr_setAGCkneeWidth(asdr_batch_t *b, int ch, float db);
void asdr_setAGCattackTime(asdr_batch_t *b, int ch, float ms);
void asdr_setAGCreleaseTime(asdr_batch_t *b, int ch, float ms);
void asdr_setAGChangTime(asdr_batch_t *b, int ch, float ms);
void asdr_setAGCstaticGain(asdr_batch_t *b, int ch, float gain);
float asdr_getAGCthreshold(asdr_batch_t *b, int ch);
float asdr_getAGCslope(asdr_batch_t *b, int ch);
float asdr_getAGCkneeWidth(asdr_batch_t *b, int ch);
float asdr_getAGCattack(asdr_batch_t *b, int ch);
float asdr_getAGCrelease(asdr_batch_t *b, int ch);
float asdr_getAAGalphaAttack(asdr_batch_t *b, int ch);
float asdr_getAGCbetaAttack(asdr_batch_t *b, int ch);
float asdr_getAGCalphaRelease(asdr_batch_t *b, int ch);
float asdr_getAGCbetaRelease(asdr_batch_t *b, int ch);
float asdr_getAGClookup(asdr_batch_t *b, int ch, int i);
float asdr_getAGCstaticGain(asdr_batch_t *b, int ch);
float asdr_getAMcarrierLevel(asdr_batch_t *b, int ch);

void asdr_enableNoiseBlanker(asdr_batch_t *b, int ch);
void asdr_disableNoiseBlanker(asdr_batch_t *b, int ch);
void asdr_setNoiseBlankerThreshold(asdr_batch_t *b, int ch, float ratio);
void asdr_setNoiseBlankerThresholdDb(asdr_batch_t *b, int ch, float db);
int asdr_NoiseBlankerisEnabled(asdr_batch_t *b, int ch);
int asdr_NoiseBlankerDetection(asdr_batch_t *b, int ch);

float asdr_getSAMfrequency(asdr_batch_t *b, int ch);
int asdr_getSAMphaseLockStatus(asdr_batch_t *b, int ch);

int asdr_read_status(asdr_batch_t *b, int32_t *agc_active, int32_t *nb_detected, int32_t *sam_locked,
                     float *sam_frequency, float *am_carrier);
enum { ASDR_TAP_SCALED_I = 0, ASDR_TAP_SCALED_Q, ASDR_TAP_NB_I, ASDR_TAP_NB_Q, ASDR_TAP_IF_I, ASDR_TAP_IF_Q,
       ASDR_TAP_MIX_I, ASDR_TAP_MIX_Q, ASDR_TAP_DEMOD, ASDR_TAP_AUDIO_FILT, ASDR_TAP_AGC, ASDR_TAP_ALS,
       ASDR_N_TAPS };
int asdr_enable_taps(asdr_batch_t *b, int on);
int asdr_read_taps(asdr_batch_t *b, float *dst );
int asdr_set_launch_timing(asdr_batch_t *b, int on);
float asdr_last_kernel_ms(asdr_batch_t *b);
int asdr_region_timing_begin(asdr_batch_t *b, void *stream);
int asdr_region_timing_end(asdr_batch_t *b, float *ms_total, long *n_calls);
int asdr_kernel_timing_begin(asdr_batch_t *b, int max_launches);
int asdr_kernel_timing_end(asdr_batch_t *b, float *ms, int cap);
int asdr_control_plane_flush(asdr_batch_t *b, long long stats[4]);
unsigned int asdr_get_chain_constants(asdr_batch_t *b, int ch, float out[12]);
int asdr_set_exact_unknown_mode(asdr_batch_t *b, int on);
int asdr_get_exact_unknown_mode(asdr_batch_t *b);
long asdr_stream_pipeline_launches(asdr_batch_t *b);
long asdr_stream_pipeline_recoveries(asdr_batch_t *b);
int asdr_set_stream_fir_helpers(asdr_batch_t *b, int mode);
long asdr_stream_pipeline_h3_calls(asdr_batch_t *b);
long asdr_stream_pipeline_alloc_failures(asdr_batch_t *b);
long asdr_stream_pipeline_headroom_refusals(asdr_batch_t *b);
int asdr_stream_pipeline_max_groups(asdr_batch_t *b);
int asdr_set_stream_pipeline(asdr_batch_t *b, int on);
int asdr_set_launch_split(asdr_batch_t *b, int pieces, int min_waves);
int asdr_set_sam_launch_form(asdr_batch_t *b, int fused, int split_min_channels);
int asdr_set_als_launch_form(asdr_batch_t *b, int split_min_channels);
int asdr_debug_set_stream_spin_limit(asdr_batch_t *b, unsigned int polls);
int asdr_debug_set_stream_max_groups(asdr_batch_t *b, int groups);
int asdr_schedule_layout(asdr_batch_t *b, int out[8]);
const char *asdr_version(void);
int asdr_kernels_count(void);
const char *asdr_kernels_name(int i);
unsigned long long asdr_kernels_launches(int i);
void asdr_kernels_launches_reset(void);

#ifdef __cplusplus
}
#endif
#endif
```

Baseline: 83790.

## Pass uniform channel parameters by kernel argument for uniform multi-wave groups

The host now tracks whether every channel in a uniform direct-launch group has identical parameter rows, updating that state incrementally as rows change. When they match, the parameter row is copied into the kernel arguments and a new mw_u kernel variant reads parameters from the argument block instead of loading per-channel rows from global memory. It also switches on early idle-ring loads in that variant. The cost is larger launch arguments, extra host-side comparisons, and another kernel specialization.

Result: faster. 85370 (median of 6 runs) (+1.9%).

```diff
diff --git a/audiosdr_amd/binding.py b/audiosdr_amd/binding.py
--- a/audiosdr_amd/binding.py
+++ b/audiosdr_amd/binding.py
@@ -46,7 +46,7 @@
 
 EXPORTS = (["asdr_create", "asdr_destroy", "asdr_last_error", "asdr_n_channels", "asdr_update", "asdr_update_device",
             "asdr_synchronize", "asdr_setDemodMode", "asdr_getDemodMode", "asdr_setALSfilterParams", "asdr_getAGClookup",
-            "asdr_read_status", "asdr_control_plane_flush", "asdr_get_chain_constants", "asdr_stream_pipeline_launches", "asdr_schedule_layout", "asdr_set_exact_unknown_mode", "asdr_get_exact_unknown_mode", "asdr_stream_pipeline_recoveries", "asdr_stream_pipeline_max_groups", "asdr_set_stream_fir_helpers", "asdr_stream_pipeline_h3_calls", "asdr_set_stream_pipeline", "asdr_set_sam_launch_form", "asdr_set_als_launch_form", "asdr_debug_set_stream_spin_limit", "asdr_debug_set_stream_max_groups", "asdr_enable_taps", "asdr_read_taps", "asdr_last_kernel_ms", "asdr_version",
+            "asdr_read_status", "asdr_control_plane_flush", "asdr_params_uniform_groups", "asdr_get_chain_constants", "asdr_stream_pipeline_launches", "asdr_schedule_layout", "asdr_set_exact_unknown_mode", "asdr_get_exact_unknown_mode", "asdr_stream_pipeline_recoveries", "asdr_stream_pipeline_max_groups", "asdr_set_stream_fir_helpers", "asdr_stream_pipeline_h3_calls", "asdr_set_stream_pipeline", "asdr_set_sam_launch_form", "asdr_set_als_launch_form", "asdr_debug_set_stream_spin_limit", "asdr_debug_set_stream_max_groups", "asdr_enable_taps", "asdr_read_taps", "asdr_last_kernel_ms", "asdr_version",
             "asdr_kernel_timing_begin", "asdr_kernel_timing_end", "asdr_set_launch_timing", "asdr_region_timing_begin", "asdr_region_timing_end", "asdr_update_device_strided", "asdr_capture_open",
             "asdr_capture_close", "asdr_capture_capacity", "asdr_capture_position", "asdr_capture_rewind",
             "asdr_capture_device_ptr", "asdr_capture_update_device", "asdr_capture_read",
@@ -140,6 +140,8 @@
         L.asdr_get_chain_constants.argtypes = [vp, _i, C.POINTER(C.c_float)]; L.asdr_get_chain_constants.restype = C.c_uint
     if path is None or hasattr(L, "asdr_control_plane_flush"):
         L.asdr_control_plane_flush.argtypes = [vp, C.POINTER(C.c_longlong)]; L.asdr_control_plane_flush.restype = _i
+    if path is None or hasattr(L, "asdr_params_uniform_groups"):
+        L.asdr_params_uniform_groups.argtypes = [vp, C.POINTER(C.c_long)]; L.asdr_params_uniform_groups.restype = _i
     L.asdr_enable_taps.argtypes = [vp, _i]; L.asdr_enable_taps.restype = _i
     L.asdr_read_taps.argtypes = [vp, fp]; L.asdr_read_taps.restype = _i
     L.asdr_kernel_timing_begin.argtypes = [vp, _i]; L.asdr_kernel_timing_begin.restype = _i
@@ -358,6 +360,13 @@
         return {"rows_refilled": int(st[0]), "schedule_rebuilt": bool(st[1]), "waves_plain": int(st[2]) & 0x1FFFFF,
                 "waves_sam": (int(st[2]) >> 21) & 0x1FFFFF, "waves_als": (int(st[2]) >> 42) & 0x1FFFFF, "agc_tables_alive": int(st[3])}
 
+    def params_uniform_groups(self):
+        rows = C.c_long(0)
+        g = int(self._L.asdr_params_uniform_groups(self._h, C.byref(rows)))
+        if g < 0:
+            self._chk(g)
+        return g, int(rows.value)
+
     def last_kernel_ms(self):
         return float(self._L.asdr_last_kernel_ms(self._h))
 
diff --git a/audiosdr_amd/csrc/asdr_device.h b/audiosdr_amd/csrc/asdr_device.h
--- a/audiosdr_amd/csrc/asdr_device.h
+++ b/audiosdr_amd/csrc/asdr_device.h
@@ -135,6 +135,9 @@
   uint32_t als_stage_cur, als_stage_prev;
   LoEntry *lo_ring;
   ChainConsts k;
+  ChanParams uni;
+  uint32_t uni_valid;
+  uint32_t pad_uni_;
 } UpdateArgs;
 #define ASDR_ALS_STAGE_SLOTS 32
 #define ASDR_ALS_CHUNK 8
diff --git a/audiosdr_amd/csrc/asdr_host.cpp b/audiosdr_amd/csrc/asdr_host.cpp
--- a/audiosdr_amd/csrc/asdr_host.cpp
+++ b/audiosdr_amd/csrc/asdr_host.cpp
@@ -194,6 +194,11 @@
   int kind_first[ASDR_KERNEL_KINDS] = {}, kind_slots[ASDR_KERNEL_KINDS] = {}, kind_uniform_slots[ASDR_KERNEL_KINDS] = {};
   int left_first = 0, left_slots = 0, left_kind = ASDR_KERNEL_PLAIN;
   bool kind_direct[ASDR_KERNEL_KINDS] = {};
+  bool kind_puni[ASDR_KERNEL_KINDS] = {}, puni_recheck[ASDR_KERNEL_KINDS] = {};
+  long puni_diff[ASDR_KERNEL_KINDS] = {};
+  std::vector<uint8_t> puni_differs;
+  long stat_puni_rows_compared = 0;
+  bool uniform_params = true;
   long stat_rows_refilled = 0, stat_sched_rebuilds = 0, stat_bulk_uploads = 0;
   int stat_lo_groups_without_entry = 0;
   ChanParams *d_params = nullptr;
@@ -432,6 +437,34 @@
   if (b->dirty.size() > (size_t)b->n / 8 + 64) { b->all_dirty = true; }
 }
 
+inline bool params_rows_equal(const ChanParams &x, const ChanParams &y) {
+  return memcmp(&x, &y, offsetof(ChanParams, reset)) == 0 &&
+         memcmp(&x.if_table, &y.if_table, offsetof(ChanParams, pad_) - offsetof(ChanParams, if_table)) == 0;
+}
+void puni_pass(asdr_batch *b, int k) {
+  b->puni_recheck[k] = false; b->puni_diff[k] = 0; b->kind_puni[k] = false;
+  if (!b->kind_direct[k]) return;
+  const int ch0 = b->sched[b->kind_first[k]].ch, nu = b->kind_uniform_slots[k];
+  const ChanParams &r = b->hp[ch0];
+  long diff = 0;
+  for (int c = ch0; c < ch0 + nu; c++) { const uint8_t d = params_rows_equal(b->hp[c], r) ? 0 : 1; b->puni_differs[c] = d; diff += d; }
+  b->stat_puni_rows_compared += nu;
+  b->puni_diff[k] = diff; b->kind_puni[k] = (diff == 0);
+}
+void puni_row_changed(asdr_batch *b, int c) {
+  for (int k = 0; k < ASDR_KERNEL_KINDS; k++) {
+    if (!b->kind_direct[k] || b->puni_recheck[k]) continue;
+    const int ch0 = b->sched[b->kind_first[k]].ch;
+    if (c < ch0 || c >= ch0 + b->kind_uniform_slots[k]) continue;
+    if (c == ch0) { b->puni_recheck[k] = true; return; }
+    const uint8_t d = params_rows_equal(b->hp[c], b->hp[ch0]) ? 0 : 1;
+    b->stat_puni_rows_compared++;
+    b->puni_diff[k] += (long)d - (long)b->puni_differs[c]; b->puni_differs[c] = d;
+    b->kind_puni[k] = (b->puni_diff[k] == 0);
+    return;
+  }
+}
+
 void flush_host(asdr_batch *b, std::vector<int32_t> &rows_out, bool &bulk, bool &sched_rebuilt) {
   const int rows = b->n + 1;
   compact_agc_pool(b);
@@ -446,6 +479,7 @@
     }
     b->stat_rows_refilled = rows;
     b->stat_bulk_uploads++;
+    for (int k = 0; k < ASDR_KERNEL_KINDS; k++) b->puni_recheck[k] = true;
   } else if (!b->dirty.empty()) {
     std::sort(b->dirty.begin(), b->dirty.end());
     for (int32_t i : b->dirty) {
@@ -454,6 +488,7 @@
       if (sched_key(b->hp[i]) != old_key) b->sched_dirty = true;
       b->dirty_flag[i] = 0;
     }
+    if (!b->sched_dirty) for (int32_t i : b->dirty) if (i < b->n) puni_row_changed(b, i);
     rows_out = b->dirty;
     b->stat_rows_refilled = (long)rows_out.size();
   }
@@ -565,7 +600,9 @@
     b->sched_dirty = false;
     sched_rebuilt = true;
     b->stat_sched_rebuilds++;
-  }
+    for (int k = 0; k < ASDR_KERNEL_KINDS; k++) b->puni_recheck[k] = true;
+  }
+  for (int k = 0; k < ASDR_KERNEL_KINDS; k++) if (b->puni_recheck[k]) puni_pass(b, k);
 }
 
 int flush(asdr_batch *b, hipStream_t stream) {
@@ -619,6 +656,12 @@
   a.nb_phase = b->nb_phase; a.als_phase = b->als_phase;
   a.lo_cache = b->d_lo; a.lo_parity = b->lo_parity; a.lo_write = 0; a.lo_writer_bit = ASDR_LO_WRITER;
   a.k = b->k;
+}
+
+void set_uni(asdr_batch *b, UpdateArgs &a, int ch0) {
+  const int k = kernel_kind(b->hp[ch0]);
+  a.uni_valid = 0u;
+  if (b->uniform_params && b->kind_direct[k] && b->kind_puni[k] && b->sched[b->kind_first[k]].ch == ch0) { a.uni = b->hp[ch0]; a.uni_valid = 1u; }
 }
 
 int apply_resets(asdr_batch *b, hipStream_t stream) {
@@ -798,6 +841,7 @@
   b->sam_fused = getenv("ASDR_SAM_FUSED") != nullptr;
   b->sam_split_min = getenv("ASDR_SAM_SPLIT_MIN") ? atoi(getenv("ASDR_SAM_SPLIT_MIN")) : ASDR_SAM_SPLIT_MIN_CHANNELS;
   b->stream_pipeline = getenv("ASDR_NO_STREAM_PIPELINE") == nullptr;
+  b->uniform_params = getenv("ASDR_NO_UNIFORM_PARAMS") == nullptr;
   b->als_split_min = getenv("ASDR_ALS_SPLIT_MIN") ? atoi(getenv("ASDR_ALS_SPLIT_MIN")) : 0x7fffffff;
   if (getenv("ASDR_LAUNCH_SPLIT")) b->launch_split = std::max(1, std::min(atoi(getenv("ASDR_LAUNCH_SPLIT")), 8));
   if (getenv("ASDR_LAUNCH_SPLIT_MIN_WAVES")) b->launch_split_min_waves = std::max(8, atoi(getenv("ASDR_LAUNCH_SPLIT_MIN_WAVES")));
@@ -884,6 +928,7 @@
   b->hp.resize(rows);
   memset(b->hp.data(), 0, rows * sizeof(ChanParams));
   b->dirty_flag.assign(rows, 0);
+  b->puni_differs.assign(rows, 0);
   b->reset.assign(rows, ASDR_R_ALL);
   b->reset_lo = 0; b->reset_hi = (int)rows - 1;
   for (size_t i = 0; i < rows; i++) chan_init(b, (int)i);
@@ -1086,8 +1131,8 @@
     HIPCHK(hipMemsetAsync(b->d_stream_prog, 0, (size_t)(3 * w + 1) * sizeof(uint32_t), stream));
     if (n_sub > 1) HIPCHK(hipEventRecord(b->ev_fork, stream));
     a.sched = b->d_sched + subs[pipe_sub].first; a.n_sched = subs[pipe_sub].slots;
-    a.direct_ch0 = -1;
-    if (b->kind_direct[ASDR_KERNEL_PLAIN]) { const SlotInfo &s0 = b->sched[subs[pipe_sub].first]; a.direct_ch0 = s0.ch; a.direct_mode = s0.mode; a.direct_flags = s0.flags; a.direct_lo = s0.lo; }
+    a.direct_ch0 = -1; a.uni_valid = 0u;
+    if (b->kind_direct[ASDR_KERNEL_PLAIN]) { const SlotInfo &s0 = b->sched[subs[pipe_sub].first]; a.direct_ch0 = s0.ch; a.direct_mode = s0.mode; a.direct_flags = s0.flags; a.direct_lo = s0.lo; set_uni(b, a, s0.ch); }
     a.lo_write = 0u;
     a.xch_a = b->d_xch_a; a.xch_b = b->d_xch_b; a.xch_c = b->d_xch_b + (size_t)(b->n + 1) * ASDR_STREAM_DEPTH * ASDR_N; a.stream_prog = b->d_stream_prog; a.stream_err = b->d_stream_prog + 3 * ((b->n + 7) / 8) + 1;
     a.stream_waves = w; a.lo_ring = b->d_lo_ring; a.stream_spin_limit = b->stream_spin_limit;
@@ -1112,8 +1157,8 @@
         if (!s) return fail("stream creation failed");
         HIPCHK(hipStreamWaitEvent(s, b->ev_fork, 0));
         UpdateArgs o = a_side;
-        o.sched = b->d_sched + subs[i].first; o.n_sched = subs[i].slots; o.direct_ch0 = -1; o.lo_write = 1u;
-        if (subs[i].uniform && b->kind_direct[subs[i].kind]) { const SlotInfo &s0 = b->sched[subs[i].first]; o.direct_ch0 = s0.ch; o.direct_mode = s0.mode; o.direct_flags = s0.flags; o.direct_lo = s0.lo; }
+        o.sched = b->d_sched + subs[i].first; o.n_sched = subs[i].slots; o.direct_ch0 = -1; o.uni_valid = 0u; o.lo_write = 1u;
+        if (subs[i].uniform && b->kind_direct[subs[i].kind]) { const SlotInfo &s0 = b->sched[subs[i].first]; o.direct_ch0 = s0.ch; o.direct_mode = s0.mode; o.direct_flags = s0.flags; o.direct_lo = s0.lo; set_uni(b, o, s0.ch); }
         if (asdr_launch_update(&o, subs[i].kind, subs[i].uniform, s) != 0) return fail("update kernel launch failed");
         HIPCHK(hipEventRecord(b->ev_join[n_aux - 1], s));
       }
@@ -1157,8 +1202,8 @@
           if (cnt == 0) continue;
           UpdateArgs al = a;
           al.sched = b->d_sched + first; al.n_sched = cnt;
-          al.direct_ch0 = -1;
-          if (su.uniform && b->kind_direct[su.kind]) { const SlotInfo &s0 = b->sched[su.first]; al.direct_ch0 = s0.ch + lo; al.direct_mode = s0.mode; al.direct_flags = s0.flags; al.direct_lo = s0.lo; }
+          al.direct_ch0 = -1; al.uni_valid = 0u;
+          if (su.uniform && b->kind_direct[su.kind]) { const SlotInfo &s0 = b->sched[su.first]; al.direct_ch0 = s0.ch + lo; al.direct_mode = s0.mode; al.direct_flags = s0.flags; al.direct_lo = s0.lo; set_uni(b, al, s0.ch); }
           al.lo_cache = b->d_lo + (size_t)(1 + (l % ASDR_LANES)) * 2 * ASDR_LO_ENTRIES;
           al.lo_write = 1u;
           al.lo_writer_bit = ASDR_LO_WRITER_LANE(l % ASDR_LANES);
@@ -1230,8 +1275,8 @@
     for (int i = 0; i < 3 * R; i++) if (!b->ev_samc[i]) HIPCHK(hipEventCreateWithFlags(&b->ev_samc[i], hipEventDisableTiming));
     const int i0 = items[0].sub, first0 = items[0].first;
     const size_t slots = b->xch_sam_chunk_slots;
-    a.sched = b->d_sched + first0; a.n_sched = items[0].slots; a.direct_ch0 = -1; a.lo_write = 1u;
-    if (b->kind_direct[subs[i0].kind]) { const SlotInfo &s0 = b->sched[subs[i0].first]; a.direct_ch0 = s0.ch; a.direct_mode = s0.mode; a.direct_flags = s0.flags; a.direct_lo = s0.lo; }
+    a.sched = b->d_sched + first0; a.n_sched = items[0].slots; a.direct_ch0 = -1; a.uni_valid = 0u; a.lo_write = 1u;
+    if (b->kind_direct[subs[i0].kind]) { const SlotInfo &s0 = b->sched[subs[i0].first]; a.direct_ch0 = s0.ch; a.direct_mode = s0.mode; a.direct_flags = s0.flags; a.direct_lo = s0.lo; set_uni(b, a, s0.ch); }
     a.xch_sam = b->d_xch_sam_chunk; a.sam_lock = reinterpret_cast<uint32_t *>(b->d_xch_sam_chunk + (size_t)S * slots * 2 * ASDR_N);
     a.sam_sets = (uint32_t)S; a.sam_set_stride = (uint32_t)(slots * 2 * ASDR_N); a.sam_lock_stride = (uint32_t)slots;
     a.taps = nullptr;
@@ -1273,8 +1318,8 @@
     HIPCHK(hipEventRecord(b->ev_fork, stream));
     HIPCHK(hipStreamWaitEvent(s_chain, b->ev_fork, 0));
     const int i0 = items[0].sub, first0 = items[0].first;
-    a.sched = b->d_sched + first0; a.n_sched = items[0].slots; a.direct_ch0 = -1; a.lo_write = 1u;
-    if (b->kind_direct[subs[i0].kind]) { const SlotInfo &s0 = b->sched[subs[i0].first]; a.direct_ch0 = s0.ch; a.direct_mode = s0.mode; a.direct_flags = s0.flags; a.direct_lo = s0.lo; }
+    a.sched = b->d_sched + first0; a.n_sched = items[0].slots; a.direct_ch0 = -1; a.uni_valid = 0u; a.lo_write = 1u;
+    if (b->kind_direct[subs[i0].kind]) { const SlotInfo &s0 = b->sched[subs[i0].first]; a.direct_ch0 = s0.ch; a.direct_mode = s0.mode; a.direct_flags = s0.flags; a.direct_lo = s0.lo; set_uni(b, a, s0.ch); }
     a.als_stage = b->d_als_stage; a.als_stage_cur = 0u; a.als_stage_prev = (uint32_t)(S - 1); a.als_phase = b->als_phase;
     if (asdr_launch_als_stage_seed(&a, 0, b->n, s_chain) != 0) return fail("update kernel launch failed");
     const int n_chunks = (n_blocks + G - 1) / G;
@@ -1330,11 +1375,11 @@
       if (!s && it != main_item) return fail("stream creation failed");
       if (it != main_item) HIPCHK(hipStreamWaitEvent(s, b->ev_fork, 0));
       a.sched = b->d_sched + first; a.n_sched = items[it].slots;
-      a.direct_ch0 = -1;
+      a.direct_ch0 = -1; a.uni_valid = 0u;
       a.lo_write = 1u;
       if (subs[i].uniform && b->kind_direct[subs[i].kind]) {
         const SlotInfo &s0 = b->sched[subs[i].first];
-        a.direct_ch0 = s0.ch + (first - subs[i].first); a.direct_mode = s0.mode; a.direct_flags = s0.flags; a.direct_lo = s0.lo;
+        a.direct_ch0 = s0.ch + (first - subs[i].first); a.direct_mode = s0.mode; a.direct_flags = s0.flags; a.direct_lo = s0.lo; set_uni(b, a, s0.ch);
         if (first != subs[i].first) a.lo_write = 0u;
       }
       const bool sam3 = sam_split && (subs[i].kind == ASDR_KERNEL_SAM || subs[i].kind == ASDR_KERNEL_SAM_ALS);
@@ -2275,6 +2320,20 @@
   return 0;
 }
 
+int asdr_params_uniform_groups(asdr_batch_t *b, long *rows_compared) {
+  if (!b) return fail("null batch");
+  if (is_sharded(b)) {
+    int acc = 0; long rows = 0;
+    for (asdr_batch *sh : b->shards) { long r = 0; const int g = asdr_params_uniform_groups(sh, &r); if (g < 0) return -1; acc += g; rows += r; }
+    if (rows_compared) *rows_compared = rows;
+    return acc;
+  }
+  int g = 0;
+  for (int k = 0; k < ASDR_KERNEL_KINDS; k++) g += (b->kind_direct[k] && b->kind_puni[k]) ? 1 : 0;
+  if (rows_compared) *rows_compared = b->stat_puni_rows_compared;
+  return g;
+}
+
 int asdr_control_plane_flush(asdr_batch_t *b, long long stats[4]) {
   if (!b) return fail("null batch");
   if (is_sharded(b)) {
diff --git a/audiosdr_amd/csrc/asdr_kernels.hip b/audiosdr_amd/csrc/asdr_kernels.hip
--- a/audiosdr_amd/csrc/asdr_kernels.hip
+++ b/audiosdr_amd/csrc/asdr_kernels.hip
@@ -895,7 +895,7 @@
       }
     }
 }
-template <int STRIDE, bool HAS_ALS, bool HAS_SAM, bool UNIFORM, int WAVES, int ROLE = 0, bool ONEBLK_ = false, int FIR_HELPERS = 1>
+template <int STRIDE, bool HAS_ALS, bool HAS_SAM, bool UNIFORM, int WAVES, int ROLE = 0, bool ONEBLK_ = false, int FIR_HELPERS = 1, bool UPAR = false>
 __device__ __forceinline__ void asdr_update_body(const UpdateArgs &a, float *lds_wg) {
   constexpr bool C16 = (STRIDE == 320);
   constexpr bool PRE_ROLE = (ROLE == 4 || ROLE == 8), POST_ROLE = (ROLE == 5 || ROLE == 9 || ROLE == 10), LOOPED_ROLE = (ROLE == 7 || ROLE == 8 || ROLE == 9 || ROLE == 10);
@@ -968,6 +968,7 @@
   const int loff_ = c8 * STRIDE;
 #define P (*Pp)
   const ChainConsts K = a.k;
+  auto pv = [](float x) -> float { if constexpr (UPAR) asm volatile("" : "+v"(x)); return x; };
 
   const uint32_t mode = UNIFORM ? (uint32_t)__builtin_amdgcn_readfirstlane(slot.y) : (uint32_t)slot.y;
   const uint32_t pflags = UNIFORM ? (uint32_t)__builtin_amdgcn_readfirstlane(slot.z) : (uint32_t)slot.z;
@@ -1035,7 +1036,7 @@
       if (need_in) { seen_in = stream_wait(prog + (ROLE - 2) * a.stream_waves + wave_g, b1, err, a.stream_spin_limit); if (seen_in == ASDR_STREAM_FAIL) break; }
       if (need_free) { seen_free = stream_wait(prog + ROLE * a.stream_waves + wave_g, freed, err, a.stream_spin_limit); if (seen_free == ASDR_STREAM_FAIL) break; }
     }
-    const ChanParams *Pp = row_ptr(a.params, (uint32_t)ch * (uint32_t)sizeof(ChanParams));
+    const ChanParams *Pp = UPAR ? &a.uni : row_ptr(a.params, (uint32_t)ch * (uint32_t)sizeof(ChanParams));
     ChanSmall *S = row_ptr(a.small, (uint32_t)ch * (uint32_t)sizeof(ChanSmall));
     float *L = lds + loff;
     int *Li = reinterpret_cast<int *>(L);
@@ -1049,8 +1050,8 @@
 #define PL_CH(c) (__builtin_amdgcn_ds_bpermute((c) << 5, ch))
 #define Sp row_ptr(a.small, (uint32_t)PL_CH(pl_c) * (uint32_t)sizeof(ChanSmall))
 #define Spa row_ptr(a.small, (uint32_t)PL_CH(pa_c) * (uint32_t)sizeof(ChanSmall))
-#define Ppl row_ptr(a.params, (uint32_t)PL_CH(pl_c) * (uint32_t)sizeof(ChanParams))
-#define Ppa row_ptr(a.params, (uint32_t)PL_CH(pa_c) * (uint32_t)sizeof(ChanParams))
+#define Ppl (UPAR ? &a.uni : row_ptr(a.params, (uint32_t)PL_CH(pl_c) * (uint32_t)sizeof(ChanParams)))
+#define Ppa (UPAR ? &a.uni : row_ptr(a.params, (uint32_t)PL_CH(pa_c) * (uint32_t)sizeof(ChanParams)))
 #define Lp (lds + pl_c * STRIDE)
 #define Lpa (lds + pa_c * STRIDE)
 #else
@@ -1147,7 +1148,7 @@
     uint32_t mkc[5] = {0x01010101u, 0x01010101u, 0x01010101u, 0x01010101u, 0x01010101u};
     float gain_i, gain_q;
     if (ROLE == 1 && ASDR_STREAM_R1_CARRY && blk > 0) { gain_i = r1_gain_i; gain_q = r1_gain_q; }
-    else { gain_i = P.in_gain_i; gain_q = P.in_gain_q; if (ROLE == 1) { r1_gain_i = gain_i; r1_gain_q = gain_q; } }
+    else { gain_i = pv(P.in_gain_i); gain_q = pv(P.in_gain_q); if (ROLE == 1) { r1_gain_i = gain_i; r1_gain_q = gain_q; } }
     float g_oi = gain_i, g_oq = gain_q, g_mi = 0.0f, g_mq = 0.0f, nb_avg0 = 0.0f;
     uint32_t agc_hc_early = 0u, agc_hang_early = 0u;
     bool agc_piped = false;
@@ -1193,7 +1194,7 @@
 
     if (nb_wave) {
     } else if (DO1) {
-      const bool unit_in = UNIT_OK && __all(gain_i == 1.0f && gain_q == 1.0f);
+      const bool unit_in = UNIT_OK && (UPAR ? (a.uni.in_gain_i == 1.0f && a.uni.in_gain_q == 1.0f) : __all(gain_i == 1.0f && gain_q == 1.0f));
 #pragma unroll
       for (int h = 0; h < 2; ++h) {
         float xi[8], xq[8];
@@ -1495,7 +1496,7 @@
       WAVE_SYNC();
       uint32_t fm = 0u, ft = 0u;
       if (nb_en) {
-        const float thr = nb_thr;
+        const float thr = pv(nb_thr);
 #pragma unroll
         for (int h = 0; h < 2; ++h) {
           float av[8];
@@ -1984,7 +1985,7 @@
           const int chq = mw_channel(16 * (mw_rel - 1) + mw_casc);
           mw_af_S = row_ptr(a.small, (uint32_t)chq * (uint32_t)sizeof(ChanSmall));
           af_s4 = *reinterpret_cast<const float4 *>(&mw_af_S->af_state[4 * pl_st]);
-          const float *cf = &c_bq_pool[row_ptr(a.params, (uint32_t)chq * (uint32_t)sizeof(ChanParams))->audio_table][5 * pl_st];
+          const float *cf = &c_bq_pool[(UPAR ? &a.uni : row_ptr(a.params, (uint32_t)chq * (uint32_t)sizeof(ChanParams)))->audio_table][5 * pl_st];
 #pragma unroll
           for (int z = 0; z < 5; ++z) af_cf[z] = cf[z];
         }
@@ -2104,7 +2105,10 @@
           r2_pref = true;
         }
       }
-      constexpr bool IDL_EARLY = (ROLE == 2);
+#ifndef ASDR_UPAR_IDL_EARLY
+#define ASDR_UPAR_IDL_EARLY 1
+#endif
+      constexpr bool IDL_EARLY = (ROLE == 2) || (UPAR && ASDR_UPAR_IDL_EARLY != 0);
       if (IDL_EARLY && is_ssb) {
 #pragma unroll
         for (int m = 0; m < 4; ++m) load4(hi_ring + (hs ^ 1u) * 128 + 32 * m, idl + 4 * m);
@@ -2611,7 +2615,7 @@
             } else {
             const int chq = mw_channel(q);
             ChanSmall *Sq = row_ptr(a.small, (uint32_t)chq * (uint32_t)sizeof(ChanSmall));
-            const ChanParams *Pq = row_ptr(a.params, (uint32_t)chq * (uint32_t)sizeof(ChanParams));
+            const ChanParams *Pq = UPAR ? &a.uni : row_ptr(a.params, (uint32_t)chq * (uint32_t)sizeof(ChanParams));
             mwx[MWX * q + 7] = agc_chain(std::false_type{}, lds_wg + q * STRIDE, Sq, Sq->agc_old_abs, Sq->agc_hang_counter, Sq->agc_gain, Pq->agc_alpha_att, Pq->agc_beta_att,
                                        Pq->agc_alpha_rel, Pq->agc_beta_rel, Pq->agc_hang_count, is_am, mwx[MWX * q + 6]);
             }
@@ -2789,7 +2793,7 @@
       }
     }
     {
-      const float og = P.output_gain;
+      const float og = pv(P.output_gain);
       union { int4 v; int16_t s[8]; } ro[2];
 #pragma unroll
       for (int h = 0; h < 2; ++h) {
@@ -2887,6 +2891,10 @@
 extern "C" __global__ __launch_bounds__(64 * ASDR_MW_WAVES, ASDR_WAVES_PER_EU) void asdr_update_kernel_mw(UpdateArgs a) {
   __shared__ __attribute__((aligned(16))) float lds[ASDR_MW_WAVES * 8 * ASDR_STRIDE + ASDR_MW_WAVES * 8 * 16 + 260 + 12];
   asdr_update_body<ASDR_STRIDE, false, false, true, ASDR_MW_WAVES, 0, true>(a, lds);
+}
+extern "C" __global__ __launch_bounds__(64 * ASDR_MW_WAVES, ASDR_WAVES_PER_EU) void asdr_update_kernel_mw_u(UpdateArgs a) {
+  __shared__ __attribute__((aligned(16))) float lds[ASDR_MW_WAVES * 8 * ASDR_STRIDE + ASDR_MW_WAVES * 8 * 16 + 260 + 12];
+  asdr_update_body<ASDR_STRIDE, false, false, true, ASDR_MW_WAVES, 0, true, 1, true>(a, lds);
 }
 ASDR_KERNEL(asdr_update_kernel_sam, ASDR_SAM_WAVES * 8 * ASDR_STRIDE + 260, ASDR_WAVES_PER_EU, ASDR_STRIDE, false, true, false, ASDR_SAM_WAVES)
 #ifndef ASDR_ALS_WAVES_PER_EU
@@ -3212,6 +3220,7 @@
   "asdr_update_kernel_c16",
   "asdr_update_kernel_mixed",
   "asdr_update_kernel_mw",
+  "asdr_update_kernel_mw_u",
   "asdr_update_kernel_one",
   "asdr_update_kernel_sam"
 };
@@ -3350,6 +3359,9 @@
     if (uniform && c16_on && a->n_blocks == 1 && a->run_if == nullptr && a->direct_ch0 >= 0 && a->taps == nullptr && ssb_class && n_waves >= c16_min)
       ASDR_LAUNCH(asdr_update_kernel_c16, dim3(n_waves), dim3(64), (size_t)c16_pad, stream, *a);
     else
+    if (uniform && mw_on && a->n_blocks == 1 && a->run_if == nullptr && a->direct_ch0 >= 0 && n_waves >= mw_min && a->uni_valid)
+      ASDR_LAUNCH(asdr_update_kernel_mw_u, dim3((n_waves + ASDR_MW_WAVES - 1) / ASDR_MW_WAVES), dim3(64 * ASDR_MW_WAVES), 0, stream, *a);
+    else
     if (uniform && mw_on && a->n_blocks == 1 && a->run_if == nullptr && a->direct_ch0 >= 0 && n_waves >= mw_min)
       ASDR_LAUNCH(asdr_update_kernel_mw, dim3((n_waves + ASDR_MW_WAVES - 1) / ASDR_MW_WAVES), dim3(64 * ASDR_MW_WAVES), 0, stream, *a);
     else
diff --git a/include/asdr.h b/include/asdr.h
--- a/include/asdr.h
+++ b/include/asdr.h
@@ -150,6 +150,7 @@
 int asdr_kernel_timing_begin(asdr_batch_t *b, int max_launches);
 int asdr_kernel_timing_end(asdr_batch_t *b, float *ms, int cap);
 int asdr_control_plane_flush(asdr_batch_t *b, long long stats[4]);
+int asdr_params_uniform_groups(asdr_batch_t *b, long *rows_compared);
 unsigned int asdr_get_chain_constants(asdr_batch_t *b, int ch, float out[12]);
 int asdr_set_exact_unknown_mode(asdr_batch_t *b, int on);
 int asdr_get_exact_unknown_mode(asdr_batch_t *b);
```
